# philips/janus

Hardware: AMD Instinct MI355X
Metric: reports prepared+aggregated/sec (helper, Prio3Histogram len=256) at 1/2/4/8 GPUs (higher is better)
Workload: dtype u32 limbs (Field128 mod-p integer arithmetic); 1 GPU; Prio3Histogram length=256 chunk_length=16 helper prepare_init+prepare_shares_to_prepare_message+prepare_next+aggregate, 1 segment; reports_per_gpu=1048576, global_batch=1048576, parallelism=dp1 (report shards; RCCL all-gather + mod-p combine)

## Files before the change

### janus_amd/csrc/prio3_accumulate.hip

```cpp
#include <hip/hip_runtime.h>

#include <algorithm>
#include <type_traits>

#include "prio3_host.h"
#include "sha256_device.h"

struct ZeroRanges {
  uint8_t* dst[4];
  size_t bytes[4];
};
__global__ __launch_bounds__(256) void k_zero(ZeroRanges z) {
  const size_t tid = blockIdx.x * (size_t)blockDim.x + threadIdx.x, nth = (size_t)gridDim.x * blockDim.x;
#pragma unroll
  for (int k = 0; k < 4; k++) {
    uint8_t* d = z.dst[k];
    const size_t n = z.bytes[k];
    if (!d || !n) continue;
    const size_t head = std::min(n, (size_t)((16 - ((uintptr_t)d & 15)) & 15));
    const size_t n16 = (n - head) / 16;
    for (size_t i = tid; i < n16; i += nth) ((uint4*)(d + head))[i] = make_uint4(0, 0, 0, 0);
    for (size_t i = tid * 4; i < head; i += nth * 4) *(uint32_t*)(d + i) = 0u;
    for (size_t i = head + 16 * n16 + tid * 4; i < n; i += nth * 4) *(uint32_t*)(d + i) = 0u;
  }
}


template <class F, int SG>
__global__ __launch_bounds__(256) void k_acc_seg(uint32_t n, size_t ld, uint32_t chunk,
                                                 uint32_t out_len, uint32_t nseg, const void* src,
                                                 const uint8_t* status, const uint32_t* seg,
                                                 const uint8_t* accept, void* partial,
                                                 uint64_t* pcount) {
  typedef typename F::T T;
  __shared__ T red[256];
  __shared__ uint32_t cred[256];
  const uint32_t e = blockIdx.x, c = blockIdx.y, s0 = blockIdx.z * SG;
  const uint32_t lo = c * chunk, hi = min(n, lo + chunk);
  T acc[SG];
  uint32_t cnt[SG];
#pragma unroll
  for (int q = 0; q < SG; q++) {
    acc[q] = F::zero();
    cnt[q] = 0;
  }
  for (uint32_t r = lo + threadIdx.x; r < hi; r += 256) {
    const uint32_t sr = seg ? seg[r] : 0u;
    const bool ok = status[r] == PRIO3_STATUS_FINISHED && sr < nseg && (!accept || accept[r]);
    const uint32_t k = (ok ? sr : 0xffffffffu) - s0;
    if (k < (uint32_t)SG) {
      const T x = F::load(src, (size_t)e * ld + r);
#pragma unroll
      for (int q = 0; q < SG; q++)
        if ((uint32_t)q == k) {
          acc[q] = F::add(acc[q], x);
          cnt[q]++;
        }
    }
  }
#pragma unroll
  for (int q = 0; q < SG; q++) {
    if (s0 + q >= nseg) break;
    red[threadIdx.x] = acc[q];
    cred[threadIdx.x] = cnt[q];
    __syncthreads();
    for (uint32_t st = 128; st > 0; st >>= 1) {
      if (threadIdx.x < st) {
        red[threadIdx.x] = F::add(red[threadIdx.x], red[threadIdx.x + st]);
        cred[threadIdx.x] += cred[threadIdx.x + st];
      }
      __syncthreads();
    }
    if (threadIdx.x == 0) {
      F::store(partial, ((size_t)c * nseg + s0 + q) * out_len + e, red[0]);
      if (e == 0) pcount[(size_t)c * nseg + s0 + q] = cred[0];
    }
    __syncthreads();
  }
}

template <class F>
__global__ void k_acc_fin(uint32_t nchunks, uint32_t out_len, uint32_t nseg, const void* partial,
                          const uint64_t* pcount, uint8_t* agg, uint64_t* count) {
  typedef typename F::T T;
  const uint32_t e = blockIdx.x * blockDim.x + threadIdx.x, s = blockIdx.y;
  if (e < out_len) {
    T acc = F::zero();
    for (uint32_t c = 0; c < nchunks; c++)
      acc = F::add(acc, F::load(partial, ((size_t)c * nseg + s) * out_len + e));
    F::store(agg, (size_t)s * out_len + e, acc);
  }
  if (e == 0) {
    uint64_t t = 0;
    for (uint32_t c = 0; c < nchunks; c++) t += pcount[(size_t)c * nseg + s];
    count[s] = t;
  }
}


template <class F>
__global__ __launch_bounds__(256) void k_acc_fin_blk(uint32_t nchunks, uint32_t out_len,
                                                     uint32_t nseg, const void* partial,
                                                     const uint64_t* pcount, uint8_t* agg,
                                                     uint64_t* count) {
  typedef typename F::T T;
  __shared__ T red[256];
  __shared__ uint64_t cred[256];
  const uint32_t e = blockIdx.x, s = blockIdx.y;
  T acc = F::zero();
  uint64_t t = 0;
  for (uint32_t c = threadIdx.x; c < nchunks; c += 256) {
    acc = F::add(acc, F::load(partial, ((size_t)c * nseg + s) * out_len + e));
    if (e == 0) t += pcount[(size_t)c * nseg + s];
  }
  red[threadIdx.x] = acc;
  cred[threadIdx.x] = t;
  __syncthreads();
  for (uint32_t st = 128; st > 0; st >>= 1) {
    if (threadIdx.x < st) {
      red[threadIdx.x] = F::add(red[threadIdx.x], red[threadIdx.x + st]);
      cred[threadIdx.x] += cred[threadIdx.x + st];
    }
    __syncthreads();
  }
  if (threadIdx.x == 0) {
    F::store(agg, (size_t)s * out_len + e, red[0]);
    if (e == 0) count[s] = cred[0];
  }
}

template <class F>
__global__ __launch_bounds__(256) void k_acc_multi(const AccDesc* descs, uint8_t* base) {
  typedef typename F::T T;
  __shared__ T red[256];
  __shared__ uint32_t cred[256];
  const AccDesc d = descs[blockIdx.y];
  const uint32_t e = blockIdx.x;
  if (e >= d.out_len) return;
  const uint32_t* seg = (d.flags & 1) ? (const uint32_t*)(base + d.seg_off) : nullptr;
  const uint8_t* acc = (d.flags & 2) ? base + d.acc_off : nullptr;
  for (uint32_t s0 = 0; s0 < d.nseg; s0 += 8) {
    T a[8];
    uint32_t c[8];
#pragma unroll
    for (int q = 0; q < 8; q++) {
      a[q] = F::zero();
      c[q] = 0;
    }
    for (uint32_t r = threadIdx.x; r < d.n; r += 256) {
      const uint32_t s = seg ? seg[r] : 0u;
      const bool inc = d.status[r] == PRIO3_STATUS_FINISHED && s < d.nseg && (!acc || acc[r]);
      const uint32_t k = s - s0;
      if (inc && k < 8u) {
        const T x = F::load(d.src, (size_t)e * d.ld + r);
#pragma unroll
        for (int q = 0; q < 8; q++)
          if ((uint32_t)q == k) {
            a[q] = F::add(a[q], x);
            c[q]++;
          }
      }
    }
    const uint32_t ns = min(8u, d.nseg - s0);
    for (uint32_t q = 0; q < ns; q++) {
      T v = F::zero();
      uint32_t cv = 0;
#pragma unroll
      for (int q2 = 0; q2 < 8; q2++)
        if ((uint32_t)q2 == q) {
          v = a[q2];
          cv = c[q2];
        }
      red[threadIdx.x] = v;
      cred[threadIdx.x] = cv;
      __syncthreads();
      for (uint32_t st = 128; st > 0; st >>= 1) {
        if (threadIdx.x < st) {
          red[threadIdx.x] = F::add(red[threadIdx.x], red[threadIdx.x + st]);
          cred[threadIdx.x] += cred[threadIdx.x + st];
        }
        __syncthreads();
      }
      if (threadIdx.x == 0) {
        F::store(base + d.agg_off, (size_t)(s0 + q) * d.out_len + e, red[0]);
        if (e == 0) ((uint64_t*)(base + d.cnt_off))[s0 + q] = cred[0];
      }
      __syncthreads();
    }
  }
}

__global__ __launch_bounds__(256) void k_agg_waves(uint32_t nwaves, uint32_t M,
                                                   const uint32_t* wpart, const uint32_t* wseg,
                                                   unsigned long long* cpart, uint32_t* cseg,
                                                   unsigned long long* agg64) {
  static_assert(WCH <= 64, "one chunk's wave segments are read by one wave");
  const uint32_t slot = 4 * (blockIdx.x * blockDim.x + threadIdx.x), c = blockIdx.y;
  const uint32_t w0 = c * WCH, w1 = min(nwaves, w0 + WCH), lane = threadIdx.x & 63u;
  const uint32_t my = w0 + lane < w1 ? wseg[w0 + lane] : 0xffffffffu;
  const uint64_t fused = __ballot(my != 0xffffffffu);
  const uint32_t s0 = fused ? (uint32_t)__shfl((int)my, __ffsll((long long)fused) - 1) : 0xffffffffu;
  const bool mixed = __any(my != 0xffffffffu && my != s0);
  if (slot == 0 && blockIdx.x == 0) cseg[c] = mixed ? 0xffffffffu : s0;
  if (s0 == 0xffffffffu) return;
  const bool act = slot < M * 8;
  const uint32_t ls = act ? slot : 0u;
  const size_t row = (size_t)M * 8;
  if (!mixed) {
    if (!act) return;
    unsigned long long a0 = 0, a1 = 0, a2 = 0, a3 = 0;
#pragma unroll
    for (uint32_t i = 0; i < WCH; i++) {
      const uint32_t w = min(w0 + i, w1 - 1);
      const uint4 v = *(const uint4*)(wpart + (size_t)w * row + slot);
      const uint32_t m = 0u - (uint32_t)((fused >> i) & 1u);
      a0 += v.x & m, a1 += v.y & m, a2 += v.z & m, a3 += v.w & m;
    }
    unsigned long long* o = cpart + (size_t)c * row + slot;
    o[0] = a0, o[1] = a1, o[2] = a2, o[3] = a3;
    return;
  }
  unsigned long long a0 = 0, a1 = 0, a2 = 0, a3 = 0;
  uint32_t cur = 0xffffffffu;
  auto flush = [&]() {
    if (cur == 0xffffffffu || !act) return;
    unsigned long long* o = agg64 + (size_t)cur * row + slot;
    if (a0) atomicAdd(o, a0);
    if (a1) atomicAdd(o + 1, a1);
    if (a2) atomicAdd(o + 2, a2);
    if (a3) atomicAdd(o + 3, a3);
  };
#pragma unroll 1
  for (uint32_t b = 0; b < WCH; b += 8) {
    uint4 v[8];
#pragma unroll
    for (uint32_t j = 0; j < 8; j++)
      v[j] = *(const uint4*)(wpart + (size_t)min(w0 + b + j, w1 - 1) * row + ls);
#pragma unroll
    for (uint32_t j = 0; j < 8; j++) {
      const uint32_t sg = (uint32_t)__builtin_amdgcn_readlane((int)my, (int)(b + j));
      if (sg == 0xffffffffu) continue;
      if (sg != cur) {
        flush();
        cur = sg;
        a0 = a1 = a2 = a3 = 0;
      }
      a0 += v[j].x, a1 += v[j].y, a2 += v[j].z, a3 += v[j].w;
    }
  }
  flush();
}

constexpr uint32_t FIX_T = 64;
static uint32_t fix_per(uint32_t n) { return n >= (1u << 18) ? 4096u : 512u; }
__global__ __launch_bounds__(256) void k_agg_fix(uint32_t n, const uint8_t* status,
                                                 const uint32_t* seg, const uint8_t* accept,
                                                 const uint32_t* wseg, uint32_t* fix,
                                                 uint32_t fix_cap, uint32_t nseg,
                                                 unsigned long long* counts, uint32_t oor_masked,
                                                 uint32_t per, uint32_t wshift) {
  __shared__ uint32_t tseg[FIX_T];
  __shared__ unsigned int tcnt[FIX_T];
  if (threadIdx.x < FIX_T) {
    tseg[threadIdx.x] = 0xffffffffu;
    tcnt[threadIdx.x] = 0;
  }
  __syncthreads();
  const uint32_t lo = blockIdx.x * per, hi = min(n, lo + per);
  for (uint32_t base = lo; base < hi; base += 256) {
    const uint32_t r = base + threadIdx.x;
    const bool valid = r < hi;
    const uint32_t sg = valid ? (seg ? seg[r] : 0u) : 0xffffffffu;
    const bool inc = valid && sg < nseg && status[r] == PRIO3_STATUS_FINISHED &&
                     (!accept || accept[r]);
    const bool fused = valid && wseg[r >> wshift] != 0xffffffffu && (!oor_masked || sg < nseg);
    const uint32_t s0 = (uint32_t)__shfl((int)sg, 0);
    const bool uni = __all(!valid || sg == s0);
    const unsigned long long b = __ballot(inc);
    auto add = [&](uint32_t s, unsigned int k) {
      const uint32_t h = s % FIX_T;
      const uint32_t old = atomicCAS(&tseg[h], 0xffffffffu, s);
      if (old == 0xffffffffu || old == s) atomicAdd(&tcnt[h], k);
      else atomicAdd(&counts[s], (unsigned long long)k);
    };
    if (uni) {
      if ((threadIdx.x & 63u) == 0 && b) add(s0, (unsigned int)__popcll(b));
    } else if (inc) {
      add(sg, 1u);
    }
    if (valid && fused != inc) {
      const uint32_t i = atomicAdd(&fix[0], 1u);
      if (i < fix_cap) fix[1 + i] = r | (inc ? 0u : 0x80000000u);
    }
  }
  __syncthreads();
  if (threadIdx.x < FIX_T && tseg[threadIdx.x] != 0xffffffffu && tcnt[threadIdx.x])
    atomicAdd(&counts[tseg[threadIdx.x]], (unsigned long long)tcnt[threadIdx.x]);
}

DEV f128 fold_halves_impl(const unsigned long long (&Hs)[8]);
DEV f128 fold_halves(const unsigned long long (&Hs)[8]) { return fold_halves_impl(Hs); }

__global__ __launch_bounds__(256) void k_agg_final(uint32_t M, size_t ld,
                                                   const unsigned long long* agg64,
                                                   uint32_t nchunks,
                                                   const unsigned long long* cpart,
                                                   const uint32_t* cseg, const uint32_t* fix,
                                                   const uint32_t* seg, const void* meas,
                                                   uint8_t* agg) {
  const uint32_t idx = blockIdx.x, s = idx / M, e = idx % M;
  const uint32_t tid = threadIdx.x, h = tid & 7u, cl = tid >> 3;
  __shared__ unsigned long long red[256];
  __shared__ f128 fadd[256], fsub[256];
  unsigned long long acc = 0;
  for (uint32_t c = cl; c < nchunks; c += 32)
    if (cseg[c] == s) acc += cpart[((size_t)c * M + e) * 8 + h];
  red[tid] = acc;
  f128 ad = zero128(), sb = zero128();
  const uint32_t nfix = fix[0];
  for (uint32_t i = tid; i < nfix; i += 256) {
    const uint32_t ent = fix[1 + i], r = ent & 0x7fffffffu;
    if ((seg ? seg[r] : 0u) != s) continue;
    const f128 x = Fp128::load(meas, (size_t)e * ld + r);
    if (ent & 0x80000000u) sb = add128(sb, x);
    else ad = add128(ad, x);
  }
  fadd[tid] = ad;
  fsub[tid] = sb;
  __syncthreads();
  for (uint32_t st = 128; st >= 8; st >>= 1) {
    if (tid < st) red[tid] += red[tid + st];
    __syncthreads();
  }
  for (uint32_t st = 128; st >= 1; st >>= 1) {
    if (tid < st) {
      fadd[tid] = add128(fadd[tid], fadd[tid + st]);
      fsub[tid] = add128(fsub[tid], fsub[tid + st]);
    }
    __syncthreads();
  }
  if (tid != 0) return;
  unsigned long long Hs[8];
  for (int hh = 0; hh < 8; hh++) Hs[hh] = red[hh] + agg64[(size_t)idx * 8 + hh];
  Fp128::store(agg, idx, sub128(add128(fold_halves(Hs), fadd[0]), fsub[0]));
}

__global__ __launch_bounds__(256) void k_agg_final_s(uint32_t M, size_t ld,
                                                     const unsigned long long* agg64,
                                                     uint32_t nchunks,
                                                     const unsigned long long* cpart,
                                                     const uint32_t* cseg, const uint32_t* fix,
                                                     const uint32_t* seg, const void* meas,
                                                     uint8_t* agg) {
  const uint32_t s = blockIdx.y, tid = threadIdx.x, h = tid & 7u, lane = tid & 63u;
  const uint32_t e = blockIdx.x * 32u + (tid >> 3);
  const bool live = e < M;
  const uint32_t ec = live ? e : 0u;
  unsigned long long H = agg64[((size_t)s * M + ec) * 8 + h];
  for (uint32_t c = 0; c < nchunks; c++)
    if (cseg[c] == s) H += cpart[((size_t)c * M + ec) * 8 + h];
  f128 ad = zero128(), sb = zero128();
  const uint32_t nfix = fix[0];
  for (uint32_t i = h; i < nfix; i += 8) {
    const uint32_t ent = fix[1 + i], r = ent & 0x7fffffffu;
    if ((seg ? seg[r] : 0u) != s) continue;
    const f128 x = Fp128::load(meas, (size_t)ec * ld + r);
    if (ent & 0x80000000u) sb = add128(sb, x);
    else ad = add128(ad, x);
  }
  if (nfix) {
#pragma unroll
    for (int m = 1; m < 8; m <<= 1) {
      f128 xa, xs;
#pragma unroll
      for (int k = 0; k < 4; k++) {
        xa.w[k] = (uint32_t)__shfl_xor((int)ad.w[k], m);
        xs.w[k] = (uint32_t)__shfl_xor((int)sb.w[k], m);
      }
      ad = add128(ad, xa);
      sb = add128(sb, xs);
    }
  }
  unsigned long long Hs[8];
#pragma unroll
  for (int k = 0; k < 8; k++) {
    const int src = (int)((lane & ~7u) + (uint32_t)k);
    Hs[k] = ((unsigned long long)(uint32_t)__shfl((int)(uint32_t)(H >> 32), src) << 32) |
            (uint32_t)__shfl((int)(uint32_t)H, src);
  }
  if (h != 0 || !live) return;
  Fp128::store(agg, (size_t)s * M + e, sub128(add128(fold_halves(Hs), ad), sb));
}

DEV f128 fold_halves_impl(const unsigned long long (&Hs)[8]) {
  uint32_t w[9] = {0, 0, 0, 0, 0, 0, 0, 0, 0};
  for (int hh = 0; hh < 8; hh++) {
    const unsigned long long H = Hs[hh];
    const int sh = 16 * hh, wi = sh >> 5, bi = sh & 31;
    const unsigned long long lo = bi ? (H << 16) & 0xffffffffull : H & 0xffffffffull;
    const unsigned long long mid = bi ? (H >> 16) & 0xffffffffull : H >> 32;
    const unsigned long long hi = bi ? H >> 48 : 0ull;
    unsigned long long c = (unsigned long long)w[wi] + lo;
    w[wi] = (uint32_t)c;
    c = (unsigned long long)w[wi + 1] + mid + (c >> 32);
    w[wi + 1] = (uint32_t)c;
    c = (unsigned long long)w[wi + 2] + hi + (c >> 32);
    w[wi + 2] = (uint32_t)c;
    for (int k = wi + 3; k < 9 && (c >> 32); k++) {
      c = (unsigned long long)w[k] + (c >> 32);
      w[k] = (uint32_t)c;
    }
  }
  return red288(w, w[8]);
}

template <class F>
__global__ void k_combine(uint32_t k, uint32_t len, uint32_t n_segments, const uint8_t* in,
                          const uint64_t* cin, uint8_t* out, uint64_t* cout) {
  typedef typename F::T T;
  const uint32_t e = blockIdx.x * blockDim.x + threadIdx.x;
  if (e < len) {
    T acc = F::zero();
    for (uint32_t i = 0; i < k; i++) acc = F::add(acc, F::load(in, (size_t)i * len + e));
    F::store(out, e, acc);
  }
  if (e < n_segments) {
    uint64_t s = 0;
    for (uint32_t i = 0; i < k; i++) s += cin[(size_t)i * n_segments + e];
    cout[e] = s;
  }
}

DEV void sha256_id16(const uint32_t id[4], uint32_t out[8]) {
  uint32_t w[16];
#pragma unroll
  for (int i = 0; i < 4; i++) w[i] = __builtin_bswap32(id[i]);
  w[4] = 0x80000000u;
#pragma unroll
  for (int i = 5; i < 15; i++) w[i] = 0;
  w[15] = 128;
  uint32_t st[8];
#pragma unroll
  for (int i = 0; i < 8; i++) st[i] = sha256d::IV[i];
  sha256d::compress(st, w);
#pragma unroll
  for (int i = 0; i < 8; i++) out[i] = __builtin_bswap32(st[i]);
}

__global__ void k_meta_init(uint32_t n_segments, uint32_t* ck, unsigned long long* iv) {
  const uint32_t s = blockIdx.x * blockDim.x + threadIdx.x;
  if (s >= n_segments) return;
  if (ck)
    for (int i = 0; i < 8; i++) ck[8 * s + i] = 0;
  if (iv) {
    iv[2 * s] = ~0ull;
    iv[2 * s + 1] = 0;
  }
}

constexpr uint32_t META_T = 1024, META_W = META_T / 64, META_BLOCKS = 512;
__global__ __launch_bounds__(1024) void k_meta(uint32_t n, const uint8_t* ids, const uint64_t* times,
                                             const uint8_t* status, const uint8_t* mask,
                                             const uint32_t* seg, uint32_t n_segments, uint32_t* ck,
                                             unsigned long long* iv) {
  __shared__ uint32_t s_seg0;
  __shared__ uint32_t s_ck[META_W][8];
  __shared__ unsigned long long s_lo[META_W], s_hi[META_W];
  const uint32_t tid = threadIdx.x, lane = tid & 63u, wv = tid >> 6;
  uint32_t cur = 0xffffffffu, acc_x = 0;
  unsigned long long acc_lo = ~0ull, acc_hi = 0;
  auto flush = [&]() {
    if (cur != 0xffffffffu) {
      if (ck && tid < 8 && acc_x) atomicXor(ck + 8 * cur + tid, acc_x);
      if (iv && tid == 8 && acc_hi) {
        atomicMin(iv + 2 * cur, acc_lo);
        atomicMax(iv + 2 * cur + 1, acc_hi);
      }
    }
    acc_x = 0;
    acc_lo = ~0ull;
    acc_hi = 0;
  };
  for (uint32_t base = blockIdx.x * META_T; base < n; base += gridDim.x * META_T) {
    const uint32_t r = base + tid;
    const bool valid = r < n;
    const uint32_t sg = valid ? (seg ? seg[r] : 0u) : 0xffffffffu;
    const bool in_range = valid && sg < n_segments;
    const bool inc = in_range && status[r] == PRIO3_STATUS_FINISHED && (!mask || mask[r]);
    uint32_t h[8] = {0, 0, 0, 0, 0, 0, 0, 0};
    if (ck && inc) {
      uint32_t id[4];
      load16(ids + 16 * (size_t)r, id);
      sha256_id16(id, h);
    }
    unsigned long long lo = ~0ull, hi = 0;
    if (times && in_range) {
      lo = times[r];
      hi = lo + 1;
    }
    if (tid == 0) s_seg0 = sg;
    __syncthreads();
    const bool uniform = __syncthreads_and(!valid || sg == s_seg0) && s_seg0 < n_segments;
    if (uniform) {
#pragma unroll
      for (int off = 32; off >= 1; off >>= 1) {
#pragma unroll
        for (int i = 0; i < 8; i++) h[i] ^= (uint32_t)__shfl_xor((int)h[i], off);
        const unsigned long long l2 = __shfl_xor(lo, off), h2 = __shfl_xor(hi, off);
        lo = l2 < lo ? l2 : lo;
        hi = h2 > hi ? h2 : hi;
      }
      if (lane == 0) {
#pragma unroll
        for (int i = 0; i < 8; i++) s_ck[wv][i] = h[i];
        s_lo[wv] = lo;
        s_hi[wv] = hi;
      }
      __syncthreads();
      if (s_seg0 != cur) {
        flush();
        cur = s_seg0;
      }
      if (tid < 8) {
        uint32_t x = 0;
        for (uint32_t q = 0; q < META_W; q++) x ^= s_ck[q][tid];
        acc_x ^= x;
      }
      if (tid == 8) {
        for (uint32_t q = 0; q < META_W; q++) {
          acc_lo = s_lo[q] < acc_lo ? s_lo[q] : acc_lo;
          acc_hi = s_hi[q] > acc_hi ? s_hi[q] : acc_hi;
        }
      }
    } else {
      if (ck && inc)
#pragma unroll
        for (int i = 0; i < 8; i++) atomicXor(ck + 8 * sg + i, h[i]);
      if (iv && times && in_range) {
        atomicMin(iv + 2 * sg, lo);
        atomicMax(iv + 2 * sg + 1, hi);
      }
    }
    __syncthreads();
  }
  flush();
}

__global__ void k_combine_meta(uint32_t k, uint32_t n_segments, const uint32_t* ck_in,
                               const unsigned long long* iv_in, uint32_t* ck_out,
                               unsigned long long* iv_out) {
  const uint32_t t = blockIdx.x * blockDim.x + threadIdx.x;
  if (t >= n_segments * 8) return;
  const uint32_t s = t >> 3, w = t & 7u;
  if (ck_in && ck_out) {
    uint32_t x = 0;
    for (uint32_t i = 0; i < k; i++) x ^= ck_in[((size_t)i * n_segments + s) * 8 + w];
    ck_out[(size_t)s * 8 + w] = x;
  }
  if (iv_in && iv_out && w == 0) {
    unsigned long long lo = ~0ull, hi = 0;
    for (uint32_t i = 0; i < k; i++) {
      const unsigned long long a = iv_in[((size_t)i * n_segments + s) * 2];
      const unsigned long long d = iv_in[((size_t)i * n_segments + s) * 2 + 1];
      if (d == 0) continue;
      lo = a < lo ? a : lo;
      hi = a + d > hi ? a + d : hi;
    }
    iv_out[2 * s] = hi ? lo : 0;
    iv_out[2 * s + 1] = hi ? hi - lo : 0;
  }
}

__global__ void k_meta_final(uint32_t n_segments, unsigned long long* iv) {
  const uint32_t s = blockIdx.x * blockDim.x + threadIdx.x;
  if (s >= n_segments) return;
  const unsigned long long lo = iv[2 * s], hi = iv[2 * s + 1];
  iv[2 * s] = hi ? lo : 0;
  iv[2 * s + 1] = hi ? hi - lo : 0;
}


template <class Fn>
static int by_field(size_t es, Fn fn) {
  return es == 16 ? fn(Fp128{}) : fn(Fp64{});
}

int run_accumulate(prio3_engine* e, Run* R, uint32_t c0, uint32_t n, const uint8_t* d_status,
                   const uint32_t* d_seg, const uint8_t* d_accept, uint32_t nseg, uint8_t* d_agg,
                   uint64_t* d_counts, hipStream_t st) {
  const DevParams& d = R->dp;
  const size_t es = d.es, agg_len = (size_t)d.out_len * es;
  if (n == 0) {
    HIPCHK(hipMemsetAsync(d_agg, 0, agg_len * nseg, st));
    HIPCHK(hipMemsetAsync(d_counts, 0, 8 * (size_t)nseg, st));
    return PRIO3_OK;
  }
  const bool short_out = d.out_len <= 4;
  const uint32_t chunk = short_out ? 2048 : 8192, nchunks = (n + chunk - 1) / chunk;
  const size_t part_b = ((size_t)nchunks * nseg * agg_len + 255) & ~(size_t)255;
  int rc = PRIO3_OK;
  Slab* tmp = ws_acquire(R->device, part_b + 8 * (size_t)nchunks * nseg, st, &rc);
  if (!tmp) return rc;
  void* partial = tmp->base;
  uint64_t* pcount = (uint64_t*)(tmp->base + part_b);
  const uint8_t* src = run_out_shares(R, c0);
  const size_t ld = d.ld_out;
  const int SG = nseg == 1 ? 1 : nseg <= 4 ? 4 : 8;
  const dim3 grid(d.out_len, nchunks, (nseg + SG - 1) / SG);
  rc = by_field(es, [&](auto f) -> int {
    using F = decltype(f);
    auto seg = [&](auto sg) -> int {
      TIMED(e, st, "k_acc_seg",
            (k_acc_seg<F, decltype(sg)::value><<<grid, 256, 0, st>>>(
                n, ld, chunk, d.out_len, nseg, src, d_status, d_seg, d_accept, partial, pcount)));
      return PRIO3_OK;
    };
    const int rs = SG == 1   ? seg(std::integral_constant<int, 1>{})
                   : SG == 4 ? seg(std::integral_constant<int, 4>{})
                             : seg(std::integral_constant<int, 8>{});
    if (rs) return rs;
    if (short_out)
      TIMED(e, st, "k_acc_fin",
            (k_acc_fin_blk<F><<<dim3(d.out_len, nseg), 256, 0, st>>>(
                nchunks, d.out_len, nseg, partial, pcount, d_agg, d_counts)));
    else
      TIMED(e, st, "k_acc_fin",
            (k_acc_fin<F><<<dim3((d.out_len + 255) / 256, nseg), 256, 0, st>>>(
                nchunks, d.out_len, nseg, partial, pcount, d_agg, d_counts)));
    return PRIO3_OK;
  });
  ws_release(tmp, st);
  R->last = st;
  return rc;
}

int fused_finish(prio3_engine* e, Run* R, const uint8_t* d_status, const uint32_t* seg,
                 const uint32_t* fix_seg, const uint8_t* d_accept_mask, uint32_t S,
                 uint8_t* d_agg_shares, uint64_t* d_counts, hipStream_t st) {
  const uint32_t n = R->n, M = R->dp.meas_len, ws = R->wshift;
  const uint32_t nwaves = (n + (1u << ws) - 1) >> ws;
  {
    ZeroRanges z{};
    z.dst[0] = (uint8_t*)R->agg64;
    z.bytes[0] = (size_t)S * M * 8 * 8;
    z.dst[1] = (uint8_t*)R->fix;
    z.bytes[1] = sizeof(uint32_t);
    z.dst[2] = (uint8_t*)d_counts;
    z.bytes[2] = 8 * (size_t)S;
    TIMED(e, st, "k_zero", (k_zero<<<std::min<uint32_t>(256, (uint32_t)((z.bytes[0] / 16 + 255) / 256) + 1), 256, 0, st>>>(z)));
  }
  const uint32_t nchunks = (nwaves + WCH - 1) / WCH;
  dim3 g1((M * 8 / 4 + 255) / 256, nchunks);
  TIMED(e, st, "k_agg_waves",
        (k_agg_waves<<<g1, 256, 0, st>>>(nwaves, M, R->wpart, R->wseg, R->cpart, R->cseg,
                                         R->agg64)));
  TIMED(e, st, "k_agg_fix",
        (k_agg_fix<<<(n + fix_per(n) - 1) / fix_per(n), 256, 0, st>>>(
            n, d_status, seg, d_accept_mask, R->wseg, R->fix, (uint32_t)(R->fix_cap - 1), S,
            (unsigned long long*)d_counts, fix_seg ? 1u : 0u, fix_per(n), ws)));
  if (nchunks <= 64 && S > 1)
    TIMED(e, st, "k_agg_final",
          (k_agg_final_s<<<dim3((M + 31) / 32, S), 256, 0, st>>>(
              M, R->dp.ld, R->agg64, nchunks, R->cpart, R->cseg, R->fix, fix_seg, R->sc.meas,
              d_agg_shares)));
  else
    TIMED(e, st, "k_agg_final",
          (k_agg_final<<<S * M, 256, 0, st>>>(M, R->dp.ld, R->agg64, nchunks, R->cpart, R->cseg,
                                               R->fix, fix_seg, R->sc.meas, d_agg_shares)));
  return PRIO3_OK;
}

Slab* acc_multi_enqueue(int device, uint32_t es, uint8_t* host, const AccLayout& L,
                        uint32_t n_jobs, size_t out_bytes, hipStream_t st, int* rc) {
  const AccDesc* D = (const AccDesc*)(host + L.desc_off);
  uint32_t reps = 0, max_len = 0;
  for (uint32_t i = 0; i < n_jobs; i++) {
    reps = std::max(reps, (uint32_t)((D[i].acc_off - L.acc_off) + D[i].n));
    max_len = std::max(max_len, D[i].out_len);
  }
  Slab* sl = ws_acquire(device, L.bytes, st, rc);
  if (!sl) return nullptr;
  uint8_t* b = sl->base;
  auto h2d = [&](size_t off, size_t bytes) {
    return hipMemcpyAsync(b + off, host + off, bytes, hipMemcpyHostToDevice, st) == hipSuccess;
  };
  bool ok = h2d(L.desc_off, sizeof(AccDesc) * n_jobs) && h2d(L.seg_off, 4 * (size_t)reps) &&
            h2d(L.acc_off, reps);
  if (ok) {
    by_field(es, [&](auto f) -> int {
      k_acc_multi<decltype(f)><<<dim3(max_len, n_jobs), 256, 0, st>>>(
          (const AccDesc*)(b + L.desc_off), b);
      return 0;
    });
    ok = hipGetLastError() == hipSuccess &&
         hipMemcpyAsync(host + L.out_off, b + L.out_off, out_bytes, hipMemcpyDeviceToHost, st) ==
             hipSuccess;
  }
  if (ok) return sl;
  (void)hipStreamSynchronize(st);
  ws_release(sl, st);
  *rc = PRIO3_EDEVICE;
  return nullptr;
}

int launch_combine(prio3_engine* e, uint32_t k, uint32_t n_segments, const uint8_t* d_in,
                   const uint64_t* d_counts_in, uint8_t* d_out, uint64_t* d_counts_out,
                   hipStream_t st) {
  const uint32_t len = e->dp.out_len * n_segments;
  const uint32_t blocks = (std::max(len, n_segments) + 255) / 256;
  return by_field(e->dp.es, [&](auto f) -> int {
    TIMED(e, st, "k_combine",
          (k_combine<decltype(f)><<<blocks, 256, 0, st>>>(k, len, n_segments, d_in, d_counts_in,
                                                          d_out, d_counts_out)));
    return PRIO3_OK;
  });
}

int launch_batch_metadata(prio3_engine* e, uint32_t n, const uint8_t* d_report_ids,
                          const uint64_t* d_times, const uint8_t* d_status,
                          const uint8_t* d_accept_mask, const uint32_t* d_segment_ids,
                          uint32_t n_segments, uint32_t* ck, unsigned long long* iv,
                          hipStream_t st) {
  const uint32_t sb = (n_segments + 255) / 256;
  TIMED(e, st, "k_meta_init", (k_meta_init<<<sb, 256, 0, st>>>(n_segments, ck, iv)));
  if (n)
    TIMED(e, st, "k_meta",
          (k_meta<<<std::min((n + META_T - 1) / META_T, META_BLOCKS), META_T, 0, st>>>(
              n, d_report_ids, d_times, d_status, d_accept_mask, d_segment_ids, n_segments, ck,
              d_times ? iv : nullptr)));
  if (iv) TIMED(e, st, "k_meta_final", (k_meta_final<<<sb, 256, 0, st>>>(n_segments, iv)));
  return PRIO3_OK;
}

int launch_combine_metadata(prio3_engine* e, uint32_t k, uint32_t n_segments,
                            const uint32_t* ck_in, const unsigned long long* iv_in,
                            uint32_t* ck_out, unsigned long long* iv_out, hipStream_t st) {
  TIMED(e, st, "k_combine_meta",
        (k_combine_meta<<<(n_segments * 8 + 255) / 256, 256, 0, st>>>(k, n_segments, ck_in, iv_in,
                                                                      ck_out, iv_out)));
  return PRIO3_OK;
}
```

### janus_amd/csrc/prio3_common.h

```cpp
#pragma once
#include <atomic>
#include <mutex>
#include <string>
#include <vector>
#include "../../include/janus_prio3.h"
#include "prio3_device.h"

#define MAX_ROOTS 20

#ifdef JANUS_DEVICE_CHECKS
#define DCHECK(c)                                                                        \
  do {                                                                                   \
    if (!(c)) {                                                                          \
      printf("janus device check failed: %s (%s:%d) block %u thread %u\n", #c, __FILE__, \
             __LINE__, (unsigned)blockIdx.x, (unsigned)threadIdx.x);                     \
      __builtin_trap();                                                                  \
    }                                                                                    \
  } while (0)
#else
#define DCHECK(c) ((void)0)
#endif

struct DevParams {
  uint32_t kind, es, meas_len, out_len, jr_len, arity, calls, P, logP, glen, proof_len,
      verifier_len, chunk, bits, length, prep_share_len, helper_share_len, public_share_len,
      leader_share_len;
  uint32_t n, ld, force_slow;
  uint32_t nseg;
  uint32_t qr_len, ld_out;
  uint32_t chunk1, calls1, P1, logP1, glen1;
  uint32_t invP1_128[4], normc128[4], twon128[4];
  uint32_t vk[4];
  uint32_t dst[8][2];
  uint32_t roots128[MAX_ROOTS + 1][4];
  uint64_t roots64[MAX_ROOTS + 1];
  uint32_t invP128[4], half128[4];
  uint32_t sigma128[32][4];
  uint32_t tw128[16][4];
  uint64_t invP64, half64;
  const uint4* sigma_dev;
  uint32_t trunc_xof;
  uint32_t slow_defer, redo;
  uint32_t tws[24][4];
#ifdef JANUS_TEST_REJECT
  uint32_t test_reject;
#endif
};
#ifdef JANUS_TEST_REJECT
#define REJ_BITS(p) ((p).test_reject)
#define BX_REJ(x) ((x).rej)
#define BX_SET_REJ(x, p) ((x).rej = (p).test_reject)
#else
#define REJ_BITS(p) 0u
#define BX_REJ(x) 0u
#define BX_SET_REJ(x, p) ((void)0)
#endif

struct InPtrs {
  const uint8_t* nonces;
  const uint8_t* pub;
  const uint8_t* helper;
  const uint8_t* leader;
  const uint16_t* vk_slot = nullptr;
  const uint4* vk_tab = nullptr;
  const uint8_t* leader_src = nullptr;
  const uint32_t* seg_src = nullptr;
  uint32_t* seg_dst = nullptr;
  const uint8_t* accept_src = nullptr;
  uint8_t* accept_dst = nullptr;
  uint32_t lin_ld = 0;
};

DEV void load_vk(const DevParams& p, const InPtrs& in, uint32_t r, uint32_t vk[4]) {
  if (in.vk_slot) {
    const uint4 v = in.vk_tab[in.vk_slot[r]];
    vk[0] = v.x;
    vk[1] = v.y;
    vk[2] = v.z;
    vk[3] = v.w;
  } else {
    vk[0] = p.vk[0];
    vk[1] = p.vk[1];
    vk[2] = p.vk[2];
    vk[3] = p.vk[3];
  }
}

struct Scratch {
  void* meas;
  void* proofs;
  void* jr;
  void* qr;
  uint4* part;
  uint4* corrected;
  uint8_t* flag;
  void* Lbuf;
  void* PVbuf;
  void* acc;
  void* out;
  void* beta;
  const uint32_t* seg;
  uint32_t* wpart;
  uint32_t* wseg;
};

struct OutPtrs {
  uint8_t* prep_msgs;
  uint8_t* status;
};

template <class F>
struct FC;
template <>
struct FC<Fp128> {
  static DEV f128 root(const DevParams& p, int l) { return Fp128::from_words(p.roots128[l]); }
  static DEV f128 invP(const DevParams& p) { return Fp128::from_words(p.invP128); }
  static DEV f128 half(const DevParams& p) { return Fp128::from_words(p.half128); }
};
template <>
struct FC<Fp64> {
  static DEV uint64_t root(const DevParams& p, int l) { return p.roots64[l]; }
  static DEV uint64_t invP(const DevParams& p) { return p.invP64; }
  static DEV uint64_t half(const DevParams& p) { return p.half64; }
};

DEV void load16(const uint8_t* p, uint32_t* w) {
  uint4 v = *(const uint4*)p;
  w[0] = v.x;
  w[1] = v.y;
  w[2] = v.z;
  w[3] = v.w;
}

DEV bool prep_msg_check(const DevParams& p, const InPtrs& in, const Scratch& sc, uint32_t r,
                        const uint32_t lpart[4], uint32_t msg[4]) {
  const uint4 cor = sc.corrected[r];
  uint32_t hpart[4];
  {
    const uint4 hp = sc.part[r];
    hpart[0] = hp.x, hpart[1] = hp.y, hpart[2] = hp.z, hpart[3] = hp.w;
  }
  KState s;
  kzero(s);
  Msg mm;
  msg_zero(mm);
  msg_dst(mm, p.dst[6]);
  msg_bytes16(mm, 25, lpart);
  msg_bytes16(mm, 41, hpart);
  msg_absorb_final(s, mm, 57);
  msg[0] = kword(s, 0), msg[1] = kword(s, 1), msg[2] = kword(s, 2), msg[3] = kword(s, 3);
  return msg[0] == cor.x && msg[1] == cor.y && msg[2] == cor.z && msg[3] == cor.w;
}

struct BX {
  KState s;
  uint8_t buf[168];
  uint32_t pos;
#ifdef JANUS_TEST_REJECT
  uint32_t rej = 0;
#endif
};
DEV void bx_xor_block(BX& x) {
#pragma unroll
  for (int w = 0; w < 42; w++) {
    uint32_t v = (uint32_t)x.buf[4 * w] | ((uint32_t)x.buf[4 * w + 1] << 8) |
                 ((uint32_t)x.buf[4 * w + 2] << 16) | ((uint32_t)x.buf[4 * w + 3] << 24);
    kxor_word(x.s, w, v);
  }
  keccak_p12(x.s);
}
DEV void bx_fill(BX& x) {
#pragma unroll
  for (int w = 0; w < 42; w++) {
    uint32_t v = kword(x.s, w);
    x.buf[4 * w] = v;
    x.buf[4 * w + 1] = v >> 8;
    x.buf[4 * w + 2] = v >> 16;
    x.buf[4 * w + 3] = v >> 24;
  }
  x.pos = 0;
}
DEV void bx_absorb(BX& x, uint8_t b) {
  x.buf[x.pos++] = b;
  if (x.pos == 168) {
    bx_xor_block(x);
    x.pos = 0;
  }
}
DEV void bx_absorb_w(BX& x, const uint32_t* w, int nbytes) {
  for (int i = 0; i < nbytes; i++) bx_absorb(x, (uint8_t)(w[i >> 2] >> (8 * (i & 3))));
}
DEV void bx_init(BX& x, const uint32_t* dst2, const uint32_t* seed) {
  kzero(x.s);
  x.pos = 0;
  bx_absorb(x, 8);
  bx_absorb_w(x, dst2, 8);
  bx_absorb_w(x, seed, 16);
}
DEV void bx_finalize(BX& x) {
  for (uint32_t i = x.pos; i < 168; i++) x.buf[i] = 0;
  x.buf[x.pos] ^= 0x01;
  x.buf[167] ^= 0x80;
  bx_xor_block(x);
  bx_fill(x);
}
DEV uint8_t bx_squeeze(BX& x) {
  if (x.pos == 168) {
    keccak_p12(x.s);
    bx_fill(x);
  }
  return x.buf[x.pos++];
}
template <class F>
DEV void bx_next_elem(BX& x, uint32_t* w) {
  for (;;) {
    for (int k = 0; k < F::ES / 4; k++) {
      uint32_t v = 0;
      for (int b = 0; b < 4; b++) v |= (uint32_t)bx_squeeze(x) << (8 * b);
      w[k] = v;
    }
    if (F::accept(F::from_words(w), BX_REJ(x))) return;
  }
}

template <class F>
DEV void bx_expand(const DevParams& p, const uint32_t* dst2, const uint32_t* seed,
                   const uint8_t* binder, int blen, uint32_t n, void* base, size_t ld,
                   uint32_t r) {
  BX x;
  BX_SET_REJ(x, p);
  bx_init(x, dst2, seed);
  for (int i = 0; i < blen; i++) bx_absorb(x, binder[i]);
  bx_finalize(x);
  for (uint32_t i = 0; i < n; i++) {
    uint32_t w[4];
    bx_next_elem<F>(x, w);
    F::store(base, (size_t)i * ld + r, F::from_words(w));
  }
}

template <class F>
DEV void put_elem(const DevParams& p, void* base, uint32_t idx, uint32_t r, const uint32_t* w,
                  uint32_t& flag) {
  typename F::T x = F::from_words(w);
  if (!F::accept(x, REJ_BITS(p))) flag = 1;
  DCHECK(r < p.ld);
  F::store(base, (size_t)idx * p.ld + r, x);
}

template <class F, class Put>
DEV void squeeze_block_with(const KState& s, uint32_t b, uint32_t n_elems, uint32_t& pend0,
                            uint32_t& pend1, Put&& put) {
  if constexpr (F::ES == 16) {
    uint32_t e0 = 21 * (b >> 1);
    if ((b & 1) == 0) {
#pragma unroll
      for (int t = 0; t < 10; t++) {
        uint32_t w[4] = {kword(s, 4 * t), kword(s, 4 * t + 1), kword(s, 4 * t + 2),
                         kword(s, 4 * t + 3)};
        if (e0 + t < n_elems) put(e0 + t, w);
      }
      pend0 = kword(s, 40);
      pend1 = kword(s, 41);
    } else {
      {
        uint32_t w[4] = {pend0, pend1, kword(s, 0), kword(s, 1)};
        if (e0 + 10 < n_elems) put(e0 + 10, w);
      }
#pragma unroll
      for (int t = 0; t < 10; t++) {
        uint32_t w[4] = {kword(s, 2 + 4 * t), kword(s, 3 + 4 * t), kword(s, 4 + 4 * t),
                         kword(s, 5 + 4 * t)};
        if (e0 + 11 + t < n_elems) put(e0 + 11 + t, w);
      }
    }
  } else {
    uint32_t e0 = 21 * b;
#pragma unroll
    for (int t = 0; t < 21; t++) {
      uint32_t w[2] = {kword(s, 2 * t), kword(s, 2 * t + 1)};
      if (e0 + t < n_elems) put(e0 + t, w);
    }
  }
}

template <class F>
DEV void squeeze_block(const DevParams& p, const KState& s, uint32_t b, uint32_t n_elems,
                       uint32_t& pend0, uint32_t& pend1, void* base, uint32_t r,
                       uint32_t& flag) {
  squeeze_block_with<F>(s, b, n_elems, pend0, pend1, [&](uint32_t i, const uint32_t* w) {
    put_elem<F>(p, base, i, r, w, flag);
  });
}

DEV void shl_add160(sum128& a, const f128& m, uint32_t s) {
  uint32_t w0 = m.w[0], w1 = m.w[1], w2 = m.w[2], w3 = m.w[3], w4 = 0;
  if (s) {
    const uint32_t rs = 32 - s;
    w4 = m.w[3] >> rs;
    w3 = __builtin_amdgcn_alignbit(m.w[3], m.w[2], rs);
    w2 = __builtin_amdgcn_alignbit(m.w[2], m.w[1], rs);
    w1 = __builtin_amdgcn_alignbit(m.w[1], m.w[0], rs);
    w0 = m.w[0] << s;
  }
  uint32_t c;
  a.w[0] = addc(a.w[0], w0, 0, &c);
  a.w[1] = addc(a.w[1], w1, c, &c);
  a.w[2] = addc(a.w[2], w2, c, &c);
  a.w[3] = addc(a.w[3], w3, c, &c);
  a.w[4] = a.w[4] + w4 + c;
}

struct TruncSink {
  void* out;
  size_t ld_out;
  uint32_t r, nb, n_ent, e, bit;
  sum128 acc;
  DEV TruncSink(const DevParams& p, void* o, uint32_t rr)
      : out(o), ld_out(p.ld_out), r(rr), nb(p.bits), n_ent(p.out_len), e(0), bit(0) {
    sum_zero(acc);
  }
  DEV void put(const f128& m) {
    if (e >= n_ent) return;
    shl_add160(acc, m, bit);
    if (++bit == nb) {
      Fp128::store(out, (size_t)e * ld_out + r, sum_reduce(acc));
      sum_zero(acc);
      bit = 0;
      e++;
    }
  }
};

template <bool TR>
DEV void squeeze_meas(const DevParams& p, const KState& s, uint32_t b, uint32_t n_elems,
                      uint32_t& pend0, uint32_t& pend1, void* base, uint32_t r, uint32_t& flag,
                      TruncSink& ts) {
  squeeze_block_with<Fp128>(s, b, n_elems, pend0, pend1, [&](uint32_t i, const uint32_t* w) {
    put_elem<Fp128>(p, base, i, r, w, flag);
    if constexpr (TR) ts.put(mk128(w[0], w[1], w[2], w[3]));
  });
}


DEV uint32_t bitrev(uint32_t x, uint32_t d) { return __builtin_bitreverse32(x) >> (32 - d); }

template <class F>
DEV void dft_lane(const DevParams& p, void* buf, uint32_t r, uint32_t n, uint32_t logn) {
  typedef typename F::T T;
  const size_t ld = p.ld;
  DCHECK(r < ld);
  for (uint32_t l = 1; l <= logn; l++) {
    const uint32_t half = 1u << (l - 1);
    const T wl = FC<F>::root(p, l);
    T w = F::one();
    for (uint32_t i = 0; i < half; i++) {
      for (uint32_t j = i; j < n; j += 2 * half) {
        T u = F::load(buf, (size_t)j * ld + r);
        T v = F::mul(w, F::load(buf, (size_t)(j + half) * ld + r));
        F::store(buf, (size_t)j * ld + r, F::add(u, v));
        F::store(buf, (size_t)(j + half) * ld + r, F::sub(u, v));
      }
      w = F::mul(w, wl);
    }
  }
}

template <class F>
DEV typename F::T ldf(const void* base, uint32_t e, size_t ld, uint32_t r) {
  DCHECK(r < ld);
  return F::load(base, (size_t)e * ld + r);
}


template <int N, int LOGN>
DEV void dft_reg(const DevParams& p, f128 (&x)[N], int stride) {
  typedef Fp128 F;
#pragma unroll
  for (int l = 1; l <= LOGN; l++) {
    const int half = 1 << (l - 1);
#pragma unroll
    for (int i = 0; i < half; i++) {
      const f128 w = F::from_words(p.tw128[i * stride * (N >> l)]);
#pragma unroll
      for (int j = i; j < N; j += 2 * half) {
        const f128 u = x[j];
        const f128 v = (i == 0) ? x[j + half] : F::mul(w, x[j + half]);
        x[j] = F::add(u, v);
        x[j + half] = F::sub(u, v);
      }
    }
  }
}

template <class F>
DEV bool flp_query_lane(const DevParams& p, const void* meas, const void* proofs, const void* jr,
                        typename F::T t, void* Lbuf, void* PVbuf, void* acc, uint32_t r,
                        typename F::T& v, typename F::T& pt) {
  typedef typename F::T T;
  const size_t ld = p.ld;
  const uint32_t P = p.P, A = p.arity;
  T tp = t;
  for (uint32_t l = 0; l < p.logP; l++) tp = F::mul(tp, tp);
  const bool t_ok = !F::eq(tp, F::one());
  {
    T pw = FC<F>::invP(p);
    for (uint32_t e = 0; e < P; e++) {
      F::store(Lbuf, (size_t)bitrev(e, p.logP) * ld + r, pw);
      pw = F::mul(pw, t);
    }
    dft_lane<F>(p, Lbuf, r, p.P, p.logP);
  }
  for (uint32_t e = 0; e < P; e++) {
    T q = ldf<F>(proofs, A + e, ld, r);
    if (e + P < p.glen) q = F::add(q, ldf<F>(proofs, A + e + P, ld, r));
    F::store(PVbuf, (size_t)bitrev(e, p.logP) * ld + r, q);
  }
  dft_lane<F>(p, PVbuf, r, p.P, p.logP);
  pt = F::zero();
  for (uint32_t e = p.glen; e-- > 0;) pt = F::add(F::mul(pt, t), ldf<F>(proofs, A + e, ld, r));
  auto Lc = [&](uint32_t c) { return ldf<F>(Lbuf, (P - c) & (P - 1), ld, r); };
  {
    const T L0 = Lc(0);
    for (uint32_t w = 0; w < A; w++)
      F::store(acc, (size_t)w * ld + r, F::mul(ldf<F>(proofs, w, ld, r), L0));
  }
  auto acc_add = [&](uint32_t w, const T& v) {
    size_t idx = (size_t)w * ld + r;
    F::store(acc, idx, F::add(F::load(acc, idx), v));
  };
  v = F::zero();
  if (p.kind == PRIO3_COUNT) {
    const T m = ldf<F>(meas, 0, ld, r);
    const T x = F::mul(m, Lc(1));
    acc_add(0, x);
    acc_add(1, x);
    v = F::sub(ldf<F>(PVbuf, 1, ld, r), m);
  } else if (p.kind == PRIO3_SUM) {
    const T r0 = ldf<F>(jr, 0, ld, r);
    T rp = r0;
    for (uint32_t i = 0; i < p.meas_len; i++) {
      acc_add(0, F::mul(ldf<F>(meas, i, ld, r), Lc(i + 1)));
      v = F::add(v, F::mul(rp, ldf<F>(PVbuf, i + 1, ld, r)));
      rp = F::mul(rp, r0);
    }
  } else {
    const T r0 = ldf<F>(jr, 0, ld, r);
    const T half = FC<F>::half(p);
    T rp = r0, range = F::zero(), sum = F::zero();
    for (uint32_t k = 0; k < p.calls; k++) {
      const T L = Lc(k + 1);
      for (uint32_t j = 0; j < p.chunk; j++) {
        const uint32_t i = k * p.chunk + j;
        const T m = i < p.meas_len ? ldf<F>(meas, i, ld, r) : F::zero();
        acc_add(2 * j, F::mul(F::mul(rp, m), L));
        acc_add(2 * j + 1, F::mul(F::sub(m, half), L));
        rp = F::mul(rp, r0);
        sum = F::add(sum, m);
      }
      range = F::add(range, ldf<F>(PVbuf, k + 1, ld, r));
    }
    if (p.kind == PRIO3_SUMVEC) {
      v = range;
    } else {
      const T r1 = ldf<F>(jr, 1, ld, r);
      v = F::add(F::mul(r1, range), F::mul(F::mul(r1, r1), F::sub(sum, half)));
    }
  }
  return t_ok;
}

namespace {

typedef unsigned __int128 u128;
const u128 HP128 = (((u128)0xffffffffffffffe4ULL) << 64) | 1;
const uint64_t HP64 = 0xffffffff00000001ULL;

u128 hmul(u128 a, u128 b, u128 p) {
  u128 r = 0;
  a %= p;
  while (b) {
    if (b & 1) {
      r += a;
      if (r < a || r >= p) r -= p;
    }
    u128 a2 = a + a;
    if (a2 < a || a2 >= p) a2 -= p;
    a = a2;
    b >>= 1;
  }
  return r;
}
u128 hpow(u128 a, u128 e, u128 p) {
  u128 r = 1;
  while (e) {
    if (e & 1) r = hmul(r, a, p);
    a = hmul(a, a, p);
    e >>= 1;
  }
  return r;
}

}

struct KTime {
  std::string name;
  double ms = 0;
  uint64_t launches = 0;
};

struct Mp64Params {
  uint32_t meas_len, out_len, bits, chunk, calls, P, logP, glen, proof_len ,
      arity, vlen, np;
  uint32_t dst[8][2];
  uint32_t vk_ist[8], vk_ost[8];
  uint32_t z_ist[8], z_ost[8];
  uint64_t alpha, alpha_inv, invP, half;
  const uint64_t* sigma;
};

struct prio3_engine;
bool query_sum_takes(const DevParams& p);
bool launch_query_sum(const DevParams& p, InPtrs in, Scratch sc, OutPtrs out, hipStream_t st,
                      bool leader = false);
int launch_mp64(prio3_engine* e, uint32_t n, uint32_t ld, InPtrs in, OutPtrs out, Scratch sc,
                hipStream_t st);
int launch_mp64_leader(prio3_engine* e, uint32_t n, uint32_t ld, InPtrs in, OutPtrs out,
                       Scratch sc, hipStream_t st);
int launch_mp64_leader_next(uint32_t n, const uint8_t* d_prep_msgs, Scratch sc, uint8_t* d_status,
                            hipStream_t st);
bool launch_xof_pair(const DevParams& p, InPtrs in, Scratch sc, hipStream_t st);
bool prep_pair_takes(const DevParams& p, bool pull);
bool launch_prep_pair(const DevParams& p, InPtrs in, Scratch sc, OutPtrs out, hipStream_t st,
                      bool fuse, bool pull);
bool launch_query_wide(const DevParams& p, InPtrs in, Scratch sc, OutPtrs out, hipStream_t st);
bool query_wide_takes(const DevParams& p);
void launch_fpvec_query(const DevParams& p, InPtrs in, Scratch sc, OutPtrs out, hipStream_t st,
                        bool wide, bool leader);
bool fpvec_query_wide_takes(const DevParams& p);

struct Slab;
struct Run {
  prio3_engine* e = nullptr;
  Slab* slab = nullptr;
  int device = 0;
  DevParams dp;
  uint32_t n = 0;
  Scratch sc{};
  uint8_t *nonces = nullptr, *pub = nullptr, *helper = nullptr, *leader = nullptr,
          *linput = nullptr, *msgs = nullptr, *status = nullptr;
  uint32_t *wpart = nullptr, *wseg = nullptr, *cseg = nullptr, *fix = nullptr;
  uint4* corr_all = nullptr;
  unsigned long long *cpart = nullptr, *agg64 = nullptr;
  size_t fix_cap = 0;
  bool fused = false;
  bool aggregate = false;
  bool lfused = false;
  uint32_t wshift = 6;
  uint32_t nseg = 0;
  const uint32_t* seg = nullptr;
  uint32_t* gseg = nullptr;
  uint8_t *gaccept = nullptr, *gagg = nullptr, *gcnt = nullptr;
  std::atomic<int> refs{1};
  hipStream_t last = nullptr;
  bool keep = false;
  uint32_t hpke_stride = 0;
  uint8_t *hstatus = nullptr, *hpt = nullptr;
  uint32_t* hretry = nullptr;
  uint32_t* gck = nullptr;
  unsigned long long* giv = nullptr;
};

struct prio3_engine {
  prio3_params params;
  prio3_sizes_t sz;
  DevParams dp;
  int device;
  Run* cur = nullptr;
  int fuse_acc = 1;
  int leader_fast = 1;
  int leader_fuse_acc = 1;
  int chunks = 0;
  int64_t fp_sub_bytes = 0;
  int coalesce = 1;
  int experimental_fpvec = 0;
  std::vector<hipStream_t> side;
  std::vector<hipEvent_t> side_ev;
  hipEvent_t fork_ev = nullptr;
  int force_slow = 0;
  int force_generic = 0;
  int n_cu = 256;
  int fp_round = 1;
  int pair_max = 196608;
  int timing = 0;
  int keep_scratch = 0;
  int upload_aead = 0;
  Mp64Params mp{};
  uint64_t* d_sigma64 = nullptr;
  uint4* d_sigma128 = nullptr;
  std::vector<KTime> times;
  std::mutex tmu;
  std::mutex mu;
  int lane = 0;
  std::vector<prio3_engine*> members;
  prio3_engine* owner = nullptr;
  std::atomic<uint32_t> rr{0};
  std::atomic<uint64_t> placed_jobs{0}, placed_reports{0};
};
```

### janus_amd/csrc/prio3_engine.hip

```cpp
#include <hip/hip_runtime.h>

#include <cstdio>
#include <cstdlib>
#include <cstring>
#include <mutex>
#include <string>
#include <type_traits>
#include <vector>

#include "../../include/janus_hpke.h"
#include "../../include/janus_prio3.h"
#include "prio3_host.h"
#include "sha256_host.h"

DEV void pull_body(const PullRanges& pr, size_t tid, size_t nth) {
#pragma unroll
  for (int k = 0; k < 4; k++) {
    const size_t n16 = pr.bytes[k] / 16;
    const uint4* s16 = (const uint4*)pr.src[k];
    uint4* d16 = (uint4*)pr.dst[k];
    for (size_t i = tid; i < n16; i += nth) d16[i] = s16[i];
    const size_t t = 16 * n16 + tid;
    if (t < pr.bytes[k] && tid < 16) pr.dst[k][t] = pr.src[k][t];
  }
// ... 92 lines not shown
static uint32_t optimal_chunk_length(uint32_t m) {
  if (m <= 1) return 1;
  uint32_t max_log2 = 0;
  while ((1u << max_log2) < m) max_log2++;
  max_log2 += 1;
  uint64_t best = UINT64_MAX;
  uint32_t best_chunk = 1;
  for (uint32_t l = max_log2; l >= 1; l--) {
    const uint64_t calls = (1ull << l) - 1, chunk = (m + calls - 1) / calls;
    const uint64_t cost = 2 * chunk + 2 * ((1ull << l) - 1) + 1;
    if (cost < best) {
      best = cost;
      best_chunk = (uint32_t)chunk;
    }
  }
  return best_chunk;
}

static int fill_sizes(const prio3_params* pp, prio3_sizes_t* s, DevParams* dp) {
  if (!pp) return PRIO3_EINVAL;
  uint32_t proofs = pp->num_proofs ? pp->num_proofs : 1;
  const bool mp = pp->kind == PRIO3_SUMVEC_F64_MP;
  if (mp ? (proofs < 2 || proofs > 8) : proofs != 1) return mp ? PRIO3_EINVAL : PRIO3_EUNSUPPORTED;
  DevParams d;
  memset(&d, 0, sizeof d);
  d.kind = pp->kind;
  d.bits = pp->bits;
  d.length = pp->length;
  d.chunk = pp->chunk_length;
  uint32_t algo;
  switch (pp->kind) {
    case PRIO3_COUNT:
      algo = 0;
      d.es = 8;
      d.meas_len = 1;
      d.out_len = 1;
      d.jr_len = 0;
      d.arity = 2;
      d.calls = 1;
      break;
    case PRIO3_SUM:
      if (pp->bits == 0 || pp->bits > 64) return PRIO3_EINVAL;
      algo = 1;
      d.es = 16;
      d.meas_len = pp->bits;
      d.out_len = 1;
      d.jr_len = 1;
      d.arity = 1;
      d.calls = pp->bits;
      break;
    case PRIO3_SUMVEC:
      if (pp->bits == 0 || pp->bits > 64 || pp->length == 0 || pp->chunk_length == 0)
        return PRIO3_EINVAL;
      algo = 2;
      d.es = 16;
      d.meas_len = pp->bits * pp->length;
      d.out_len = pp->length;
      d.jr_len = 1;
      d.arity = 2 * pp->chunk_length;
      d.calls = (d.meas_len + pp->chunk_length - 1) / pp->chunk_length;
      break;
    case PRIO3_SUMVEC_F64_MP:
      if (pp->bits == 0 || pp->bits > 64 || pp->length == 0 || pp->chunk_length == 0)
        return PRIO3_EINVAL;
      algo = 0xFFFF1003u;
      d.es = 8;
      d.meas_len = pp->bits * pp->length;
      d.out_len = pp->length;
      d.jr_len = 1;
      d.arity = 2 * pp->chunk_length;
      d.calls = (d.meas_len + pp->chunk_length - 1) / pp->chunk_length;
      break;
    case PRIO3_FPVEC_BOUNDED_L2:
      if ((pp->bits != 16 && pp->bits != 32) || pp->length == 0 || pp->length > (1u << 22))
        return PRIO3_EINVAL;
      algo = 0xFFFF0000u;
      d.es = 16;
      d.meas_len = pp->bits * pp->length + 2 * pp->bits - 2;
      d.out_len = pp->length;
      d.jr_len = 2;
      d.qr_len = 2;
      d.chunk = optimal_chunk_length(d.meas_len);
      d.arity = 2 * d.chunk;
      d.calls = (d.meas_len + d.chunk - 1) / d.chunk;
      d.chunk1 = optimal_chunk_length(pp->length);
      d.calls1 = (pp->length + d.chunk1 - 1) / d.chunk1;
      break;
    case PRIO3_HISTOGRAM:
      if (pp->length == 0 || pp->chunk_length == 0) return PRIO3_EINVAL;
      algo = 3;
      d.es = 16;
      d.meas_len = pp->length;
      d.out_len = pp->length;
      d.jr_len = 2;
      d.arity = 2 * pp->chunk_length;
      d.calls = (pp->length + pp->chunk_length - 1) / pp->chunk_length;
      break;
    default:
      return PRIO3_EINVAL;
  }
  d.P = next_pow2(1 + d.calls);
  d.logP = 0;
  while ((1u << d.logP) < d.P) d.logP++;
  if (d.logP > MAX_ROOTS) return PRIO3_EUNSUPPORTED;
  d.glen = 2 * (d.P - 1) + 1;
  d.proof_len = d.arity + d.glen;
  d.verifier_len = d.arity + 2;
  if (!d.qr_len) d.qr_len = 1;
  if (d.kind == PRIO3_FPVEC_BOUNDED_L2) {
    d.P1 = next_pow2(1 + d.calls1);
    while ((1u << d.logP1) < d.P1) d.logP1++;
    if (d.logP1 > MAX_ROOTS) return PRIO3_EUNSUPPORTED;
    d.glen1 = 2 * (d.P1 - 1) + 1;
    d.proof_len += d.chunk1 + d.glen1;
    d.verifier_len = 1 + d.arity + 1 + d.chunk1 + 1;
  }
  const uint32_t S = mp ? 32 : 16;
  d.helper_share_len = d.jr_len ? 3 * S : 2 * S;
  d.public_share_len = d.jr_len ? 2 * S : 0;
  d.prep_share_len = d.verifier_len * proofs * d.es + (d.jr_len ? S : 0);
  d.leader_share_len = (d.meas_len + d.proof_len * proofs) * d.es + (d.jr_len ? S : 0);
  for (uint32_t u = 1; u <= 7; u++) {
    uint8_t b[8] = {8, 0, (uint8_t)(algo >> 24), (uint8_t)(algo >> 16), (uint8_t)(algo >> 8),
                    (uint8_t)algo, 0, (uint8_t)u};
    memcpy(d.dst[u], b, 8);
  }
  {
    u128 g128 = 0;
    for (const char* c = "145091266659756586618791329697897684742"; *c; c++)
      g128 = g128 * 10 + (u128)(*c - '0');
    uint64_t g64 = 1753635133440165772ULL;
    for (int l = 0; l <= MAX_ROOTS; l++) {
      u128 r = g128;
      for (int i = 0; i < 66 - l; i++) r = hmul(r, r, HP128);
      for (int k = 0; k < 4; k++) d.roots128[l][k] = (uint32_t)(r >> (32 * k));
      u128 r64 = g64;
      for (int i = 0; i < 32 - l; i++) r64 = hmul(r64, r64, HP64);
      d.roots64[l] = (uint64_t)r64;
    }
    u128 ip = hpow(d.P, HP128 - 2, HP128), h = hpow(2, HP128 - 2, HP128);
    for (int k = 0; k < 4; k++) {
      d.invP128[k] = (uint32_t)(ip >> (32 * k));
      d.half128[k] = (uint32_t)(h >> (32 * k));
    }
    d.invP64 = (uint64_t)hpow(d.P, HP64 - 2, HP64);
    if (d.kind == PRIO3_FPVEC_BOUNDED_L2) {
      const u128 ip1 = hpow(d.P1, HP128 - 2, HP128);
      const u128 nc = ((u128)d.out_len << (2 * d.bits - 2)) >> 1;
      const u128 tn = (u128)1 << d.bits;
      for (int k = 0; k < 4; k++) {
        d.invP1_128[k] = (uint32_t)(ip1 >> (32 * k));
        d.normc128[k] = (uint32_t)(nc >> (32 * k));
        d.twon128[k] = (uint32_t)(tn >> (32 * k));
      }
    }
    if (d.P <= 32) {
      u128 alpha = 0;
      for (int k = 0; k < 4; k++) alpha |= (u128)d.roots128[d.logP][k] << (32 * k);
      for (uint32_t e2 = 0; e2 < d.P; e2++) {
        u128 ae = hpow(alpha, e2, HP128), s = 0, x = 1;
        for (uint32_t cc = 1; cc <= d.calls; cc++) {
          x = hmul(x, ae, HP128);
          s += x;
          if (s < x || s >= HP128) s -= HP128;
        }
        for (int k = 0; k < 4; k++) d.sigma128[e2][k] = (uint32_t)(s >> (32 * k));
      }
      for (uint32_t i = 0; i < d.P / 2; i++) {
        u128 w = hpow(alpha, i, HP128);
        for (int k = 0; k < 4; k++) d.tw128[i][k] = (uint32_t)(w >> (32 * k));
      }
    } else if (d.P == 64 || d.P == 128) {
      u128 alpha = 0;
      for (int k = 0; k < 4; k++) alpha |= (u128)d.roots128[d.logP][k] << (32 * k);
      const u128 aq = hpow(alpha, 8, HP128);
      for (uint32_t i = 0; i < d.P / 16; i++) {
        const u128 w = hpow(aq, i, HP128);
        for (int k = 0; k < 4; k++) d.tw128[i][k] = (uint32_t)(w >> (32 * k));
      }
      for (uint32_t i = 0; i < 8; i++) {
        const u128 w = hpow(alpha, i, HP128);
        for (int k = 0; k < 4; k++) d.tw128[8 + i][k] = (uint32_t)(w >> (32 * k));
      }
    }
    if (d.P >= 16 && d.P <= 128) {
      u128 alpha = 0;
      for (int k = 0; k < 4; k++) alpha |= (u128)d.roots128[d.logP][k] << (32 * k);
      const u128 w16 = hpow(alpha, d.P / 16, HP128), a16 = hpow(alpha, 16, HP128);
      for (uint32_t i = 0; i < 8; i++) {
        const u128 v[3] = {hpow(w16, i, HP128), hpow(alpha, i, HP128), hpow(a16, i, HP128)};
        for (int t = 0; t < 3; t++)
          for (int k = 0; k < 4; k++) d.tws[8 * t + i][k] = (uint32_t)(v[t] >> (32 * k));
      }
    }
    d.half64 = (uint64_t)hpow(2, HP64 - 2, HP64);
  }
  if (s) {
    s->field_bytes = d.es;
    s->meas_len = d.meas_len;
    s->out_len = d.out_len;
    s->proof_len = d.proof_len;
    s->verifier_len = d.verifier_len;
    s->joint_rand_len = d.jr_len;
    s->nonce_len = 16;
    s->public_share_len = d.public_share_len;
    s->helper_share_len = d.helper_share_len;
    s->prep_share_len = d.prep_share_len;
    s->prep_msg_len = d.jr_len ? S : 0;
    s->agg_share_len = d.out_len * d.es;
    s->leader_input_share_len = d.leader_share_len;
  }
  d.proof_len *= proofs;
  if (dp) *dp = d;
  return PRIO3_OK;
}

std::vector<Pending>& pending() {
  static thread_local std::vector<Pending> v;
  return v;
}
size_t time_slot(prio3_engine* e, const char* name) {
  std::lock_guard<std::mutex> lk(e->tmu);
  for (size_t i = 0; i < e->times.size(); i++)
    if (e->times[i].name == name) return i;
  e->times.push_back(KTime{name, 0, 0});
  return e->times.size() - 1;
}
void count_launch(prio3_engine* e, const char* name) {
  const size_t i = time_slot(e, name);
  std::lock_guard<std::mutex> lk(e->tmu);
  e->times[i].launches += 1;
}
void collect_times(prio3_engine* e, bool wait) {
  auto& v = pending();
  std::vector<Pending> keep;
  for (auto& pd : v) {
    if (pd.e != e || (!wait && hipEventQuery(pd.b) == hipErrorNotReady)) {
      keep.push_back(pd);
      continue;
    }
    float ms = 0;
    (void)hipEventSynchronize(pd.b);
    (void)hipEventElapsedTime(&ms, pd.a, pd.b);
    {
      std::lock_guard<std::mutex> lk(e->tmu);
      e->times[pd.idx].ms += ms;
      e->times[pd.idx].launches += 1;
    }
    (void)hipEventDestroy(pd.a);
    (void)hipEventDestroy(pd.b);
  }
  v.swap(keep);
}

static size_t fp_column_bytes(const DevParams& d) {
  const size_t es = d.es;
  return es * ((size_t)d.meas_len + d.proof_len + d.jr_len + d.qr_len + 2 * ((size_t)d.P + d.P1) +
               d.calls) +
         16 + 16 + 1;
}

static uint32_t fp_sub_ld(const prio3_engine* e, const DevParams& d, uint32_t ld_out,
                          size_t other_bytes) {
  const size_t per = fp_column_bytes(d);
  int64_t budget = e->fp_sub_bytes;
  if (budget <= 0) {
    size_t fr = 0, tot = 0, idle = 0;
    if (hipMemGetInfo(&fr, &tot) != hipSuccess) {
      (void)hipGetLastError();
      fr = tot = 0;
    }
    (void)ws_pool_bytes(e->device, &idle);
    const int64_t outb = (int64_t)(d.es * d.out_len * (size_t)ld_out + 64 * (size_t)ld_out);
    const int64_t reserve = std::max<int64_t>((int64_t)8 << 30, (int64_t)(0.10 * (double)tot));
    budget = (int64_t)(fr + idle) - outb - reserve - (int64_t)other_bytes;
  }
  uint64_t cols = (uint64_t)std::max<int64_t>(budget, 1) / per;
  cols = std::max<uint64_t>(256, cols & ~255ull);
  return (uint32_t)std::min<uint64_t>(ld_out, cols);
}

static size_t run_carve(Run* R, unsigned flags, uint8_t* base) {
  const DevParams& d = R->dp;
  const size_t es = d.es, ld = d.ld, ldo = d.ld_out, n = R->n ? R->n : 1;
  size_t off = 0;
  auto take = [&](auto** ptr, size_t bytes) {
    *ptr = base ? (std::remove_pointer_t<decltype(ptr)>)(base + off) : nullptr;
    off += (bytes + 255) & ~(size_t)255;
  };
  if (flags & RUN_SCRATCH) {
    const bool fp = d.kind == PRIO3_FPVEC_BOUNDED_L2;
    take(&R->sc.meas, es * d.meas_len * ld);
    take(&R->sc.proofs, es * d.proof_len * ld);
    take(&R->sc.jr, es * (d.jr_len ? d.jr_len : 1) * ld);
    take(&R->sc.qr, es * d.qr_len * ld);
    take(&R->sc.part, 16 * ld);
    take(&R->sc.corrected, 16 * ld);
    take(&R->sc.flag, ld);
    take(&R->sc.Lbuf, es * ((size_t)d.P + d.P1) * ld);
    take(&R->sc.PVbuf, es * ((size_t)d.P + d.P1) * ld);
    take(&R->sc.acc, fp ? 16 : es * d.arity * ld);
    take(&R->sc.out, own_out(d) ? es * d.out_len * ldo : 16);
    take(&R->sc.beta, es * d.calls * ld);
    if (fp) take(&R->corr_all, 16 * n);
  }
  if (flags & RUN_IO) {
    const size_t ml = R->e->sz.prep_msg_len ? R->e->sz.prep_msg_len : 16;
    take(&R->nonces, 16 * n);
    take(&R->pub, (size_t)(d.public_share_len ? d.public_share_len : 16) * n);
    take(&R->helper, (size_t)d.helper_share_len * n);
    take(&R->leader, (size_t)d.prep_share_len * n);
    take(&R->msgs, ml * n);
    take(&R->status, n);
  }
  if (flags & RUN_LINPUT) take(&R->linput, (size_t)d.leader_share_len * n);
  if (flags & RUN_AGG_IO) {
    const size_t S = R->nseg ? R->nseg : 1;
    take(&R->gseg, 4 * n);
    take(&R->gaccept, n);
    take(&R->gagg, (size_t)d.out_len * es * S);
    take(&R->gcnt, 8 * S);
  }
  if (flags & RUN_HPKE) {
    take(&R->hstatus, n);
    take(&R->hpt, (size_t)R->hpke_stride * n);
    take(&R->hretry, 4 * (n + 1));
  }
  if (flags & RUN_JIX) {
    const size_t S = R->nseg ? R->nseg : 1;
    take(&R->gck, 32 * S);
    take(&R->giv, 16 * S);
  }
  if (flags & RUN_FUSED) {
    const size_t waves = (n + 31) / 32, M = d.meas_len, chunks = (waves + WCH - 1) / WCH;
    take(&R->wpart, waves * M * 8 * sizeof(uint32_t));
    take(&R->wseg, waves * sizeof(uint32_t));
    take(&R->cpart, chunks * M * 8 * 8);
    take(&R->cseg, chunks * sizeof(uint32_t));
    take(&R->agg64, (size_t)(R->nseg ? R->nseg : 1) * M * 8 * 8);
    take(&R->fix, (n + 1) * sizeof(uint32_t));
  }
  return off;
}

static Run* run_create(prio3_engine* e, uint32_t n, unsigned flags, uint32_t nseg,
                       hipStream_t st, int* rc, uint32_t hpke_stride = 0) {
  Run* R = new Run();
  R->e = e;
  R->hpke_stride = hpke_stride;
  R->device = e->device;
  R->n = n;
  R->nseg = nseg;
  R->dp = e->dp;
  R->dp.n = n;
  R->dp.nseg = nseg ? nseg : 1;
  const uint32_t ld_out = ((n ? n : 1) + 63) & ~63u;
  R->dp.ld_out = ld_out;
  R->dp.ld = ld_out;
  if ((flags & RUN_SCRATCH) && e->dp.kind == PRIO3_FPVEC_BOUNDED_L2) {
    const size_t other = run_carve(R, flags & ~RUN_SCRATCH, nullptr);
    R->dp.ld = fp_sub_ld(e, e->dp, ld_out, other);
  }
  const size_t bytes = run_carve(R, flags, nullptr);
  R->slab = ws_acquire(e->device, bytes, st, rc);
  if (!R->slab) {
    delete R;
    return nullptr;
  }
  run_carve(R, flags, R->slab->base);
  R->keep = e->keep_scratch != 0;
  R->fix_cap = (size_t)n + 1;
  R->last = st;
  return R;
}

static void run_release(Run* R, hipStream_t st, bool use_st) {
  if (!R) return;
  if (R->refs.fetch_sub(1) != 1) return;
  ws_release(R->slab, use_st ? st : R->last, R->keep);
  delete R;
}

static int run_output_shares(Run* R, uint32_t c0, uint32_t n, uint8_t* out, hipStream_t st) {
  const DevParams& d = R->dp;
  const size_t es = d.es;
  if (n == 0) return PRIO3_OK;
  const uint8_t* src = run_out_shares(R, c0);
  std::vector<uint8_t> soa((size_t)d.out_len * n * es);
  HIPCHK(hipMemcpy2DAsync(soa.data(), n * es, src, (size_t)d.ld_out * es, n * es, d.out_len,
                          hipMemcpyDeviceToHost, st));
  HIPCHK(hipStreamSynchronize(st));
  for (uint32_t r = 0; r < n; r++)
    for (uint32_t i = 0; i < d.out_len; i++)
      memcpy(out + ((size_t)r * d.out_len + i) * es, soa.data() + ((size_t)i * n + r) * es, es);
  return PRIO3_OK;
}

int engine_device(const prio3_engine* e) { return e->device; }
int engine_exec_id(const prio3_engine* e) { return e->device * EXEC_LANES + e->lane; }

static prio3_engine* place(prio3_engine* e, uint32_t n) {
  prio3_engine* best = e;
  const size_t k = e->members.size();
  if (k > 1) {
    const uint32_t s0 = e->rr.fetch_add(1, std::memory_order_relaxed);
    uint64_t bl = UINT64_MAX;
    for (size_t i = 0; i < k; i++) {
      prio3_engine* m = e->members[(s0 + i) % k];
      const uint64_t l = exec_load(engine_exec_id(m));
      if (l < bl) {
        bl = l;
        best = m;
      }
    }
  }
  best->placed_jobs.fetch_add(1, std::memory_order_relaxed);
  best->placed_reports.fetch_add(n, std::memory_order_relaxed);
  return best;
}

void engine_vk(const prio3_engine* e, uint8_t out[16]) { memcpy(out, e->dp.vk, 16); }

static uint64_t fnv(uint64_t h, const void* p, size_t n) {
  const uint8_t* b = (const uint8_t*)p;
  for (size_t i = 0; i < n; i++) h = (h ^ b[i]) * 1099511628211ull;
  return h;
}

uint32_t engine_job_align(const prio3_engine* e) { return fusable(e) ? 64u : 1u; }

uint64_t engine_group_key(const prio3_engine* e) {
  uint64_t h = 1469598103934665603ull;
  h = fnv(h, &e->params, sizeof e->params);
  h = fnv(h, &e->device, sizeof e->device);
  const int opts[] = {e->force_slow, e->chunks, e->fuse_acc,           e->leader_fast,
                      e->leader_fuse_acc, e->fp_round, e->experimental_fpvec, e->force_generic,
                      e->timing, e->pair_max};
  h = fnv(h, opts, sizeof opts);
  h = fnv(h, &e->fp_sub_bytes, sizeof e->fp_sub_bytes);
  if (e->dp.kind == PRIO3_SUMVEC_F64_MP || !e->coalesce) {
    static std::atomic<uint64_t> solo{0};
    const uint64_t u[2] = {(uint64_t)(uintptr_t)e, e->coalesce ? 0 : ++solo};
    h = fnv(h, u, sizeof u);
  }
  return h;
}

uint64_t exec_job_key(const ExecJob* j) {
  uint64_t h = engine_group_key(j->e);
  if (j->opener) {
    const uint64_t u[4] = {0x5345414C4544ull, hpke_opener_key(j->opener), j->ct_stride,
                           (uint64_t)j->require_taskprov};
    h = fnv(h, u, sizeof u);
    if (j->fallback) {
      const uint64_t f[2] = {0x46414C4C4241434Bull, hpke_opener_key(j->fallback)};
      h = fnv(h, f, sizeof f);
    }
  }
  if (j->jix) {
    const uint64_t u = 0x4A4F42494E444558ull;
    h = fnv(h, &u, sizeof u);
  }
  return h;
}

void engine_io_layout(const prio3_engine* e, uint32_t cap, IoLayout* L, const ExecJob* job) {
  const DevParams& d = e->dp;
  const bool sealed = job && job->opener;
  L->len[0] = 16;
  L->len[1] = d.public_share_len;
  L->len[2] = sealed ? 0 : d.helper_share_len;
  L->len[3] = d.prep_share_len;
  size_t off = 0;
  for (int f = 0; f < 4; f++) {
    L->off[f] = off;
    off += (L->len[f] * cap + 15) & ~(size_t)15;
  }
  L->slot_off = off;
  off += (2 * (size_t)cap + 15) & ~(size_t)15;
  L->tab_off = off;
  off += 16 * (size_t)exec_max_keys();
  L->msg_len = e->sz.prep_msg_len;
  L->msg_off = off;
  off += L->msg_len * cap;
  L->status_off = off;
  off += cap;
  off = (off + 15) & ~(size_t)15;
  L->seg_off = off;
  off += (4 * (size_t)cap + 15) & ~(size_t)15;
  L->accept_off = off;
  off += (cap + 15) & ~(size_t)15;
  L->agg_len = (size_t)d.out_len * d.es;
  L->max_seg = (uint32_t)std::max<size_t>(1, std::min<size_t>(EXEC_MAX_SEGS,
                                                                ((size_t)16 << 20) / L->agg_len));
  L->agg_off = off;
  off += (L->agg_len * L->max_seg + 15) & ~(size_t)15;
  L->cnt_off = off;
  off += 8 * (size_t)L->max_seg;
  L->nenc = L->ct_stride = 0;
  if (sealed) {
    auto up = [](size_t x) { return (x + 15) & ~(size_t)15; };
    L->nenc = (uint32_t)hpke_opener_nenc(job->opener);
    L->ct_stride = job->ct_stride;
    off = up(off);
    L->enc_off = off;
    off += up((size_t)L->nenc * cap);
    L->ct_off = off;
    off += up((size_t)L->ct_stride * cap);
    L->ctlen_off = off;
    off += up(4 * (size_t)cap);
    L->time_off = off;
    off += up(8 * (size_t)cap);
    L->tslot_off = off;
    off += up(2 * (size_t)cap);
    L->ttab_off = off;
    off += 32 * (size_t)HPKE_MAX_TASKS;
    L->dtab_off = off;
    off += 8 * (size_t)HPKE_MAX_TASKS;
  }
  L->jix = job && job->jix;
  if (L->jix) {
    auto up = [](size_t x) { return (x + 15) & ~(size_t)15; };
    const size_t S = L->max_seg;
    off = up(off);
    L->jdesc_off = off;
    off += up(sizeof(JixJobDesc) * S);
    L->jclosed_off = off;
    off += 16 * (size_t)JIX_GROUP_CLOSED;
    L->jseg_off = off;
    off += up(4 * (size_t)cap);
    L->jrej_off = off;
    off += up(cap);
    L->jdup_off = off;
    off += up(cap);
    L->jstart_off = off;
    off += 8 * S;
    L->jinfo_off = off;
    off += up(sizeof(prio3_job_index_info) * S);
    L->ck_off = off;
    off += 32 * S;
    L->iv_off = off;
    off += 16 * S;
  }
  L->bytes = off;
}

static void record_prep(GroupRun* gr, hipStream_t st) {
  if (hipEventCreateWithFlags(&gr->prep, hipEventDisableTiming) != hipSuccess ||
      hipEventRecord(gr->prep, st) != hipSuccess) {
    (void)hipGetLastError();
    if (gr->prep) (void)hipEventDestroy(gr->prep);
    gr->prep = nullptr;
  }
}

static int group_begin(prio3_engine* lead, const DeviceGuard& dg, int jobs, bool own_queue,
                       uint32_t n, unsigned flags, uint32_t nseg, uint32_t hpke_stride,
                       GroupRun* gr) {
  *gr = GroupRun();
  gr->lead = lead;
  gr->jobs = jobs;
  HIPCHK(dg.rc);
  hipStream_t st = own_queue ? ws_exec_stream_get(lead->device) : ws_stream_get(lead->device);
  if (!st) return PRIO3_EDEVICE;
  int rc = PRIO3_OK;
  Run* R = run_create(lead, n, flags, nseg, st, &rc, hpke_stride);
  if (!R) {
    ws_exec_stream_put(lead->device, st);
    return rc;
  }
  gr->st = st;
  gr->R = R;
  return PRIO3_OK;
}
static int group_fail(GroupRun* gr, int code) {
  (void)hipStreamSynchronize(gr->st);
  run_release(gr->R, gr->st, true);
  if (gr->prep) (void)hipEventDestroy(gr->prep);
  ws_exec_stream_put(gr->lead->device, gr->st);
  *gr = GroupRun();
  return code;
}

__global__ __launch_bounds__(256) void k_hpke_merge(uint32_t n, const uint8_t* hs, uint8_t* status,
                                                    const uint64_t* times, const uint16_t* tslot,
                                                    const uint64_t* dtab) {
  const uint32_t i = blockIdx.x * 256u + threadIdx.x;
  if (i >= n) return;
  if (hs[i])
    status[i] = (uint8_t)(0x80u | hs[i]);
  else if (times && times[i] > dtab[tslot[i]])
    status[i] = (uint8_t)PRIO3_STATUS_REPORT_TOO_EARLY;
}

__global__ __launch_bounds__(256) void k_hpke_retry_list(uint32_t n, const uint8_t* hs,
                                                         const uint32_t* ct_len,
                                                         uint32_t ct_stride, uint32_t* list) {
  const uint32_t i = blockIdx.x * 256u + threadIdx.x;
  bool q = false;
  if (i < n && hs[i] == 4) {
    const uint32_t cl = ct_len[i];
    q = cl >= 16 && cl <= ct_stride;
  }
  const uint64_t m = __ballot(q);
  if (!m) return;
  const uint32_t lane = threadIdx.x & 63u;
  uint32_t base = 0;
  if (lane == 0) base = atomicAdd(list, (uint32_t)__popcll(m));
  base = (uint32_t)__shfl((int)base, 0);
  if (q) list[1 + base + (uint32_t)__popcll(m & ((1ull << lane) - 1ull))] = i;
}

int engine_group_issue(prio3_engine* lead, const GroupView& g, GroupRun* gr, bool own_queue) {
  DeviceGuard dg_(lead->device);
  const bool mp = lead->dp.kind == PRIO3_SUMVEC_F64_MP;
  const bool agg = g.nseg > 0;
  const bool fuse = agg && fusable(lead);
  IoLayout L;
  if (g.L)
    L = *g.L;
  else
    engine_io_layout(lead, g.cap, &L);
  const bool sealed = L.ct_stride > 0 && g.opener;
  const bool jix = g.njix > 0 && agg && sealed && L.jix;
  if (g.njix && !jix) return PRIO3_EINVAL;
  int rc = group_begin(lead, dg_, g.jobs, own_queue, g.n,
                       RUN_SCRATCH | RUN_IO | (agg ? (unsigned)RUN_AGG_IO : 0u) |
                           (fuse ? (unsigned)RUN_FUSED : 0u) | (sealed ? (unsigned)RUN_HPKE : 0u) |
                           (jix ? (unsigned)RUN_JIX : 0u),
                       agg ? g.nseg : 0, sealed ? L.ct_stride : 0, gr);
  if (rc) return rc;
  Run* R = gr->R;
  hipStream_t st = gr->st;
  auto fail = [&](int code) { return group_fail(gr, code); };
  const uint8_t* hd = g.stg_dev;
  InPtrs in{hd + L.off[0], L.len[1] ? hd + L.off[1] : nullptr, hd + L.off[2], R->leader};
  if (jix) {
    uint8_t* sd = g.stg_dev;
    JixGroupArgs a{};
    a.desc = (const JixJobDesc*)(hd + L.jdesc_off);
    a.closed = (const unsigned long long*)(hd + L.jclosed_off);
    a.ids = hd + L.off[0];
    a.times = (const unsigned long long*)(hd + L.time_off);
    a.accept = hd + L.accept_off;
    a.ids_dev = R->nonces;
    a.gseg = R->gseg;
    a.gaccept = R->gaccept;
    a.seg_out = (uint32_t*)(sd + L.jseg_off);
    a.rej_out = sd + L.jrej_off;
    a.dup_out = sd + L.jdup_off;
    a.starts_out = (unsigned long long*)(sd + L.jstart_off);
    a.info_out = (prio3_job_index_info*)(sd + L.jinfo_off);
    if (launch_jix_group(lead, g.njix, a, st) != PRIO3_OK) return fail(PRIO3_EDEVICE);
  }
  if (sealed) {
    HpkeGroupArgs a{};
    a.n = g.n;
    a.ct_stride = L.ct_stride;
    a.share_len = lead->dp.helper_share_len;
    a.pub_len = (uint32_t)L.len[1];
    a.require_taskprov = g.require_taskprov;
    a.enc = hd + L.enc_off;
    a.ct = hd + L.ct_off;
    a.ct_len = (const uint32_t*)(hd + L.ctlen_off);
    a.ids = hd + L.off[0];
    a.times = (const uint64_t*)(hd + L.time_off);
    a.pubs = L.len[1] ? hd + L.off[1] : nullptr;
    a.task_slot = (const uint16_t*)(hd + L.tslot_off);
    a.task_tab = (const uint32_t*)(hd + L.ttab_off);
    a.pt = R->hpt;
    a.shares = R->helper;
    a.status = R->hstatus;
    if (hpke_open_group_launch(g.opener, a, st) != PRIO3_OK) return fail(PRIO3_EDEVICE);
    if (g.fallback) {
// ... 1481 lines not shown
```

### janus_amd/csrc/prio3_host.h

```cpp
#pragma once
#include <hip/hip_runtime.h>

#include <cstdio>
#include <vector>

#include "prio3_common.h"
#include "prio3_runtime.h"

#define HIPCHK(x)                                                                   \
  do {                                                                              \
    hipError_t _e = (x);                                                            \
    if (_e != hipSuccess) {                                                         \
      fprintf(stderr, "janus_prio3: HIP error %s at %s:%d\n", hipGetErrorString(_e), \
              __FILE__, __LINE__);                                                  \
      return PRIO3_EDEVICE;                                                         \
    }                                                                               \
  } while (0)

struct Pending {
  prio3_engine* e;
  size_t idx;
  hipEvent_t a, b;
};
std::vector<Pending>& pending();
size_t time_slot(prio3_engine* e, const char* name);
void count_launch(prio3_engine* e, const char* name);
void collect_times(prio3_engine* e, bool wait = true);
#define TIMED(e, st, name, launch)                                   \
  do {                                                               \
    hipEvent_t _a = nullptr, _b = nullptr;                           \
    const bool _t = (e)->timing == 1 && hipEventCreate(&_a) == hipSuccess && \
                    hipEventCreate(&_b) == hipSuccess;               \
    if (_t) (void)hipEventRecord(_a, st);                            \
    launch;                                                          \
    HIPCHK(hipGetLastError());                                       \
    if (_t) {                                                        \
      (void)hipEventRecord(_b, st);                                  \
      pending().push_back(Pending{(e), time_slot(e, name), _a, _b}); \
    } else if ((e)->timing == 2) {                                   \
      count_launch((e), name);                                       \
    }                                                                \
  } while (0)

enum : unsigned {
  RUN_SCRATCH = 1,
  RUN_IO = 2,
  RUN_LINPUT = 8,
  RUN_FUSED = 16,
  RUN_AGG_IO = 32,
  RUN_HPKE = 64,
  RUN_JIX = 128,
};

static inline bool own_out(const DevParams& d) {
  return d.kind == PRIO3_SUM || d.kind == PRIO3_SUMVEC || d.kind == PRIO3_SUMVEC_F64_MP ||
         d.kind == PRIO3_FPVEC_BOUNDED_L2;
}
static inline const uint8_t* run_out_shares(const Run* R, uint32_t c0) {
  return (const uint8_t*)(own_out(R->dp) ? R->sc.out : R->sc.meas) + (size_t)R->dp.es * c0;
}

constexpr uint32_t WCH = 32;

struct PooledStream {
  int device;
  hipStream_t s;
  explicit PooledStream(int dev) : device(dev), s(ws_stream_get(dev)) {}
  ~PooledStream() { ws_stream_put(device, s); }
};

struct PullRanges {
  const uint8_t* src[4];
  uint8_t* dst[4];
  size_t bytes[4];
};
bool launch_pull(const PullRanges& pr, unsigned blocks, hipStream_t st);

bool fusable(const prio3_engine* e);
bool leader_fuse_takes(const prio3_engine* e);
bool leader_prep_takes(const prio3_engine* e);
int prepare_run(prio3_engine* e, Run* R, InPtrs in, OutPtrs out, hipStream_t st, bool fuse,
                bool allow_chunks, const PullRanges* pull = nullptr);
int leader_init_run(prio3_engine* e, Run* R, const uint8_t* d_nonces,
                    const uint8_t* d_public_shares, const uint8_t* d_leader_input_shares,
                    uint8_t* d_prep_shares, uint8_t* d_status, hipStream_t st,
                    const uint16_t* vk_slot = nullptr, const uint4* vk_tab = nullptr,
                    uint32_t lin_ld = 0);

int run_accumulate(prio3_engine* e, Run* R, uint32_t c0, uint32_t n, const uint8_t* d_status,
                   const uint32_t* d_seg, const uint8_t* d_accept, uint32_t nseg, uint8_t* d_agg,
                   uint64_t* d_counts, hipStream_t st);
int fused_finish(prio3_engine* e, Run* R, const uint8_t* d_status, const uint32_t* seg,
                 const uint32_t* fix_seg, const uint8_t* d_accept_mask, uint32_t S,
                 uint8_t* d_agg_shares, uint64_t* d_counts, hipStream_t st);
Slab* acc_multi_enqueue(int device, uint32_t es, uint8_t* host, const AccLayout& L,
                        uint32_t n_jobs, size_t out_bytes, hipStream_t st, int* rc);
int launch_combine(prio3_engine* e, uint32_t k, uint32_t n_segments, const uint8_t* d_in,
                   const uint64_t* d_counts_in, uint8_t* d_out, uint64_t* d_counts_out,
                   hipStream_t st);
int launch_batch_metadata(prio3_engine* e, uint32_t n, const uint8_t* d_report_ids,
                          const uint64_t* d_times, const uint8_t* d_status,
                          const uint8_t* d_accept_mask, const uint32_t* d_segment_ids,
                          uint32_t n_segments, uint32_t* ck, unsigned long long* iv,
                          hipStream_t st);
int launch_combine_metadata(prio3_engine* e, uint32_t k, uint32_t n_segments,
                            const uint32_t* ck_in, const unsigned long long* iv_in,
                            uint32_t* ck_out, unsigned long long* iv_out, hipStream_t st);

struct JixGroupArgs {
  const JixJobDesc* desc;
  const unsigned long long* closed;
  const uint8_t* ids;
  const unsigned long long* times;
  const uint8_t* accept;
  uint8_t* ids_dev;
  uint32_t* gseg;
  uint8_t* gaccept;
  uint32_t* seg_out;
  uint8_t *rej_out, *dup_out;
  unsigned long long* starts_out;
  prio3_job_index_info* info_out;
};
int launch_jix_group(prio3_engine* e, uint32_t n_jobs, const JixGroupArgs& a, hipStream_t st);

extern "C" int launch_leader_init(const DevParams& dp, const uint8_t* d_nonces,
                                  const uint8_t* d_pub, const uint8_t* d_lshares,
                                  const Scratch& sc, uint8_t* d_prep_shares, uint8_t* d_status,
                                  hipStream_t st, const uint16_t* vk_slot, const uint4* vk_tab);
extern "C" int launch_leader_next(const DevParams& dp, const uint8_t* d_prep_msgs,
                                  const Scratch& sc, uint8_t* d_status, hipStream_t st);
extern "C" int launch_leader_next_multi(uint32_t es, const LNextDesc* d_desc,
                                        const uint8_t* d_msgs, uint8_t* d_status, uint32_t n_jobs,
                                        uint32_t max_n, hipStream_t st);
```

### janus_amd/csrc/prio3_prepare.hip

```cpp
#include <hip/hip_runtime.h>

#include <algorithm>

#include "prio3_host.h"
#include "prio3_query_sum.h"

#ifndef XOFD_BLOCK
#define XOFD_BLOCK 256
#endif
#ifndef XOFD_OCC
#define XOFD_OCC 3
#endif
template <class F>
__device__ __forceinline__ void xof_body(const DevParams& p, const InPtrs& in, const Scratch& sc,
                                         const uint32_t r) {
  if (r >= p.n) return;
  constexpr uint32_t ES = F::ES;
  uint32_t flag = p.force_slow;
  uint32_t nonce[4], km[4], kp[4], kb[4] = {0, 0, 0, 0};
  load16(in.nonces + 16 * (size_t)r, nonce);
  const uint8_t* hs = in.helper + (size_t)r * p.helper_share_len;
  load16(hs, km);
  load16(hs + 16, kp);
  const bool JR = p.jr_len > 0;
  if (JR) load16(hs + 32, kb);

  {
    KState s;
    kzero(s);
    Msg m;
    msg_zero(m);
    msg_dst(m, p.dst[5]);
    {
      uint32_t vk[4];
      load_vk(p, in, r, vk);
      msg_bytes16(m, 9, vk);
    }
    msg_byte(m, 25, 1);
    msg_bytes16(m, 26, nonce);
    msg_absorb_final(s, m, 42);
    uint32_t q0 = 0, q1 = 0;
    squeeze_block<F>(p, s, 0, p.qr_len, q0, q1, sc.qr, r, flag);
  }

  KState ms;
  kzero(ms);
  {
    Msg m;
    msg_zero(m);
    msg_dst(m, p.dst[1]);
    msg_bytes16(m, 9, km);
    msg_byte(m, 25, 1);
    msg_absorb_final(ms, m, 26);
  }
  const uint32_t M = p.meas_len;
  const uint32_t mbytes = M * ES;
  const uint32_t K = (mbytes + 167) / 168;
  const uint32_t L = 42 + mbytes;
  const uint32_t B = L / 168, rem = L % 168;
  KState js;
  uint32_t pre[11], tail[11];
  uint32_t part[4] = {0, 0, 0, 0};
  if (JR) {
    kzero(js);
    Msg m;
    msg_zero(m);
    msg_dst(m, p.dst[7]);
    msg_bytes16(m, 9, kb);
    msg_byte(m, 25, 1);
    msg_bytes16(m, 26, nonce);
#pragma unroll
    for (int j = 0; j < 11; j++) pre[j] = m.w[j];
  }
#pragma unroll
  for (int j = 0; j < 11; j++) tail[j] = 0;
  uint32_t pend0 = 0, pend1 = 0;
  const uint32_t nb = JR ? B + 1 : K;
  for (uint32_t b = 0; b < nb; b++) {
    const bool hasW = b < K;
    if (hasW) squeeze_block<F>(p, ms, b, M, pend0, pend1, sc.meas, r, flag);
    if (JR && b < B) {
      const uint32_t w0 = hasW ? kword(ms, 0) : 0u;
#pragma unroll
      for (int j = 0; j < 10; j++)
        kxor_word(js, j, b == 0 ? pre[j] : __builtin_amdgcn_alignbit(tail[j + 1], tail[j], 16));
      kxor_word(js, 10, b == 0 ? ((pre[10] & 0xffffu) | (w0 << 16))
                               : __builtin_amdgcn_alignbit(w0, tail[10], 16));
#pragma unroll
      for (int j = 11; j < 42; j++)
        kxor_word(js, j, hasW ? __builtin_amdgcn_alignbit(kword(ms, j - 10), kword(ms, j - 11), 16)
                              : 0u);
      keccak_p12(js);
    } else if (JR) {
      uint32_t x[42];
#pragma unroll
      for (int j = 0; j < 10; j++)
        x[j] = b == 0 ? pre[j] : __builtin_amdgcn_alignbit(tail[j + 1], tail[j], 16);
      uint32_t w0 = hasW ? kword(ms, 0) : 0u;
      x[10] = b == 0 ? ((pre[10] & 0xffffu) | (w0 << 16))
                     : __builtin_amdgcn_alignbit(w0, tail[10], 16);
#pragma unroll
      for (int j = 11; j < 42; j++)
        x[j] = hasW ? __builtin_amdgcn_alignbit(kword(ms, j - 10), kword(ms, j - 11), 16) : 0u;
      {
#pragma unroll
        for (int j = 0; j < 42; j++) {
          const uint32_t lo = 4 * j;
          uint32_t mask = (lo + 4 <= rem) ? 0xffffffffu
                                          : (lo >= rem ? 0u : ((1u << (8 * (rem - lo))) - 1u));
          x[j] &= mask;
          if ((uint32_t)j == (rem >> 2)) x[j] ^= 1u << (8 * (rem & 3));
        }
        x[41] ^= 0x80000000u;
#pragma unroll
        for (int j = 0; j < 42; j++) kxor_word(js, j, x[j]);
        keccak_p12(js);
        part[0] = kword(js, 0);
        part[1] = kword(js, 1);
        part[2] = kword(js, 2);
        part[3] = kword(js, 3);
      }
    }
    if (hasW) {
#pragma unroll
      for (int t = 0; t < 11; t++) tail[t] = kword(ms, 31 + t);
    }
    if (b + 1 < K) keccak_p12(ms);
  }

  {
    KState s;
    kzero(s);
    Msg m;
    msg_zero(m);
    msg_dst(m, p.dst[2]);
    msg_bytes16(m, 9, kp);
    msg_byte(m, 25, 1);
    msg_byte(m, 26, 1);
    msg_absorb_final(s, m, 27);
    const uint32_t PL = p.proof_len;
    const uint32_t Kp = (PL * ES + 167) / 168;
    uint32_t q0 = 0, q1 = 0;
    for (uint32_t b = 0; b < Kp; b++) {
      squeeze_block<F>(p, s, b, PL, q0, q1, sc.proofs, r, flag);
      if (b + 1 < Kp) keccak_p12(s);
    }
  }

  if (JR) {
    uint32_t pub0[4];
    load16(in.pub + (size_t)r * p.public_share_len, pub0);
    KState s;
    kzero(s);
    Msg m;
    msg_zero(m);
    msg_dst(m, p.dst[6]);
    msg_bytes16(m, 25, pub0);
    msg_bytes16(m, 41, part);
    msg_absorb_final(s, m, 57);
    uint32_t cor[4] = {kword(s, 0), kword(s, 1), kword(s, 2), kword(s, 3)};
    KState t;
    kzero(t);
    Msg m2;
    msg_zero(m2);
    msg_dst(m2, p.dst[3]);
    msg_bytes16(m2, 9, cor);
    msg_byte(m2, 25, 1);
    msg_absorb_final(t, m2, 26);
    uint32_t q0 = 0, q1 = 0;
    squeeze_block<F>(p, t, 0, p.jr_len, q0, q1, sc.jr, r, flag);
    sc.part[r] = make_uint4(part[0], part[1], part[2], part[3]);
    sc.corrected[r] = make_uint4(cor[0], cor[1], cor[2], cor[3]);
  }
  sc.flag[r] = (uint8_t)flag;
}
template <class F>
__global__ __launch_bounds__(256, XOFD_OCC) void k_xof(DevParams p, InPtrs in, Scratch sc) {
  xof_body<F>(p, in, sc, blockIdx.x * blockDim.x + threadIdx.x);
}


template <bool FUSE, bool TR = false, bool PULL = false>
__device__ __forceinline__ void xofd_body(const DevParams& p, const InPtrs& in, const Scratch& sc,
                                          const uint32_t r) {
  typedef Fp128 F;
  const uint32_t lane = threadIdx.x & 63u;
  bool fuse = false, oor = false, haspad = false;
  uint32_t s0 = 0;
  if constexpr (FUSE) {
    const bool valid = r < p.n;
    const uint32_t sg = valid ? (sc.seg ? sc.seg[r] : 0u) : 0xffffffffu;
    const uint64_t inr = __ballot(valid && sg < p.nseg);
    s0 = inr ? (uint32_t)__shfl((int)sg, __ffsll((long long)inr) - 1) : 0xffffffffu;
    oor = valid && sg >= p.nseg;
    fuse = inr != 0 && __all(valid && (sg == s0 || sg >= p.nseg));
    haspad = __any(oor);
    if (lane == 0 && (r - lane) < p.n && !fuse) sc.wseg[r >> 6] = 0xffffffffu;
  }
  if (r >= p.n) return;
  uint32_t flag = p.force_slow;
  uint32_t nonce[4], km[4], kb[4];
  load16(in.nonces + 16 * (size_t)r, nonce);
  const uint8_t* hs = in.helper + (size_t)r * p.helper_share_len;
  load16(hs, km);
  load16(hs + 32, kb);
  {
    KState s;
    kzero(s);
    Msg m;
    msg_zero(m);
    msg_dst(m, p.dst[5]);
    {
      uint32_t vk[4];
      load_vk(p, in, r, vk);
      msg_bytes16(m, 9, vk);
    }
    msg_byte(m, 25, 1);
    msg_bytes16(m, 26, nonce);
    msg_absorb_final(s, m, 42);
    if (p.qr_len == 1) {
      uint32_t w[4] = {kword(s, 0), kword(s, 1), kword(s, 2), kword(s, 3)};
      put_elem<F>(p, sc.qr, 0, r, w, flag);
    } else {
      uint32_t q0 = 0, q1 = 0;
      squeeze_block<F>(p, s, 0, p.qr_len, q0, q1, sc.qr, r, flag);
    }
  }
  const uint32_t M = p.meas_len, K = (M * 16 + 167) / 168;
  const uint32_t L = 42 + M * 16, B = L / 168, rem = L % 168;
  KState ms, js;
  kzero(ms);
  kzero(js);
  {
    Msg m;
    msg_zero(m);
    msg_dst(m, p.dst[1]);
    msg_bytes16(m, 9, km);
    msg_byte(m, 25, 1);
    msg_absorb_final(ms, m, 26);
  }
  uint32_t pend0 = 0, pend1 = 0;
  TruncSink ts(p, sc.out, r);
  const int Mi = (int)M;
  uint4* tile = nullptr;
  if constexpr (FUSE) {
    __shared__ uint4 fuse_tiles[XOFD_BLOCK / 64][FTILE * 64];
    tile = fuse_tiles[__builtin_amdgcn_readfirstlane(threadIdx.x >> 6)];
  }
  uint32_t* const wrow =
      FUSE && !PULL ? sc.wpart + (size_t)__builtin_amdgcn_readfirstlane(r >> 6) * M * 8u
                    : nullptr;
  const uint32_t wlane = (lane & 7u) * 8u + (lane >> 3);
  auto mword = [&](int w) __attribute__((always_inline)) {
    return mk128(kword(ms, w), kword(ms, w + 1), kword(ms, w + 2), kword(ms, w + 3));
  };
  auto stage = [&](int e, int slot, f128 x) __attribute__((always_inline)) {
    if (e >= Mi) return;
    if (haspad && oor) x = zero128();
    tile_stage(tile, slot, lane, x);
  };
  auto flush = [&](int eb, int n) __attribute__((always_inline)) {
    const int cnt = min(n, Mi - eb);
    if (cnt <= 0) return;
    tile_fence();
    const uint32_t tot = tile_halfsum(tile, lane);
    if ((int)(lane & 7u) < cnt) {
      if constexpr (PULL) sc.wpart[((size_t)(r >> 6) * M + (uint32_t)eb) * 8u + wlane] = tot;
      else (wrow + (size_t)eb * 8u)[wlane] = tot;
    }
    tile_fence();
  };
  auto fuse_top = [&](uint32_t b, uint32_t q0, uint32_t q1) __attribute__((always_inline)) {
    const int e0 = 21 * (int)(b >> 1);
    if ((b & 1) == 0) {
      if (b) flush(e0 - 5, 5);
#pragma unroll
      for (int t = 0; t < 8; t++) stage(e0 + t, t, mword(4 * t));
    } else {
      stage(e0 + 10, 2, mk128(q0, q1, kword(ms, 0), kword(ms, 1)));
#pragma unroll
      for (int t = 0; t < 5; t++) stage(e0 + 11 + t, 3 + t, mword(2 + 4 * t));
    }
  };
  auto fuse_mid = [&](uint32_t b) __attribute__((always_inline)) {
    const int e0 = 21 * (int)(b >> 1);
    if ((b & 1) == 0) {
      flush(e0, 8);
      stage(e0 + 8, 0, mword(32));
      stage(e0 + 9, 1, mword(36));
    } else {
      flush(e0 + 8, 8);
#pragma unroll
      for (int t = 0; t < 5; t++) stage(e0 + 16 + t, t, mword(22 + 4 * t));
    }
  };
  auto fuse_tail = [&](uint32_t b) __attribute__((always_inline)) {
    const int e0 = 21 * (int)(b >> 1);
    if ((b & 1) == 0) flush(e0 + 8, 2);
    else flush(e0 + 16, 5);
  };
  auto wmask = [&](int j) __attribute__((always_inline)) {
    const uint32_t lo = 4u * (uint32_t)j;
    return (lo + 4 <= rem) ? 0xffffffffu : (lo >= rem ? 0u : ((1u << (8 * (rem - lo))) - 1u));
  };
  auto carry_tail = [&](bool last) __attribute__((always_inline)) {
#pragma unroll
    for (int j = 0; j < 10; j++) {
      uint32_t x = __builtin_amdgcn_alignbit(kword(ms, 32 + j), kword(ms, 31 + j), 16);
      if (last) x &= wmask(j);
      kxor_word(js, j, x);
    }
    uint32_t x = kword(ms, 41) >> 16;
    if (last) x &= wmask(10);
    kxor_word(js, 10, x);
  };
  {
    if (FUSE && fuse) fuse_top(0, 0, 0);
    squeeze_meas<TR>(p, ms, 0, M, pend0, pend1, sc.meas, r, flag, ts);
    Msg m;
    msg_zero(m);
    msg_dst(m, p.dst[7]);
    msg_bytes16(m, 9, kb);
    msg_byte(m, 25, 1);
    msg_bytes16(m, 26, nonce);
#pragma unroll
    for (int j = 0; j < 10; j++) kxor_word(js, j, m.w[j]);
    kxor_word(js, 10, (m.w[10] & 0xffffu) | (kword(ms, 0) << 16));
#pragma unroll
    for (int j = 11; j < 42; j++)
      kxor_word(js, j, __builtin_amdgcn_alignbit(kword(ms, j - 10), kword(ms, j - 11), 16));
    keccak_p12(js);
    if (FUSE && fuse) fuse_mid(0);
    carry_tail(B == 1);
    keccak_p12(ms);
  }
  if constexpr (PULL) {
    if (in.seg_dst) in.seg_dst[r] = in.seg_src[r];
    if (in.accept_dst) in.accept_dst[r] = in.accept_src[r];
  }
  const uint32_t Q = PULL ? p.prep_share_len / 16 : 0u;
  const size_t wbase = PULL ? (size_t)(r - lane) * (p.prep_share_len / 16) + lane : 0;
  const uint4* lsrc = PULL ? (const uint4*)in.leader_src + wbase : nullptr;
  uint4* ldst = PULL ? (uint4*)in.leader + wbase : nullptr;
#pragma unroll 1
  for (uint32_t b = 1; b < B; b++) {
    uint4 pc0, pc1;
    uint32_t q0 = 0, q1 = 0;
    if constexpr (PULL) {
      q0 = Q * (b - 1) / (B - 1);
      q1 = Q * b / (B - 1);
      if (q0 < q1) pc0 = lsrc[64 * (size_t)q0];
      if (q0 + 1 < q1) pc1 = lsrc[64 * (size_t)(q0 + 1)];
    }
    if (FUSE && fuse) fuse_top(b, pend0, pend1);
    squeeze_meas<TR>(p, ms, b, M, pend0, pend1, sc.meas, r, flag, ts);
    kxor_word(js, 10, kword(ms, 0) << 16);
#pragma unroll
    for (int j = 11; j < 42; j++)
      kxor_word(js, j, __builtin_amdgcn_alignbit(kword(ms, j - 10), kword(ms, j - 11), 16));
    keccak_p12(js);
    if (FUSE && fuse) fuse_mid(b);
    carry_tail(b + 1 == B);
    if (b + 1 < K) keccak_p12(ms);
    if constexpr (PULL) {
      if (q0 < q1) ldst[64 * (size_t)q0] = pc0;
      if (q0 + 1 < q1) ldst[64 * (size_t)(q0 + 1)] = pc1;
    }
  }
  uint32_t part[4];
  {
    const bool hasW = B < K;
    if (FUSE && fuse && hasW) fuse_top(B, pend0, pend1);
    if (hasW) squeeze_meas<TR>(p, ms, B, M, pend0, pend1, sc.meas, r, flag, ts);
#pragma unroll
    for (int j = 0; j < 42; j++) {
      uint32_t x = 0;
      if (j == 10) x = hasW ? kword(ms, 0) << 16 : 0u;
      else if (j > 10)
        x = hasW ? __builtin_amdgcn_alignbit(kword(ms, j - 10), kword(ms, j - 11), 16) : 0u;
      x &= wmask(j);
      if ((uint32_t)j == (rem >> 2)) x ^= 1u << (8 * (rem & 3));
      if (j == 41) x ^= 0x80000000u;
      kxor_word(js, j, x);
    }
    keccak_p12(js);
    if (FUSE && fuse) {
      if (hasW) fuse_mid(B);
      fuse_tail(hasW ? B : B - 1);
    }
    part[0] = kword(js, 0);
    part[1] = kword(js, 1);
    part[2] = kword(js, 2);
    part[3] = kword(js, 3);
  }
  {
    uint32_t kp[4];
    load16(hs + 16, kp);
    KState s;
    kzero(s);
    Msg m;
    msg_zero(m);
    msg_dst(m, p.dst[2]);
    msg_bytes16(m, 9, kp);
    msg_byte(m, 25, 1);
    msg_byte(m, 26, 1);
    msg_absorb_final(s, m, 27);
    const uint32_t PL = p.proof_len, Kp = (PL * 16 + 167) / 168;
    uint32_t q0 = 0, q1 = 0;
    for (uint32_t b = 0; b < Kp; b++) {
      squeeze_block<F>(p, s, b, PL, q0, q1, sc.proofs, r, flag);
      if (b + 1 < Kp) keccak_p12(s);
    }
  }
  {
    uint32_t pub0[4];
    load16(in.pub + (size_t)r * p.public_share_len, pub0);
    KState s;
    kzero(s);
    Msg m;
    msg_zero(m);
    msg_dst(m, p.dst[6]);
    msg_bytes16(m, 25, pub0);
    msg_bytes16(m, 41, part);
    msg_absorb_final(s, m, 57);
    uint32_t cor[4] = {kword(s, 0), kword(s, 1), kword(s, 2), kword(s, 3)};
    KState t;
    kzero(t);
    Msg m2;
    msg_zero(m2);
    msg_dst(m2, p.dst[3]);
    msg_bytes16(m2, 9, cor);
    msg_byte(m2, 25, 1);
    msg_absorb_final(t, m2, 26);
    uint32_t q0 = 0, q1 = 0;
    squeeze_block<F>(p, t, 0, p.jr_len, q0, q1, sc.jr, r, flag);
    sc.part[r] = make_uint4(part[0], part[1], part[2], part[3]);
    sc.corrected[r] = make_uint4(cor[0], cor[1], cor[2], cor[3]);
  }
  sc.flag[r] = (uint8_t)flag;
  if constexpr (FUSE) {
    if (fuse) {
      const bool anyflag = __any(flag != 0);
      if (lane == 0) sc.wseg[r >> 6] = anyflag ? 0xffffffffu : s0;
    }
  }
}
template <bool FUSE, bool TR = false>
__global__ __launch_bounds__(XOFD_BLOCK, XOFD_OCC) void k_xofd(DevParams p, InPtrs in, Scratch sc) {
  xofd_body<FUSE, TR>(p, in, sc, blockIdx.x * blockDim.x + threadIdx.x);
}


template <class F>
#ifndef XOF_OCC
#define XOF_OCC 4
#endif
#ifndef JR_OCC
#define JR_OCC 4
#endif
__global__ __launch_bounds__(256, XOF_OCC) void k_xof_a(DevParams p, InPtrs in, Scratch sc) {
  const uint32_t r = blockIdx.x * blockDim.x + threadIdx.x;
  if (r >= p.n) return;
  constexpr uint32_t ES = F::ES;
  uint32_t flag = p.force_slow;
  uint32_t nonce[4], km[4], kp[4];
  load16(in.nonces + 16 * (size_t)r, nonce);
  const uint8_t* hs = in.helper + (size_t)r * p.helper_share_len;
  load16(hs, km);
  load16(hs + 16, kp);
  {
    KState s;
    kzero(s);
    Msg m;
    msg_zero(m);
    msg_dst(m, p.dst[5]);
    {
      uint32_t vk[4];
      load_vk(p, in, r, vk);
      msg_bytes16(m, 9, vk);
    }
    msg_byte(m, 25, 1);
    msg_bytes16(m, 26, nonce);
    msg_absorb_final(s, m, 42);
    uint32_t w[4] = {kword(s, 0), kword(s, 1), kword(s, 2), kword(s, 3)};
    put_elem<F>(p, sc.qr, 0, r, w, flag);
  }
  {
    KState s;
    kzero(s);
    Msg m;
    msg_zero(m);
    msg_dst(m, p.dst[1]);
    msg_bytes16(m, 9, km);
    msg_byte(m, 25, 1);
    msg_absorb_final(s, m, 26);
    const uint32_t M = p.meas_len, K = (M * ES + 167) / 168;
    uint32_t q0 = 0, q1 = 0;
    for (uint32_t b = 0; b < K; b++) {
      squeeze_block<F>(p, s, b, M, q0, q1, sc.meas, r, flag);
      if (b + 1 < K) keccak_p12(s);
    }
  }
  {
    KState s;
    kzero(s);
    Msg m;
    msg_zero(m);
    msg_dst(m, p.dst[2]);
    msg_bytes16(m, 9, kp);
    msg_byte(m, 25, 1);
    msg_byte(m, 26, 1);
    msg_absorb_final(s, m, 27);
    const uint32_t PL = p.proof_len, Kp = (PL * ES + 167) / 168;
    uint32_t q0 = 0, q1 = 0;
    for (uint32_t b = 0; b < Kp; b++) {
      squeeze_block<F>(p, s, b, PL, q0, q1, sc.proofs, r, flag);
      if (b + 1 < Kp) keccak_p12(s);
    }
  }
  sc.flag[r] = (uint8_t)flag;
}

template <bool FUSE, bool LEADER = false>
__global__ __launch_bounds__(256, JR_OCC) void k_jrpart(DevParams p, InPtrs in, Scratch sc) {
  const uint32_t r = blockIdx.x * blockDim.x + threadIdx.x;
  const uint32_t lane = threadIdx.x & 63u;
  bool fuse = false;
  if constexpr (FUSE) {
    const bool valid = r < p.n;
    const uint32_t sg = valid ? (sc.seg ? sc.seg[r] : 0u) : 0xffffffffu;
    const uint32_t s0 = (uint32_t)__shfl((int)sg, 0);
    const bool flagged = valid && sc.flag[r];
    fuse = __all(valid && sg == s0 && sg < p.nseg && !flagged);
    if (lane == 0 && (r - lane) < p.n) sc.wseg[r >> 6] = fuse ? s0 : 0xffffffffu;
  }
  if (r >= p.n) return;
  const size_t ld = p.ld;
  const int M = (int)p.meas_len;
  uint32_t nonce[4], kb[4];
  load16(in.nonces + 16 * (size_t)r, nonce);
  if constexpr (LEADER)
    load16(in.helper + (size_t)r * p.leader_share_len + (size_t)(p.meas_len + p.proof_len) * 16, kb);
  else
    load16(in.helper + (size_t)r * p.helper_share_len + 32, kb);
  uint32_t pre[11];
  {
    Msg m;
    msg_zero(m);
    msg_dst(m, p.dst[7]);
    msg_bytes16(m, 9, kb);
    msg_byte(m, 25, LEADER ? 0 : 1);
    msg_bytes16(m, 26, nonce);
#pragma unroll
    for (int j = 0; j < 11; j++) pre[j] = m.w[j];
  }
  const uint4* meas = (const uint4*)sc.meas;
  auto ldel = [&](int e) -> uint4 {
    const bool ok = e >= 0 && e < M;
    uint4 v = meas[(size_t)(ok ? e : 0) * ld + r];
    return ok ? v : make_uint4(0, 0, 0, 0);
  };
  auto wsel = [](const uint4& v, int k) { return k == 0 ? v.x : k == 1 ? v.y : k == 2 ? v.z : v.w; };
  auto fused_pair = [&](int e0, const uint4& a, const uint4& b) {
    if (e0 + 1 < 0 || e0 >= M) return;
    const uint32_t tot = wave_halfsum2(mk128(a.x, a.y, a.z, a.w), mk128(b.x, b.y, b.z, b.w), lane);
    const int e = e0 + (int)(lane >> 5);
    if ((lane & 3u) == 0 && e >= 0 && e < M)
      sc.wpart[((size_t)(r >> 6) * (uint32_t)M + (uint32_t)e) * 8u + ((lane >> 2) & 7u)] = tot;
  };
  const uint32_t L = 42 + (uint32_t)M * 16;
  const uint32_t B = L / 168, rem = L % 168;
  KState s;
  kzero(s);
  for (uint32_t b = 0; b <= B; b++) {
    uint32_t x[42];
    const int q21 = 21 * (int)(b >> 1);
    if ((b & 1) == 0) {
      uint4 E[11];
#pragma unroll
      for (int t = 0; t < 11; t++) E[t] = ldel(q21 - 3 + t);
      if (FUSE && fuse) {
#pragma unroll
        for (int t = 1; t < 11; t += 2) fused_pair(q21 - 3 + t, E[t], E[t + 1]);
      }
#pragma unroll
      for (int j = 0; j < 42; j++) {
        const int u0 = j - 11 + 12, u1 = j - 10 + 12;
        const uint32_t w0 = wsel(E[u0 >> 2], u0 & 3), w1 = wsel(E[u1 >> 2], u1 & 3);
        x[j] = __builtin_amdgcn_alignbit(w1, w0, 16);
      }
      if (b == 0) {
#pragma unroll
        for (int j = 0; j < 10; j++) x[j] = pre[j];
        x[10] = (pre[10] & 0xffffu) | (wsel(E[3], 0) << 16);
      }
    } else {
      uint4 E[12];
#pragma unroll
      for (int t = 0; t < 12; t++) E[t] = ldel(q21 + 7 + t);
      if (FUSE && fuse) {
#pragma unroll
        for (int t = 1; t < 12; t += 2)
          fused_pair(q21 + 7 + t, E[t], t + 1 < 12 ? E[t + 1] : make_uint4(0, 0, 0, 0));
      }
#pragma unroll
      for (int j = 0; j < 42; j++) {
        const int u0 = j + 3, u1 = j + 4;
        const uint32_t w0 = wsel(E[u0 >> 2], u0 & 3), w1 = wsel(E[u1 >> 2], u1 & 3);
        x[j] = __builtin_amdgcn_alignbit(w1, w0, 16);
      }
    }
    if (b == B) {
#pragma unroll
      for (int j = 0; j < 42; j++) {
        const uint32_t lo = 4 * j;
        uint32_t mask = (lo + 4 <= rem) ? 0xffffffffu
                                        : (lo >= rem ? 0u : ((1u << (8 * (rem - lo))) - 1u));
        x[j] &= mask;
        if ((uint32_t)j == (rem >> 2)) x[j] ^= 1u << (8 * (rem & 3));
      }
      x[41] ^= 0x80000000u;
    }
#pragma unroll
    for (int j = 0; j < 42; j++) kxor_word(s, j, x[j]);
    keccak_p12(s);
  }
  uint32_t part[4] = {kword(s, 0), kword(s, 1), kword(s, 2), kword(s, 3)};
  uint32_t flag = sc.flag[r];
  uint32_t pub0[4];
  load16(in.pub + (size_t)r * p.public_share_len + (LEADER ? 16 : 0), pub0);
  KState c;
  kzero(c);
  {
    Msg m;
    msg_zero(m);
    msg_dst(m, p.dst[6]);
    msg_bytes16(m, 25, LEADER ? part : pub0);
    msg_bytes16(m, 41, LEADER ? pub0 : part);
    msg_absorb_final(c, m, 57);
  }
  uint32_t cor[4] = {kword(c, 0), kword(c, 1), kword(c, 2), kword(c, 3)};
  {
    KState t;
    kzero(t);
    Msg m2;
    msg_zero(m2);
    msg_dst(m2, p.dst[3]);
    msg_bytes16(m2, 9, cor);
    msg_byte(m2, 25, 1);
    msg_absorb_final(t, m2, 26);
    uint32_t q0 = 0, q1 = 0;
    squeeze_block<Fp128>(p, t, 0, p.jr_len, q0, q1, sc.jr, r, flag);
  }
  sc.part[r] = make_uint4(part[0], part[1], part[2], part[3]);
  sc.corrected[r] = make_uint4(cor[0], cor[1], cor[2], cor[3]);
  sc.flag[r] = (uint8_t)flag;
}


__global__ __launch_bounds__(256) void k_leader_unpack(DevParams p, InPtrs in, Scratch sc,
                                                       uint8_t* status, uint32_t* wpart,
                                                       uint32_t* wseg) {
  typedef Fp128 F;
  constexpr int RB = 64, CE = 32;
  __shared__ uint4 tile[RB][CE + 1];
  __shared__ uint32_t bad[RB];
  const uint32_t tid = threadIdx.x, r0 = blockIdx.x * RB;
  const size_t ld = p.ld;
  const uint32_t M = p.meas_len, PL = p.proof_len, E = M + PL;
  const uint32_t nrep = min((uint32_t)RB, p.n - r0);
  if (tid < RB) bad[tid] = 0;
  for (uint32_t c0 = 0; c0 < E; c0 += CE) {
    __syncthreads();
#pragma unroll
    for (int i = 0; i < RB * CE / 256; i++) {
      const uint32_t idx = tid + 256 * i, rr = idx / CE, e = c0 + idx % CE;
      if (rr < nrep && e < E) {
        const uint4 v =
            ((const uint4*)(in.helper + (size_t)(r0 + rr) * p.leader_share_len))[e];
        if (!F::lt_p(mk128(v.x, v.y, v.z, v.w))) atomicOr(&bad[rr], 1u);
        tile[rr][idx % CE] = v;
      }
    }
    __syncthreads();
#pragma unroll
    for (int i = 0; i < RB * CE / 256; i++) {
      const uint32_t idx = tid + 256 * i, rr = idx % RB, el = idx / RB, e = c0 + el;
      if (rr < nrep && e < E) {
        if (e < M)
          ((uint4*)sc.meas)[(size_t)e * ld + r0 + rr] = tile[rr][el];
        else
          ((uint4*)sc.proofs)[(size_t)(e - M) * ld + r0 + rr] = tile[rr][el];
      }
    }
    if (wpart && nrep == RB && c0 < M) {
      const uint32_t el = tid >> 3, h = tid & 7u, e = c0 + el;
      if (e < M) {
        uint32_t sum = 0;
#pragma unroll 8
        for (uint32_t rr = 0; rr < RB; rr++) {
          const uint32_t* w = (const uint32_t*)&tile[rr][el];
          sum += (w[h >> 1] >> ((h & 1u) * 16u)) & 0xffffu;
        }
        wpart[((size_t)blockIdx.x * M + e) * 8u + h] = sum;
      }
    }
  }
  __syncthreads();
  if (tid >= nrep) return;
  const uint32_t r = r0 + tid;
  uint32_t flag = p.force_slow;
  uint32_t nonce[4];
  load16(in.nonces + 16 * (size_t)r, nonce);
  KState s;
  kzero(s);
  Msg m;
  msg_zero(m);
  msg_dst(m, p.dst[5]);
  {
    uint32_t vk[4];
    load_vk(p, in, r, vk);
    msg_bytes16(m, 9, vk);
  }
  msg_byte(m, 25, 1);
  msg_bytes16(m, 26, nonce);
  msg_absorb_final(s, m, 42);
  uint32_t w[4] = {kword(s, 0), kword(s, 1), kword(s, 2), kword(s, 3)};
  put_elem<F>(p, sc.qr, 0, r, w, flag);
  if (p.qr_len > 1) {
    uint32_t w1[4] = {kword(s, 4), kword(s, 5), kword(s, 6), kword(s, 7)};
    put_elem<F>(p, sc.qr, 1, r, w1, flag);
  }
  sc.flag[r] = (uint8_t)flag;
  status[r] = bad[tid] ? PRIO3_STATUS_INPUT_SHARE_DECODE : PRIO3_STATUS_FINISHED;
  if (wseg) {
    const bool fuse = nrep == RB && __all(!bad[tid]);
    if (tid == 0) wseg[blockIdx.x] = fuse ? 0u : 0xffffffffu;
  }
}

DEV void leader_jr_body(const DevParams& p, const InPtrs& in, const Scratch& sc,
                        uint8_t* status, uint32_t* wpart, uint32_t* wseg, const uint32_t r) {
// ... 636 lines not shown
  const uint32_t A = p.arity, C = p.chunk, M = p.meas_len, K = p.calls;
  uint8_t status = LEADER ? out.status[r] : PRIO3_STATUS_FINISHED;
  uint8_t* lout = LEADER ? out.prep_msgs + (size_t)r * p.prep_share_len : nullptr;
  const T t = ldf<F>(sc.qr, 0, ld, r);
  T sumL = F::zero();
  auto store_L = [&](int idx, const T& val) {
    const uint32_t c = (uint32_t)((PP - idx) & (PP - 1));
    if (c == 0) {
      F::store(sc.Lbuf, r, val);
    } else if (c <= K) {
      F::store(sc.Lbuf, (size_t)c * ld + r, val);
      sumL = F::add(sumL, val);
    }
  };
  if constexpr (PP <= 16) {
    T x[PP];
    T pw = FC<F>::invP(p);
#pragma unroll
    for (int e = 0; e < PP; e++) {
      x[__builtin_bitreverse32(e) >> (32 - LOGP)] = pw;
      pw = F::mul(pw, t);
    }
    if (F::eq(pw, FC<F>::invP(p))) status = PRIO3_STATUS_PREP_INIT;
    dft_reg<PP, LOGP>(p, x, 1);
#pragma unroll
    for (int k = 0; k < PP; k++) store_L(k, x[k]);
  } else {
    static_assert(PP == 32, "PP must be <= 32");
    T t8 = t;
#pragma unroll
    for (int i = 0; i < 3; i++) t8 = F::mul(t8, t8);
    const T t16 = F::mul(t8, t8);
    const T t32 = F::mul(t16, t16);
    if (F::eq(t32, F::one())) status = PRIO3_STATUS_PREP_INIT;
    const T ip = FC<F>::invP(p);
    const T a = F::add(F::one(), t16), b = F::sub(F::one(), t16);
    const T c = F::mul(t8, a), wd = F::mul(F::mul(t8, b), F::from_words(p.tw128[8]));
#pragma unroll
    for (int ph = 0; ph < 4; ph++) {
      const T g = ph == 0 ? F::add(a, c) : ph == 1 ? F::add(b, wd) : ph == 2 ? F::sub(a, c)
                                                                              : F::sub(b, wd);
      T x[8];
      T pw = F::mul(ip, g);
      const T ratio = ph == 0 ? t : F::mul(t, F::from_words(p.tw128[ph]));
#pragma unroll
      for (int e = 0; e < 8; e++) {
        x[__builtin_bitreverse32(e) >> 29] = pw;
        if (e + 1 < 8) pw = F::mul(pw, ratio);
      }
      dft_reg<8, 3>(p, x, 4);
#pragma unroll
      for (int k = 0; k < 8; k++) store_L(4 * k + ph, x[k]);
    }
  }
  T pt = F::zero(), range;
  {
    constexpr int GLEN = 2 * (PP - 1) + 1, NB = (GLEN + 7) / 8;
    T pw[8];
    pw[0] = F::one();
    pw[1] = t;
#pragma unroll
    for (int i = 2; i < 8; i++) pw[i] = F::mul(pw[i - 1], t);
    const T t8b = F::mul(pw[7], t);
    mac128 R;
    mac_zero(R);
    auto ldc = [&](int e) { return ldf<F>(sc.proofs, A + (e < GLEN ? e : 0), ld, r); };
    T cb[8];
#pragma unroll
    for (int i = 0; i < 8; i++) cb[i] = ldc(8 * (NB - 1) + i);
#pragma unroll 1
    for (int q = NB - 1; q >= 0; q--) {
      T cn[8];
      const int qn = q > 0 ? q - 1 : 0;
#pragma unroll
      for (int i = 0; i < 8; i++) cn[i] = ldc(8 * qn + i);
      mac128 S;
      mac_zero(S);
#pragma unroll
      for (int i = 0; i < 8; i++) {
        const int e = 8 * q + i;
        if (e < GLEN) {
          mac_add(S, cb[i], pw[i]);
          mac_add(R, cb[i], F::from_words(p.sigma128[e & (PP - 1)]));
        }
        cb[i] = cn[i];
      }
      const T sq = mac_reduce_f(S);
      pt = q == NB - 1 ? sq : F::add(F::mul(pt, t8b), sq);
    }
    range = mac_reduce_f(R);
  }
  F::store(sc.PVbuf, (size_t)1 * ld + r, pt);
  F::store(sc.PVbuf, (size_t)2 * ld + r, range);
  const T r0 = ldf<F>(sc.jr, 0, ld, r);
  {
    T rC = F::one(), sq = r0;
    for (uint32_t e = C; e; e >>= 1) {
      if (e & 1) rC = F::mul(rC, sq);
      if (e > 1) sq = F::mul(sq, sq);
    }
    T rk = F::one();
    for (uint32_t k0 = 0; k0 < K; k0 += 8) {
      T lb[8];
#pragma unroll
      for (int q = 0; q < 8; q++) lb[q] = ldf<F>(sc.Lbuf, k0 + q < K ? k0 + q + 1 : 1, ld, r);
#pragma unroll
      for (int q = 0; q < 8; q++) {
        if (k0 + q < K) {
          F::store(sc.beta, (size_t)(k0 + q) * ld + r, F::mul(lb[q], rk));
          rk = F::mul(rk, rC);
        }
      }
    }
  }
  const T half = FC<F>::half(p);
  F::store(sc.PVbuf, r, F::mul(half, sumL));
  const uint8_t* lps = in.leader + (size_t)r * p.prep_share_len;
  bool decode_ok = true;
  auto lv = [&](uint32_t e) {
    T x = F::load(lps, e);
    if (!F::lt_p(x)) decode_ok = false;
    return x;
  };
  sum128 Ssum;
  sum_zero(Ssum);
  T G = F::zero(), rj = r0;
  uint64_t lane = (uint64_t)sc.meas + (uint64_t)r * F::ES;
  asm("" : "+v"(lane));
  for (uint32_t jg = 0; jg < C; jg += GS) {
    mac128 Aa[GS], Bb[GS];
#pragma unroll
    for (int q = 0; q < GS; q++) {
      mac_zero(Aa[q]);
      mac_zero(Bb[q]);
    }
    constexpr int WIRE_AHEAD = 1;
    struct wire_ops {
      T m[GS];
      T be, L;
    };
    auto ldrow = [&](const void* base, uint32_t e) {
      const uint64_t off = ((uint64_t)base - (uint64_t)sc.meas) + (uint64_t)e * ld * F::ES;
      const uint64_t offu =
          ((uint64_t)(uint32_t)__builtin_amdgcn_readfirstlane((int)(uint32_t)(off >> 32)) << 32) |
          (uint32_t)__builtin_amdgcn_readfirstlane((int)(uint32_t)off);
      typedef uint32_t u32x4 __attribute__((ext_vector_type(4)));
      const u32x4 v = *(const __attribute__((address_space(1))) u32x4*)(lane + offu);
      return mk128(v.x, v.y, v.z, v.w);
    };
    const uint32_t Klast = K ? K - 1 : 0;
    auto issue = [&](uint32_t k, wire_ops& s) {
#pragma unroll
      for (int q = 0; q < GS; q++) {
        const uint32_t i = k * C + jg + q;
        const bool valid = (k < K) && (jg + q < C) && (i < M);
        s.m[q] = ldrow(sc.meas, i & (valid ? 0xffffffffu : 0u));
      }
      const uint32_t kc = min(k, Klast);
      s.be = ldrow(sc.beta, kc);
      s.L = ldrow(sc.Lbuf, kc + 1);
    };
    auto use = [&](uint32_t k, wire_ops& s) {
#pragma unroll
      for (int q = 0; q < GS; q++)
        asm volatile(""
                     : "+v"(s.m[q].w[0]), "+v"(s.m[q].w[1]), "+v"(s.m[q].w[2]), "+v"(s.m[q].w[3])
                     :
                     : "memory");
#pragma unroll
      for (int q = 0; q < GS; q++) {
        const bool valid = (jg + q < C) && (k * C + jg + q < M);
        const uint32_t msk = valid ? 0xffffffffu : 0u;
        const T mc = mk128(s.m[q].w[0] & msk, s.m[q].w[1] & msk, s.m[q].w[2] & msk,
                           s.m[q].w[3] & msk);
        mac_add(Aa[q], s.be, mc);
        mac_add(Bb[q], s.L, mc);
        sum_add(Ssum, mc);
      }
    };
    constexpr int NS = WIRE_AHEAD + 1;
    wire_ops ws[NS];
    uint32_t k = __builtin_amdgcn_readfirstlane(0);
    asm volatile("" : "+s"(k));
#pragma unroll
    for (int u = 0; u < WIRE_AHEAD; u++) issue(k + u, ws[u]);
#pragma unroll 1
    for (uint32_t e = K % NS; e; e--, k++) {
      issue(k + WIRE_AHEAD, ws[WIRE_AHEAD]);
      use(k, ws[0]);
#pragma unroll
      for (int u = 0; u < WIRE_AHEAD; u++) ws[u] = ws[u + 1];
    }
#pragma unroll 1
    for (; k < K; k += NS) {
#pragma unroll
      for (int u = 0; u < NS; u++) {
        issue(k + u + WIRE_AHEAD, ws[(u + WIRE_AHEAD) % NS]);
        use(k + u, ws[u]);
      }
    }
    T sd[2 * GS], lw[2 * GS], r0f;
    auto fin_load = [&](int q) {
      const uint32_t jc = jg + q < C ? jg + q : jg;
      if constexpr (!LEADER) {
        lw[2 * q] = F::load(lps, 1 + 2 * jc);
        lw[2 * q + 1] = F::load(lps, 2 + 2 * jc);
      }
    };
    const T L0 = ldrow(sc.Lbuf, 0), halfL = ldrow(sc.PVbuf, 0);
#pragma unroll
    for (int q = 0; q < GS; q++) {
      const uint32_t jc = jg + q < C ? jg + q : jg;
      sd[2 * q + 1] = ldrow(sc.proofs, 2 * jc + 1);
      sd[2 * q] = ldrow(sc.proofs, 2 * jc);
    }
    fin_load(0);
    asm volatile("" ::: "memory");
    mac128 Gq;
    mac_zero(Gq);
#pragma unroll
    for (int q = 0; q < GS; q++) {
      const uint32_t j = jg + q;
      if (q == 0 || j < C) {
        mac_add(Bb[q], sd[2 * q + 1], L0);
        T f1 = F::sub(mac_reduce_f(Bb[q]), halfL);
        if (q == 0) {
          asm volatile("" : "+v"(f1.w[0])::"memory");
          r0f = ldrow(sc.jr, 0);
#pragma unroll
          for (int q2 = 1; q2 < GS; q2++) fin_load(q2);
          asm volatile("" ::: "memory");
        }
        const T Aq = mac_reduce_f(Aa[q]);
        mac128 F0;
        mac_zero(F0);
        mac_add(F0, sd[2 * q], L0);
        mac_add(F0, rj, Aq);
        const T f0 = mac_reduce_f(F0);
        if constexpr (LEADER) {
          F::store(lout, 1 + 2 * j, f0);
          F::store(lout, 2 + 2 * j, f1);
        } else {
          if (!F::lt_p(lw[2 * q]) || !F::lt_p(lw[2 * q + 1])) decode_ok = false;
          mac_add(Gq, F::add(lw[2 * q], f0), F::add(lw[2 * q + 1], f1));
        }
        rj = F::mul(rj, r0f);
      }
    }
    if constexpr (!LEADER) G = F::add(G, mac_reduce_f(Gq));
  }
  const T S = sum_reduce(Ssum);
  pt = ldf<F>(sc.PVbuf, 1, ld, r);
  range = ldf<F>(sc.PVbuf, 2, ld, r);
  T v;
  if (p.kind == PRIO3_SUMVEC) {
    v = range;
  } else {
    const T r1 = ldf<F>(sc.jr, 1, ld, r);
    v = F::add(F::mul(r1, range), F::mul(F::mul(r1, r1), F::sub(S, half)));
  }
  if constexpr (LEADER) {
    F::store(lout, 0, v);
    F::store(lout, A + 1, pt);
    *(uint4*)(lout + (size_t)p.verifier_len * F::ES) = sc.part[r];
    out.status[r] = status;
  } else {
  const T V0 = F::add(lv(0), v);
  const T PT = F::add(lv(A + 1), pt);
  if (status == PRIO3_STATUS_FINISHED) {
    if (!decode_ok)
      status = PRIO3_STATUS_PREP_SHARE_DECODE;
    else if (!F::is_zero(V0) || !F::eq(G, PT))
      status = PRIO3_STATUS_PREP_MSG;
  }
  uint32_t lpart[4], msg[4];
  load16(lps + (size_t)p.verifier_len * F::ES, lpart);
  if (!prep_msg_check(p, in, sc, r, lpart, msg) && status == PRIO3_STATUS_FINISHED)
    status = PRIO3_STATUS_PREP_NEXT;
  if (status != PRIO3_STATUS_FINISHED) msg[0] = msg[1] = msg[2] = msg[3] = 0;
  ((uint4*)out.prep_msgs)[r] = make_uint4(msg[0], msg[1], msg[2], msg[3]);
  out.status[r] = status;
  }
  if (p.kind == PRIO3_SUMVEC) {
    for (uint32_t e = 0; e < p.out_len; e++) {
      T acc = F::zero(), pw = F::one();
      for (uint32_t b = 0; b < p.bits; b++) {
        acc = F::add(acc, F::mul(pw, ldf<F>(sc.meas, e * p.bits + b, ld, r)));
        pw = F::add(pw, pw);
      }
      F::store(sc.out, (size_t)e * ld + r, acc);
    }
  }
}
template <int GS, int PP, int LEADER = 0>
__global__ __launch_bounds__(256, 3) void k_query_h(DevParams p, InPtrs in, Scratch sc,
                                                  OutPtrs out) {
  query_h_body<GS, PP, LEADER>(p, in, sc, out, blockIdx.x * blockDim.x + threadIdx.x);
}

template <bool FUSE, bool PULL = false>
__global__ __launch_bounds__(XOFD_BLOCK, 3) void k_prep_h(DevParams p, InPtrs in, Scratch sc,
                                                   OutPtrs out) {
  const uint32_t r = blockIdx.x * blockDim.x + threadIdx.x;
  xofd_body<FUSE, false, PULL>(p, in, sc, r);
  query_h_body<2, 32>(p, in, sc, out, r);
}

template <int PP>
__global__ __launch_bounds__(256, 3) void k_leader_prep(DevParams p, InPtrs in, Scratch sc,
                                                        OutPtrs out, uint32_t* wpart,
                                                        uint32_t* wseg) {
  const uint32_t r = blockIdx.x * blockDim.x + threadIdx.x;
  leader_jr_body(p, in, sc, out.status, wpart, wseg, r);
  query_h_body<2, PP, 1>(p, in, sc, out, r);
}

template <int NPH>
__global__ __launch_bounds__(256, 3) void k_prep_sum(DevParams p, InPtrs in, Scratch sc,
                                                     OutPtrs out) {
  const uint32_t r = blockIdx.x * blockDim.x + threadIdx.x;
  xofd_body<false, false>(p, in, sc, r);
  qsum::query_sum_body<NPH, 0>(p, in, sc, out, r);
}

template <int PP>
__global__ __launch_bounds__(64) void k_slow_redo(DevParams p, InPtrs in, Scratch sc, OutPtrs out) {
  const uint32_t r0 = (blockIdx.x * blockDim.x + threadIdx.x) * REDO_RPL;
  if (r0 >= p.n || !redo_any(p, sc, r0)) return;
  const uint8_t* fl = sc.flag + r0;
  for (uint32_t i = 0; i < REDO_RPL && r0 + i < p.n; i++)
    if (fl[i]) {
      xof_slow_one<Fp128>(p, in, sc, r0 + i);
      query_h_body<2, PP>(p, in, sc, out, r0 + i);
    }
}

template <int NPH>
__global__ __launch_bounds__(64) void k_slow_redo_sum(DevParams p, InPtrs in, Scratch sc,
                                                      OutPtrs out) {
  const uint32_t r0 = (blockIdx.x * blockDim.x + threadIdx.x) * REDO_RPL;
  if (r0 >= p.n || !redo_any(p, sc, r0)) return;
  const uint8_t* fl = sc.flag + r0;
  for (uint32_t i = 0; i < REDO_RPL && r0 + i < p.n; i++)
    if (fl[i]) {
      xof_slow_one<Fp128>(p, in, sc, r0 + i);
      qsum::query_sum_body<NPH, 0>(p, in, sc, out, r0 + i);
    }
}


static void fp_sub_sizes(const prio3_engine* e, uint32_t n, uint32_t cap, bool wide,
                         uint32_t& nsub, uint32_t& sub) {
  nsub = (n + cap - 1) / cap;
  sub = std::min(cap, (((n + nsub - 1) / nsub) + 255) & ~255u);
  if (wide && e->fp_round && nsub > 1) {
    const uint32_t Q = (uint32_t)e->n_cu * 4u * 2u * 8u;
    const uint32_t s2 = sub / Q * Q;
    if (s2 > 0 && n - (nsub - 1) * s2 <= cap) sub = s2;
  }
}

template <class F>
static void launch_xof_slow(const prio3_engine* e, const DevParams& p, const InPtrs& in,
                            const Scratch& sc, hipStream_t st) {
  (void)e;
  k_xof_slow<F><<<slow_blocks(p.n), 64, 0, st>>>(p, in, sc);
}

bool fusable(const prio3_engine* e) {
  return e->fuse_acc && e->dp.kind == PRIO3_HISTOGRAM && e->dp.jr_len &&
         (42 + e->dp.meas_len * 16) / 168 >= 2;
}

static int ensure_side_streams(prio3_engine* e) {
  while (e->side.size() < 2) {
    hipStream_t s2;
    hipEvent_t j;
    HIPCHK(hipStreamCreateWithFlags(&s2, hipStreamNonBlocking));
    HIPCHK(hipEventCreateWithFlags(&j, hipEventDisableTiming));
    e->side.push_back(s2);
    e->side_ev.push_back(j);
  }
  if (!e->fork_ev) HIPCHK(hipEventCreateWithFlags(&e->fork_ev, hipEventDisableTiming));
  return PRIO3_OK;
}

static bool prep_fused_takes(const prio3_engine* e, const DevParams& dp, bool fuse) {
  if (e->force_generic) return false;
  const bool ps = dp.kind == PRIO3_HISTOGRAM || dp.kind == PRIO3_SUMVEC;
  const bool dual = dp.es == 16 && dp.jr_len && (42 + dp.meas_len * 16) / 168 >= 2;
  if (dp.kind == PRIO3_SUM) return dual && !fuse && query_sum_takes(dp);
  return ps && dual && dp.P == 32;
}

enum : int { DEFER_NONE = 0, DEFER_QH = 1, DEFER_SUM = 2, DEFER_GEN64 = 3 };
static int launch_prepare(prio3_engine* e, const DevParams& base, uint32_t c0, uint32_t n,
                          InPtrs in, OutPtrs out, Scratch sc, hipStream_t st, bool fuse,
                          int* deferred, bool pair = false) {
  DevParams dp = base;
  dp.n = n;
  dp.force_slow = (uint32_t)e->force_slow;
  dp.slow_defer = 0;
  dp.redo = 0;
  const size_t es = dp.es;
  in.nonces += 16 * (size_t)c0;
  if (in.pub) in.pub += (size_t)dp.public_share_len * c0;
  in.helper += (size_t)dp.helper_share_len * c0;
  in.leader += (size_t)dp.prep_share_len * c0;
  if (in.vk_slot) in.vk_slot += c0;
  out.prep_msgs += (size_t)(dp.kind == PRIO3_SUMVEC_F64_MP ? 32 : 16) * c0;
  out.status += c0;
  void** soa[] = {&sc.meas, &sc.proofs, &sc.jr, &sc.qr, &sc.Lbuf, &sc.PVbuf, &sc.acc, &sc.out,
                  &sc.beta};
  for (auto q : soa)
    if (*q) *q = (uint8_t*)*q + es * c0;
  sc.part += c0;
  sc.corrected += c0;
  sc.flag += c0;
  if (sc.seg) sc.seg += c0;
  if (sc.wseg) sc.wseg += c0 / 64;
  if (sc.wpart) sc.wpart += (size_t)(c0 / 64) * dp.meas_len * 8;
  const uint32_t blocks = (n + 255) / 256;
  const uint32_t xblocks = (n + XOFD_BLOCK - 1) / XOFD_BLOCK;
  if (dp.kind == PRIO3_SUMVEC_F64_MP) {
    int rc = PRIO3_OK;
    TIMED(e, st, "k_mp64_prepare", (rc = launch_mp64(e, n, dp.ld, in, out, sc, st)));
    return rc;
  }
  if (dp.kind == PRIO3_FPVEC_BOUNDED_L2) {
    uint32_t nsub, sub;
    const bool qwide = !e->force_generic && fpvec_query_wide_takes(dp);
    fp_sub_sizes(e, n, dp.ld, qwide, nsub, sub);
    for (uint32_t si = 0; si < nsub; si++) {
      const uint32_t s0 = si * sub;
      DevParams q = dp;
      q.n = si + 1 < nsub ? sub : n - s0;
      InPtrs qi = in;
      qi.nonces += 16 * (size_t)s0;
      qi.pub += (size_t)dp.public_share_len * s0;
      qi.helper += (size_t)dp.helper_share_len * s0;
      qi.leader += (size_t)dp.prep_share_len * s0;
      if (qi.vk_slot) qi.vk_slot += s0;
      OutPtrs qo = out;
      qo.prep_msgs += 16 * (size_t)s0;
      qo.status += s0;
      Scratch qs = sc;
      qs.out = (uint8_t*)sc.out + es * s0;
      const uint32_t qb = (q.n + 255) / 256;
      const bool dual = (42 + dp.meas_len * 16) / 168 >= 2;
      q.trunc_xof = dual ? 1u : 0u;
      bool paired = false;
      if (dual) TIMED(e, st, "k_xof_pair", (paired = launch_xof_pair(q, qi, qs, st)));
      if (!paired && dual)
        TIMED(e, st, "k_xofd",
              (k_xofd<false, true><<<(q.n + XOFD_BLOCK - 1) / XOFD_BLOCK, XOFD_BLOCK, 0, st>>>(
                  q, qi, qs)));
      else if (!paired)
        TIMED(e, st, "k_xof", (k_xof<Fp128><<<qb, 256, 0, st>>>(q, qi, qs)));
      TIMED(e, st, "k_xof_slow", launch_xof_slow<Fp128>(e, q, qi, qs, st));
      if (qwide)
        TIMED(e, st, "k_query_fpw", launch_fpvec_query(q, qi, qs, qo, st, true, false));
      else
        TIMED(e, st, "k_query_fp", launch_fpvec_query(q, qi, qs, qo, st, false, false));
    }
    return PRIO3_OK;
  }
  if (dp.es == 16) {
    const bool ps = dp.kind == PRIO3_HISTOGRAM || dp.kind == PRIO3_SUMVEC;
    const bool wide = ps && !e->force_generic && dp.P != 32 && query_wide_takes(dp);
    const bool dual = dp.jr_len && (42 + dp.meas_len * 16) / 168 >= 2;
    dp.trunc_xof = dp.kind == PRIO3_SUMVEC && wide && dual && !fuse ? 1u : 0u;
    if (prep_fused_takes(e, dp, fuse)) {
      dp.slow_defer = 1u;
      if (dp.kind == PRIO3_SUM) {
        if (deferred) *deferred = DEFER_SUM;
        switch (dp.P) {
          case 16: TIMED(e, st, "k_prep_sum", (k_prep_sum<1><<<blocks, 256, 0, st>>>(dp, in, sc, out))); break;
          case 32: TIMED(e, st, "k_prep_sum", (k_prep_sum<2><<<blocks, 256, 0, st>>>(dp, in, sc, out))); break;
          case 64: TIMED(e, st, "k_prep_sum", (k_prep_sum<4><<<blocks, 256, 0, st>>>(dp, in, sc, out))); break;
          default: TIMED(e, st, "k_prep_sum", (k_prep_sum<8><<<blocks, 256, 0, st>>>(dp, in, sc, out))); break;
        }
      } else {
        if (deferred) *deferred = DEFER_QH;
        const bool pl = in.leader_src != nullptr;
        bool paired = false;
        if (pair)
          TIMED(e, st, "k_prep_hp", (paired = launch_prep_pair(dp, in, sc, out, st, fuse, pl)));
        if (paired) {
        } else if (fuse && pl)
          TIMED(e, st, "k_prep_h", (k_prep_h<true, true><<<xblocks, XOFD_BLOCK, 0, st>>>(dp, in, sc, out)));
        else if (fuse)
          TIMED(e, st, "k_prep_h", (k_prep_h<true><<<xblocks, XOFD_BLOCK, 0, st>>>(dp, in, sc, out)));
        else if (pl)
          TIMED(e, st, "k_prep_h", (k_prep_h<false, true><<<xblocks, XOFD_BLOCK, 0, st>>>(dp, in, sc, out)));
        else
          TIMED(e, st, "k_prep_h", (k_prep_h<false><<<xblocks, XOFD_BLOCK, 0, st>>>(dp, in, sc, out)));
      }
      return PRIO3_OK;
    }
    if (dual) {
      if (fuse)
        TIMED(e, st, "k_xofd", (k_xofd<true><<<xblocks, XOFD_BLOCK, 0, st>>>(dp, in, sc)));
      else if (dp.trunc_xof)
        TIMED(e, st, "k_xofd", (k_xofd<false, true><<<xblocks, XOFD_BLOCK, 0, st>>>(dp, in, sc)));
      else
        TIMED(e, st, "k_xofd", (k_xofd<false><<<xblocks, XOFD_BLOCK, 0, st>>>(dp, in, sc)));
    } else {
      TIMED(e, st, "k_xof_a", (k_xof_a<Fp128><<<blocks, 256, 0, st>>>(dp, in, sc)));
      TIMED(e, st, "k_jrpart", (k_jrpart<false><<<blocks, 256, 0, st>>>(dp, in, sc)));
    }
    const bool qh_path =
        ps && !e->force_generic && !wide && (dp.P == 32 || dp.P == 16 || dp.P == 8);
    dp.slow_defer = qh_path ? 1u : 0u;
    if (qh_path && deferred) *deferred = DEFER_QH;
    if (!qh_path) TIMED(e, st, "k_xof_slow", launch_xof_slow<Fp128>(e, dp, in, sc, st));
    bool done = false;
    if (wide) TIMED(e, st, "k_query_w", (done = launch_query_wide(dp, in, sc, out, st)));
    if (done) {
    } else if (qh_path && dp.P == 32)
      TIMED(e, st, "k_query_h", (k_query_h<2, 32><<<blocks, 256, 0, st>>>(dp, in, sc, out)));
    else if (qh_path && dp.P == 16)
      TIMED(e, st, "k_query_h", (k_query_h<2, 16><<<blocks, 256, 0, st>>>(dp, in, sc, out)));
    else if (qh_path && dp.P == 8)
      TIMED(e, st, "k_query_h", (k_query_h<2, 8><<<blocks, 256, 0, st>>>(dp, in, sc, out)));
    else if (ps)
      TIMED(e, st, "k_query_ps", (k_query_ps<4><<<blocks, 256, 0, st>>>(dp, in, sc, out)));
    else {
      bool qs = false;
      if (!e->force_generic && query_sum_takes(dp))
        TIMED(e, st, "k_query_sum", (qs = launch_query_sum(dp, in, sc, out, st)));
      if (!qs) TIMED(e, st, "k_query", (k_query<Fp128><<<blocks, 256, 0, st>>>(dp, in, sc, out)));
    }
  } else {
    dp.slow_defer = 1u;
    if (deferred) *deferred = DEFER_GEN64;
    TIMED(e, st, "k_prep_gen", (k_prep_gen<Fp64><<<blocks, 256, 0, st>>>(dp, in, sc, out)));
  }
  return PRIO3_OK;
}

static int launch_slow_redo(prio3_engine* e, const DevParams& base, uint32_t n, InPtrs in,
                            OutPtrs out, Scratch sc, hipStream_t st, int family) {
  DevParams dp = base;
  dp.n = n;
  dp.force_slow = (uint32_t)e->force_slow;
  dp.trunc_xof = 0;
  dp.slow_defer = 1;
  dp.redo = 1;
  const uint32_t g = redo_blocks(n);
  if (family == DEFER_GEN64) {
    TIMED(e, st, "k_slow_redo", (k_slow_redo_gen<Fp64><<<g, 64, 0, st>>>(dp, in, sc, out)));
  } else if (family == DEFER_SUM) {
    switch (dp.P) {
      case 16: TIMED(e, st, "k_slow_redo", (k_slow_redo_sum<1><<<g, 64, 0, st>>>(dp, in, sc, out))); break;
      case 32: TIMED(e, st, "k_slow_redo", (k_slow_redo_sum<2><<<g, 64, 0, st>>>(dp, in, sc, out))); break;
      case 64: TIMED(e, st, "k_slow_redo", (k_slow_redo_sum<4><<<g, 64, 0, st>>>(dp, in, sc, out))); break;
      default: TIMED(e, st, "k_slow_redo", (k_slow_redo_sum<8><<<g, 64, 0, st>>>(dp, in, sc, out))); break;
    }
  } else if (dp.P == 32)
    TIMED(e, st, "k_slow_redo", (k_slow_redo<32><<<g, 64, 0, st>>>(dp, in, sc, out)));
  else if (dp.P == 16)
    TIMED(e, st, "k_slow_redo", (k_slow_redo<16><<<g, 64, 0, st>>>(dp, in, sc, out)));
  else
    TIMED(e, st, "k_slow_redo", (k_slow_redo<8><<<g, 64, 0, st>>>(dp, in, sc, out)));
  return PRIO3_OK;
}

static bool pulls_in_xof(const prio3_engine* e, const DevParams& dp, bool fuse, uint32_t n) {
  const uint32_t B = (42 + dp.meas_len * 16) / 168;
  return prep_fused_takes(e, dp, fuse) && dp.kind != PRIO3_SUM && dp.prep_share_len % 16 == 0 &&
         B >= 2 && dp.prep_share_len / 16 <= 2 * (B - 1) && n % 64 == 0;
}

static bool pair_takes(const prio3_engine* e, const DevParams& base, uint32_t n, bool fuse,
                       bool pulling) {
  if (e->pair_max <= 0 || n == 0 || n > (uint32_t)e->pair_max || !prep_fused_takes(e, base, fuse))
    return false;
  DevParams d = base;
  d.n = n;
  return prep_pair_takes(d, pulling);
}

int prepare_run(prio3_engine* e, Run* R, InPtrs in, OutPtrs out, hipStream_t st, bool fuse,
                bool allow_chunks, const PullRanges* pull) {
  const uint32_t n = R->n;
  if (pull && pulls_in_xof(e, R->dp, fuse, n)) {
    in.leader_src = pull->src[0];
    in.seg_src = (const uint32_t*)pull->src[1];
    in.seg_dst = (uint32_t*)pull->dst[1];
    in.accept_src = pull->src[2];
    in.accept_dst = pull->dst[2];
    allow_chunks = false;
  } else if (pull) {
    if (!launch_pull(*pull, 256, st)) return PRIO3_EDEVICE;
  }
  Scratch sc = R->sc;
  sc.seg = R->seg;
  sc.wpart = R->wpart;
  sc.wseg = R->wseg;
  R->last = st;
  const bool pair = pair_takes(e, R->dp, n, fuse, in.leader_src != nullptr);
  R->wshift = pair ? 5u : 6u;
  const uint32_t K = e->chunks > 0 ? (uint32_t)e->chunks
                     : (prep_fused_takes(e, R->dp, fuse) || R->dp.kind == PRIO3_SUMVEC_F64_MP)
                         ? 1u
                         : std::max(1u, (n + (1u << 16)) >> 17);
  const uint32_t csz = ((n + K - 1) / K + 255) & ~255u;
  int deferred = DEFER_NONE;
  if (pair || !allow_chunks || K == 1 || n <= csz || R->dp.kind == PRIO3_FPVEC_BOUNDED_L2) {
    const int rc = launch_prepare(e, R->dp, 0, n, in, out, sc, st, fuse, &deferred, pair);
    if (rc == PRIO3_OK && deferred)
      return launch_slow_redo(e, R->dp, n, in, out, sc, st, deferred);
    return rc;
  }
  int rc = ensure_side_streams(e);
  if (rc) return rc;
  HIPCHK(hipEventRecord(e->fork_ev, st));
  for (auto s2 : e->side) HIPCHK(hipStreamWaitEvent(s2, e->fork_ev, 0));
  uint32_t c = 0;
  for (uint32_t c0 = 0; c0 < n; c0 += csz, c++) {
    rc = launch_prepare(e, R->dp, c0, std::min(csz, n - c0), in, out, sc, e->side[c % 2], fuse,
                        &deferred);
    if (rc) return rc;
  }
  for (size_t i = 0; i < e->side.size(); i++) {
    HIPCHK(hipEventRecord(e->side_ev[i], e->side[i]));
    HIPCHK(hipStreamWaitEvent(st, e->side_ev[i], 0));
  }
  if (deferred) return launch_slow_redo(e, R->dp, n, in, out, sc, st, deferred);
  return PRIO3_OK;
}

static int leader_init_fpvec(prio3_engine* e, Run* R, const uint8_t* d_nonces,
                             const uint8_t* d_pub, const uint8_t* d_lin, uint8_t* d_prep_shares,
                             uint8_t* d_status, hipStream_t st) {
  DevParams dp = R->dp;
  dp.force_slow = (uint32_t)e->force_slow;
  dp.trunc_xof = 0;
  if (!fpvec_query_wide_takes(dp) || !R->corr_all) return PRIO3_EUNSUPPORTED;
  const uint32_t n = R->n, cap = dp.ld;
  uint32_t nsub, sub;
  fp_sub_sizes(e, n, cap, true, nsub, sub);
  const size_t es = dp.es;
  for (uint32_t si = 0; si < nsub; si++) {
    const uint32_t s0 = si * sub;
    DevParams q = dp;
    q.n = si + 1 < nsub ? sub : n - s0;
    InPtrs qi{d_nonces + 16 * (size_t)s0,
              d_pub ? d_pub + (size_t)dp.public_share_len * s0 : nullptr,
              d_lin + (size_t)dp.leader_share_len * s0, nullptr};
    OutPtrs qo{d_prep_shares + (size_t)dp.prep_share_len * s0, d_status + s0};
    Scratch qs = R->sc;
    qs.out = (uint8_t*)R->sc.out + es * s0;
    const uint32_t blocks = (q.n + 255) / 256, blocks64 = (q.n + 63) / 64;
    TIMED(e, st, "k_leader_unpack",
          (k_leader_unpack<<<(q.n + 63) / 64, 256, 0, st>>>(q, qi, qs, qo.status, nullptr, nullptr)));
    TIMED(e, st, "k_jrpart", (k_jrpart<false, true><<<blocks, 256, 0, st>>>(q, qi, qs)));
    TIMED(e, st, "k_leader_slowfix", (k_leader_slowfix<<<blocks64, 64, 0, st>>>(q, qi, qs)));
    TIMED(e, st, "k_query_fpw", launch_fpvec_query(q, qi, qs, qo, st, true, true));
    HIPCHK(hipMemcpyAsync(R->corr_all + s0, qs.corrected, 16 * (size_t)q.n,
                          hipMemcpyDeviceToDevice, st));
  }
  return PRIO3_OK;
}

bool leader_prep_takes(const prio3_engine* e) {
  const DevParams& dp = e->dp;
  return e->leader_fast && (dp.kind == PRIO3_HISTOGRAM || dp.kind == PRIO3_SUMVEC) && dp.jr_len &&
         (dp.P == 32 || dp.P == 16 || dp.P == 8) &&
         dp.leader_share_len == 16 * (dp.meas_len + dp.proof_len + 1);
}

int leader_init_run(prio3_engine* e, Run* R, const uint8_t* d_nonces,
                    const uint8_t* d_public_shares, const uint8_t* d_leader_input_shares,
                    uint8_t* d_prep_shares, uint8_t* d_status, hipStream_t st,
                    const uint16_t* vk_slot, const uint4* vk_tab, uint32_t lin_ld) {
  DevParams dp = R->dp;
  dp.force_slow = (uint32_t)e->force_slow;
  const uint32_t n = R->n;
  R->last = st;
  if (dp.kind == PRIO3_FPVEC_BOUNDED_L2)
    return leader_init_fpvec(e, R, d_nonces, d_public_shares, d_leader_input_shares,
                             d_prep_shares, d_status, st);
  if (dp.kind == PRIO3_SUMVEC_F64_MP) {
    int rc = PRIO3_OK;
    TIMED(e, st, "k_mp64_prepare",
          (rc = launch_mp64_leader(e, n, dp.ld, InPtrs{d_nonces, d_public_shares,
                                                       d_leader_input_shares, nullptr},
                                   OutPtrs{d_prep_shares, d_status}, R->sc, st)));
    return rc;
  }
  const bool ps = dp.kind == PRIO3_HISTOGRAM || dp.kind == PRIO3_SUMVEC;
  if (ps && dp.jr_len && (dp.P == 32 || dp.P == 16 || dp.P == 8) && e->leader_fast) {
    InPtrs in{d_nonces, d_public_shares, d_leader_input_shares, nullptr};
    in.vk_slot = vk_slot;
    in.vk_tab = vk_tab;
    in.lin_ld = lin_ld;
    OutPtrs out{d_prep_shares, d_status};
    const uint32_t blocks = (n + 255) / 256, blocks64 = (n + 63) / 64;
    uint32_t* wp = R->lfused ? R->wpart : nullptr;
    uint32_t* wsg = R->lfused ? R->wseg : nullptr;
    DevParams d1 = dp;
    d1.slow_defer = 1;
    if (dp.P == 32)
      TIMED(e, st, "k_leader_prep",
            (k_leader_prep<32><<<blocks, 256, 0, st>>>(d1, in, R->sc, out, wp, wsg)));
    else if (dp.P == 16)
      TIMED(e, st, "k_leader_prep",
            (k_leader_prep<16><<<blocks, 256, 0, st>>>(d1, in, R->sc, out, wp, wsg)));
    else
      TIMED(e, st, "k_leader_prep",
            (k_leader_prep<8><<<blocks, 256, 0, st>>>(d1, in, R->sc, out, wp, wsg)));
    dp.redo = 1;
    TIMED(e, st, "k_leader_slowfix",
          (k_leader_slowfix<<<blocks64, 64, 0, st>>>(dp, in, R->sc)));
    if (dp.P == 32)
      TIMED(e, st, "k_query_h", (k_query_h<2, 32, 1><<<blocks, 256, 0, st>>>(dp, in, R->sc, out)));
    else if (dp.P == 16)
      TIMED(e, st, "k_query_h", (k_query_h<2, 16, 1><<<blocks, 256, 0, st>>>(dp, in, R->sc, out)));
    else
      TIMED(e, st, "k_query_h", (k_query_h<2, 8, 1><<<blocks, 256, 0, st>>>(dp, in, R->sc, out)));
    return PRIO3_OK;
  }
  if (dp.kind == PRIO3_SUM && e->leader_fast && query_sum_takes(dp)) {
    InPtrs in{d_nonces, d_public_shares, d_leader_input_shares, nullptr};
    in.vk_slot = vk_slot;
    in.vk_tab = vk_tab;
    OutPtrs out{d_prep_shares, d_status};
    const uint32_t blocks = (n + 255) / 256, blocks64 = (n + 63) / 64;
    TIMED(e, st, "k_leader_unpack",
          (k_leader_unpack<<<(n + 63) / 64, 256, 0, st>>>(dp, in, R->sc, d_status, nullptr,
                                                         nullptr)));
    TIMED(e, st, "k_jrpart", (k_jrpart<false, true><<<blocks, 256, 0, st>>>(dp, in, R->sc)));
    TIMED(e, st, "k_leader_slowfix",
          (k_leader_slowfix<<<blocks64, 64, 0, st>>>(dp, in, R->sc)));
    bool ok = false;
    TIMED(e, st, "k_query_sum", (ok = launch_query_sum(dp, in, R->sc, out, st, true)));
    return ok ? PRIO3_OK : PRIO3_EDEVICE;
  }
  int rc2 = PRIO3_OK;
  TIMED(e, st, "k_leader_init",
        rc2 = launch_leader_init(dp, d_nonces, d_public_shares, d_leader_input_shares, R->sc,
                                 d_prep_shares, d_status, st, vk_slot, vk_tab));
  return rc2;
}

bool leader_fuse_takes(const prio3_engine* e) {
  const DevParams& d = e->dp;
  return e->leader_fuse_acc && e->leader_fast && d.jr_len && d.kind == PRIO3_HISTOGRAM &&
         (d.P == 32 || d.P == 16 || d.P == 8) && !own_out(d) && d.es == 16;
}
```

Baseline: 179.7 million reports/s.

## Fuse aggregation kernels, compact redo list, self-clean accumulators, single-pass meta reduce

Merges the aggregation fix-up and wave-reduction kernels into one launch with block roles. The prepare kernel now builds a compacted list of flagged reports, so the slow-redo pass touches only those instead of scanning every report. The slow-redo kernel also zeroes the next run's scratch, and the final kernels reset their accumulators, which removes separate zeroing launches. The meta kernel does its cross-block reduction in one pass using a last-block ticket. The cost is more complex cross-kernel invariants, atomics and a host mutex on the shared zero words.

```diff
diff --git a/janus_amd/csrc/prio3_accumulate.hip b/janus_amd/csrc/prio3_accumulate.hip
--- a/janus_amd/csrc/prio3_accumulate.hip
+++ b/janus_amd/csrc/prio3_accumulate.hip
@@ -1,28 +1,15 @@
 #include <hip/hip_runtime.h>
 
 #include <algorithm>
+#include <mutex>
 #include <type_traits>
+#include <vector>
 
 #include "prio3_host.h"
 #include "sha256_device.h"
 
-struct ZeroRanges {
-  uint8_t* dst[4];
-  size_t bytes[4];
-};
 __global__ __launch_bounds__(256) void k_zero(ZeroRanges z) {
-  const size_t tid = blockIdx.x * (size_t)blockDim.x + threadIdx.x, nth = (size_t)gridDim.x * blockDim.x;
-#pragma unroll
-  for (int k = 0; k < 4; k++) {
-    uint8_t* d = z.dst[k];
-    const size_t n = z.bytes[k];
-    if (!d || !n) continue;
-    const size_t head = std::min(n, (size_t)((16 - ((uintptr_t)d & 15)) & 15));
-    const size_t n16 = (n - head) / 16;
-    for (size_t i = tid; i < n16; i += nth) ((uint4*)(d + head))[i] = make_uint4(0, 0, 0, 0);
-    for (size_t i = tid * 4; i < head; i += nth * 4) *(uint32_t*)(d + i) = 0u;
-    for (size_t i = head + 16 * n16 + tid * 4; i < n; i += nth * 4) *(uint32_t*)(d + i) = 0u;
-  }
+  zero_ranges(z, blockIdx.x * (size_t)blockDim.x + threadIdx.x, (size_t)gridDim.x * blockDim.x);
 }
 
 
@@ -190,18 +177,18 @@
   }
 }
 
-__global__ __launch_bounds__(256) void k_agg_waves(uint32_t nwaves, uint32_t M,
-                                                   const uint32_t* wpart, const uint32_t* wseg,
-                                                   unsigned long long* cpart, uint32_t* cseg,
-                                                   unsigned long long* agg64) {
+__device__ __forceinline__ void agg_waves_role(uint32_t bx, uint32_t c, uint32_t nwaves,
+                                               uint32_t M, const uint32_t* wpart,
+                                               const uint32_t* wseg, unsigned long long* cpart,
+                                               uint32_t* cseg, unsigned long long* agg64) {
   static_assert(WCH <= 64, "one chunk's wave segments are read by one wave");
-  const uint32_t slot = 4 * (blockIdx.x * blockDim.x + threadIdx.x), c = blockIdx.y;
+  const uint32_t slot = 4 * (bx * blockDim.x + threadIdx.x);
   const uint32_t w0 = c * WCH, w1 = min(nwaves, w0 + WCH), lane = threadIdx.x & 63u;
   const uint32_t my = w0 + lane < w1 ? wseg[w0 + lane] : 0xffffffffu;
   const uint64_t fused = __ballot(my != 0xffffffffu);
   const uint32_t s0 = fused ? (uint32_t)__shfl((int)my, __ffsll((long long)fused) - 1) : 0xffffffffu;
   const bool mixed = __any(my != 0xffffffffu && my != s0);
-  if (slot == 0 && blockIdx.x == 0) cseg[c] = mixed ? 0xffffffffu : s0;
+  if (slot == 0) cseg[c] = mixed ? 0xffffffffu : s0;
   if (s0 == 0xffffffffu) return;
   const bool act = slot < M * 8;
   const uint32_t ls = act ? slot : 0u;
@@ -252,13 +239,25 @@
 }
 
 constexpr uint32_t FIX_T = 64;
-static uint32_t fix_per(uint32_t n) { return n >= (1u << 18) ? 4096u : 512u; }
-__global__ __launch_bounds__(256) void k_agg_fix(uint32_t n, const uint8_t* status,
-                                                 const uint32_t* seg, const uint8_t* accept,
-                                                 const uint32_t* wseg, uint32_t* fix,
-                                                 uint32_t fix_cap, uint32_t nseg,
-                                                 unsigned long long* counts, uint32_t oor_masked,
-                                                 uint32_t per, uint32_t wshift) {
+static uint32_t fix_per(uint32_t n) { return n >= (1u << 18) ? 1024u : 512u; }
+struct AggFixArgs {
+  uint32_t n;
+  const uint8_t* status;
+  const uint32_t* seg;
+  const uint8_t* accept;
+  uint32_t *fix, *ents;
+  uint32_t fix_cap, nseg;
+  unsigned long long* counts;
+  uint32_t oor_masked, per, wshift;
+};
+__device__ __forceinline__ void agg_fix_role(uint32_t blk, const AggFixArgs& a,
+                                             const uint32_t* wseg) {
+  const uint32_t n = a.n, nseg = a.nseg, wshift = a.wshift, oor_masked = a.oor_masked;
+  const uint32_t fix_cap = a.fix_cap, per = a.per;
+  const uint8_t *status = a.status, *accept = a.accept;
+  const uint32_t* seg = a.seg;
+  uint32_t *fix = a.fix, *ents = a.ents;
+  unsigned long long* counts = a.counts;
   __shared__ uint32_t tseg[FIX_T];
   __shared__ unsigned int tcnt[FIX_T];
   if (threadIdx.x < FIX_T) {
@@ -266,7 +265,7 @@
     tcnt[threadIdx.x] = 0;
   }
   __syncthreads();
-  const uint32_t lo = blockIdx.x * per, hi = min(n, lo + per);
+  const uint32_t lo = blk * per, hi = min(n, lo + per);
   for (uint32_t base = lo; base < hi; base += 256) {
     const uint32_t r = base + threadIdx.x;
     const bool valid = r < hi;
@@ -289,8 +288,8 @@
       add(sg, 1u);
     }
     if (valid && fused != inc) {
-      const uint32_t i = atomicAdd(&fix[0], 1u);
-      if (i < fix_cap) fix[1 + i] = r | (inc ? 0u : 0x80000000u);
+      const uint32_t i = atomicAdd(fix, 1u);
+      if (i < fix_cap) ents[i] = r | (inc ? 0u : 0x80000000u);
     }
   }
   __syncthreads();
@@ -298,14 +297,34 @@
     atomicAdd(&counts[tseg[threadIdx.x]], (unsigned long long)tcnt[threadIdx.x]);
 }
 
+__global__ __launch_bounds__(256) void k_agg_parts(uint32_t fix_blocks, uint32_t gx, AggFixArgs fa,
+                                                   uint32_t nwaves, uint32_t M,
+                                                   const uint32_t* wpart, const uint32_t* wseg,
+                                                   unsigned long long* cpart, uint32_t* cseg,
+                                                   unsigned long long* agg64) {
+  if (blockIdx.x < fix_blocks) {
+    agg_fix_role(blockIdx.x, fa, wseg);
+    return;
+  }
+  const uint32_t b = blockIdx.x - fix_blocks;
+  agg_waves_role(b % gx, b / gx, nwaves, M, wpart, wseg, cpart, cseg, agg64);
+}
+
 DEV f128 fold_halves_impl(const unsigned long long (&Hs)[8]);
 DEV f128 fold_halves(const unsigned long long (&Hs)[8]) { return fold_halves_impl(Hs); }
 
+struct AggFinalArgs {
+  const uint32_t* nfix;
+  const uint32_t* ents;
+  uint32_t* next;
+  unsigned long long* fcnt;
+  unsigned long long* counts;
+};
 __global__ __launch_bounds__(256) void k_agg_final(uint32_t M, size_t ld,
-                                                   const unsigned long long* agg64,
+                                                   unsigned long long* agg64,
                                                    uint32_t nchunks,
                                                    const unsigned long long* cpart,
-                                                   const uint32_t* cseg, const uint32_t* fix,
+                                                   const uint32_t* cseg, AggFinalArgs fa,
                                                    const uint32_t* seg, const void* meas,
                                                    uint8_t* agg) {
   const uint32_t idx = blockIdx.x, s = idx / M, e = idx % M;
@@ -317,9 +336,9 @@
     if (cseg[c] == s) acc += cpart[((size_t)c * M + e) * 8 + h];
   red[tid] = acc;
   f128 ad = zero128(), sb = zero128();
-  const uint32_t nfix = fix[0];
+  const uint32_t nfix = *fa.nfix;
   for (uint32_t i = tid; i < nfix; i += 256) {
-    const uint32_t ent = fix[1 + i], r = ent & 0x7fffffffu;
+    const uint32_t ent = fa.ents[i], r = ent & 0x7fffffffu;
     if ((seg ? seg[r] : 0u) != s) continue;
     const f128 x = Fp128::load(meas, (size_t)e * ld + r);
     if (ent & 0x80000000u) sb = add128(sb, x);
@@ -332,7 +351,7 @@
     if (tid < st) red[tid] += red[tid + st];
     __syncthreads();
   }
-  for (uint32_t st = 128; st >= 1; st >>= 1) {
+  for (uint32_t st = nfix ? 128 : 0; st >= 1; st >>= 1) {
     if (tid < st) {
       fadd[tid] = add128(fadd[tid], fadd[tid + st]);
       fsub[tid] = add128(fsub[tid], fsub[tid + st]);
@@ -341,28 +360,45 @@
   }
   if (tid != 0) return;
   unsigned long long Hs[8];
-  for (int hh = 0; hh < 8; hh++) Hs[hh] = red[hh] + agg64[(size_t)idx * 8 + hh];
+  for (int hh = 0; hh < 8; hh++) {
+    Hs[hh] = red[hh] + agg64[(size_t)idx * 8 + hh];
+    agg64[(size_t)idx * 8 + hh] = 0;
+  }
+  if (e == 0) {
+    fa.counts[s] = fa.fcnt[s];
+    fa.fcnt[s] = 0;
+  }
+  if (idx == 0) *fa.next = 0;
   Fp128::store(agg, idx, sub128(add128(fold_halves(Hs), fadd[0]), fsub[0]));
 }
 
 __global__ __launch_bounds__(256) void k_agg_final_s(uint32_t M, size_t ld,
-                                                     const unsigned long long* agg64,
+                                                     unsigned long long* agg64,
                                                      uint32_t nchunks,
                                                      const unsigned long long* cpart,
-                                                     const uint32_t* cseg, const uint32_t* fix,
+                                                     const uint32_t* cseg, AggFinalArgs fa,
                                                      const uint32_t* seg, const void* meas,
                                                      uint8_t* agg) {
   const uint32_t s = blockIdx.y, tid = threadIdx.x, h = tid & 7u, lane = tid & 63u;
   const uint32_t e = blockIdx.x * 32u + (tid >> 3);
   const bool live = e < M;
   const uint32_t ec = live ? e : 0u;
-  unsigned long long H = agg64[((size_t)s * M + ec) * 8 + h];
+  unsigned long long H = 0;
+  if (live) {
+    H = agg64[((size_t)s * M + e) * 8 + h];
+    agg64[((size_t)s * M + e) * 8 + h] = 0;
+  }
+  if (blockIdx.x == 0 && tid == 0) {
+    fa.counts[s] = fa.fcnt[s];
+    fa.fcnt[s] = 0;
+    if (s == 0) *fa.next = 0;
+  }
   for (uint32_t c = 0; c < nchunks; c++)
     if (cseg[c] == s) H += cpart[((size_t)c * M + ec) * 8 + h];
   f128 ad = zero128(), sb = zero128();
-  const uint32_t nfix = fix[0];
+  const uint32_t nfix = *fa.nfix;
   for (uint32_t i = h; i < nfix; i += 8) {
-    const uint32_t ent = fix[1 + i], r = ent & 0x7fffffffu;
+    const uint32_t ent = fa.ents[i], r = ent & 0x7fffffffu;
     if ((seg ? seg[r] : 0u) != s) continue;
     const f128 x = Fp128::load(meas, (size_t)ec * ld + r);
     if (ent & 0x80000000u) sb = add128(sb, x);
@@ -459,10 +495,11 @@
 }
 
 constexpr uint32_t META_T = 1024, META_W = META_T / 64, META_BLOCKS = 512;
-__global__ __launch_bounds__(1024) void k_meta(uint32_t n, const uint8_t* ids, const uint64_t* times,
-                                             const uint8_t* status, const uint8_t* mask,
-                                             const uint32_t* seg, uint32_t n_segments, uint32_t* ck,
-                                             unsigned long long* iv) {
+__global__ __launch_bounds__(1024) void k_meta_seg(uint32_t n, const uint8_t* ids,
+                                                 const uint64_t* times,
+                                                 const uint8_t* status, const uint8_t* mask,
+                                                 const uint32_t* seg, uint32_t n_segments,
+                                                 uint32_t* ck, unsigned long long* iv) {
   __shared__ uint32_t s_seg0;
   __shared__ uint32_t s_ck[META_W][8];
   __shared__ unsigned long long s_lo[META_W], s_hi[META_W];
@@ -544,6 +581,157 @@
     __syncthreads();
   }
   flush();
+}
+
+constexpr uint32_t META_FAST_SEGS = 8;
+struct MetaRow {
+  uint32_t ck[8];
+  unsigned long long lo, hi;
+};
+constexpr uint32_t META_COLS = 10;
+__global__ __launch_bounds__(1024) void k_meta(uint32_t n, const uint8_t* ids,
+                                             const uint64_t* times, const uint8_t* status,
+                                             const uint8_t* mask, const uint32_t* seg,
+                                             uint32_t n_segments, uint32_t* ck,
+                                             unsigned long long* iv, MetaRow* rows,
+                                             uint32_t* ticket) {
+  __shared__ uint32_t s_seg0;
+  __shared__ uint32_t s_ck[META_W][8];
+  __shared__ unsigned long long s_lo[META_W], s_hi[META_W];
+  __shared__ uint32_t t_ck[META_FAST_SEGS][8];
+  __shared__ unsigned long long t_lo[META_FAST_SEGS], t_hi[META_FAST_SEGS];
+  __shared__ unsigned long long s_red[META_T];
+  __shared__ unsigned long long s_fin[8][META_FAST_SEGS * META_COLS];
+  const uint32_t tid = threadIdx.x, lane = tid & 63u, wv = tid >> 6;
+  if (tid < META_FAST_SEGS * 8) t_ck[tid >> 3][tid & 7u] = 0;
+  if (tid < META_FAST_SEGS) {
+    t_lo[tid] = ~0ull;
+    t_hi[tid] = 0;
+  }
+  __syncthreads();
+  for (uint32_t base = blockIdx.x * META_T; base < n; base += gridDim.x * META_T) {
+    const uint32_t r = base + tid;
+    const bool valid = r < n;
+    const uint32_t sg = valid ? (seg ? seg[r] : 0u) : 0xffffffffu;
+    const bool in_range = valid && sg < n_segments;
+    const bool inc = in_range && status[r] == PRIO3_STATUS_FINISHED && (!mask || mask[r]);
+    uint32_t h[8] = {0, 0, 0, 0, 0, 0, 0, 0};
+    if (ck && inc) {
+      uint32_t id[4];
+      load16(ids + 16 * (size_t)r, id);
+      sha256_id16(id, h);
+    }
+    unsigned long long lo = ~0ull, hi = 0;
+    if (times && in_range) {
+      lo = times[r];
+      hi = lo + 1;
+    }
+    if (tid == 0) s_seg0 = sg;
+    __syncthreads();
+    const bool uniform = __syncthreads_and(!valid || sg == s_seg0) && s_seg0 < n_segments;
+    if (uniform) {
+#pragma unroll
+      for (int off = 32; off >= 1; off >>= 1) {
+#pragma unroll
+        for (int i = 0; i < 8; i++) h[i] ^= (uint32_t)__shfl_xor((int)h[i], off);
+        const unsigned long long l2 = __shfl_xor(lo, off), h2 = __shfl_xor(hi, off);
+        lo = l2 < lo ? l2 : lo;
+        hi = h2 > hi ? h2 : hi;
+      }
+      if (lane == 0) {
+#pragma unroll
+        for (int i = 0; i < 8; i++) s_ck[wv][i] = h[i];
+        s_lo[wv] = lo;
+        s_hi[wv] = hi;
+      }
+      __syncthreads();
+      if (tid < 8) {
+        uint32_t x = 0;
+        for (uint32_t q = 0; q < META_W; q++) x ^= s_ck[q][tid];
+        t_ck[s_seg0][tid] ^= x;
+      }
+      if (tid == 8) {
+        unsigned long long a = t_lo[s_seg0], b = t_hi[s_seg0];
+        for (uint32_t q = 0; q < META_W; q++) {
+          a = s_lo[q] < a ? s_lo[q] : a;
+          b = s_hi[q] > b ? s_hi[q] : b;
+        }
+        t_lo[s_seg0] = a;
+        t_hi[s_seg0] = b;
+      }
+    } else {
+      if (ck && inc)
+#pragma unroll
+        for (int i = 0; i < 8; i++) atomicXor(&t_ck[sg][i], h[i]);
+      if (times && in_range) {
+        atomicMin(&t_lo[sg], lo);
+        atomicMax(&t_hi[sg], hi);
+      }
+    }
+    __syncthreads();
+  }
+  const uint32_t ncols = n_segments * META_COLS;
+  MetaRow* my = rows + (size_t)blockIdx.x * n_segments;
+  if (tid < n_segments * 8)
+    __hip_atomic_store(&my[tid >> 3].ck[tid & 7u], t_ck[tid >> 3][tid & 7u], __ATOMIC_RELAXED,
+                       __HIP_MEMORY_SCOPE_AGENT);
+  if (tid >= 64 && tid < 64 + n_segments) {
+    __hip_atomic_store(&my[tid - 64].lo, t_lo[tid - 64], __ATOMIC_RELAXED,
+                       __HIP_MEMORY_SCOPE_AGENT);
+    __hip_atomic_store(&my[tid - 64].hi, t_hi[tid - 64], __ATOMIC_RELAXED,
+                       __HIP_MEMORY_SCOPE_AGENT);
+  }
+  asm volatile("s_waitcnt vmcnt(0)" ::: "memory");
+  __syncthreads();
+  if (tid == 0) {
+    const uint32_t t =
+        __hip_atomic_fetch_add(ticket, 1u, __ATOMIC_RELAXED, __HIP_MEMORY_SCOPE_AGENT);
+    const bool last = t == gridDim.x - 1;
+    if (last) {
+      __builtin_amdgcn_fence(__ATOMIC_ACQUIRE, "agent");
+      asm volatile("s_waitcnt vmcnt(0)" ::: "memory");
+    }
+    s_seg0 = last ? 1u : 0u;
+  }
+  __syncthreads();
+  if (!s_seg0) return;
+  const uint32_t G = META_T / ncols, c = tid % ncols, g = tid / ncols;
+  auto fold = [](uint32_t k, unsigned long long v, unsigned long long x) {
+    return k < 8 ? v ^ x : k == 8 ? (x < v ? x : v) : (x > v ? x : v);
+  };
+  if (g < G) {
+    const uint32_t s = c / META_COLS, k = c % META_COLS;
+    unsigned long long v = k == 8 ? ~0ull : 0ull;
+    for (uint32_t b = g; b < gridDim.x; b += G) {
+      const MetaRow* row = rows + (size_t)b * n_segments + s;
+      v = fold(k, v, k < 8 ? row->ck[k] : k == 8 ? row->lo : row->hi);
+    }
+    s_red[g * ncols + c] = v;
+  }
+  __syncthreads();
+  if (tid < 8 * ncols) {
+    const uint32_t k = c % META_COLS;
+    unsigned long long v = k == 8 ? ~0ull : 0ull;
+    for (uint32_t q = g; q < G; q += 8) v = fold(k, v, s_red[q * ncols + c]);
+    s_fin[g][c] = v;
+  }
+  __syncthreads();
+  if (tid < ncols) {
+    const uint32_t k = c % META_COLS;
+    unsigned long long v = s_fin[0][c];
+    for (uint32_t q = 1; q < 8; q++) v = fold(k, v, s_fin[q][c]);
+    s_fin[0][c] = v;
+  }
+  __syncthreads();
+  if (tid < n_segments * 8 && ck)
+    ck[tid] = (uint32_t)s_fin[0][(tid >> 3) * META_COLS + (tid & 7u)];
+  if (tid >= 64 && tid < 64 + n_segments && iv) {
+    const uint32_t s = tid - 64;
+    const unsigned long long lo = s_fin[0][s * META_COLS + 8], hi = s_fin[0][s * META_COLS + 9];
+    iv[2 * s] = hi ? lo : 0;
+    iv[2 * s + 1] = hi ? hi - lo : 0;
+  }
+  if (tid == 0) __hip_atomic_store(ticket, 0u, __ATOMIC_RELAXED, __HIP_MEMORY_SCOPE_AGENT);
 }
 
 __global__ void k_combine_meta(uint32_t k, uint32_t n_segments, const uint32_t* ck_in,
@@ -634,39 +822,51 @@
   return rc;
 }
 
+ZeroRanges fused_first_zero(const Run* R) {
+  ZeroRanges z{};
+  const size_t S = R->nseg ? R->nseg : 1;
+  z.dst[0] = (uint8_t*)R->agg64;
+  z.bytes[0] = S * R->dp.meas_len * 8 * 8;
+  z.dst[1] = (uint8_t*)R->fix;
+  z.bytes[1] = 2 * sizeof(uint32_t);
+  z.dst[2] = (uint8_t*)R->fcnt;
+  z.bytes[2] = 8 * S;
+  return z;
+}
+
 int fused_finish(prio3_engine* e, Run* R, const uint8_t* d_status, const uint32_t* seg,
                  const uint32_t* fix_seg, const uint8_t* d_accept_mask, uint32_t S,
                  uint8_t* d_agg_shares, uint64_t* d_counts, hipStream_t st) {
   const uint32_t n = R->n, M = R->dp.meas_len, ws = R->wshift;
   const uint32_t nwaves = (n + (1u << ws) - 1) >> ws;
-  {
-    ZeroRanges z{};
-    z.dst[0] = (uint8_t*)R->agg64;
-    z.bytes[0] = (size_t)S * M * 8 * 8;
-    z.dst[1] = (uint8_t*)R->fix;
-    z.bytes[1] = sizeof(uint32_t);
-    z.dst[2] = (uint8_t*)d_counts;
-    z.bytes[2] = 8 * (size_t)S;
+  if (!R->fclean) {
+    const ZeroRanges z = fused_first_zero(R);
     TIMED(e, st, "k_zero", (k_zero<<<std::min<uint32_t>(256, (uint32_t)((z.bytes[0] / 16 + 255) / 256) + 1), 256, 0, st>>>(z)));
-  }
+    R->fgen = 0;
+  }
+  R->fclean = false;
+  const uint32_t g = R->fgen & 1u;
   const uint32_t nchunks = (nwaves + WCH - 1) / WCH;
-  dim3 g1((M * 8 / 4 + 255) / 256, nchunks);
-  TIMED(e, st, "k_agg_waves",
-        (k_agg_waves<<<g1, 256, 0, st>>>(nwaves, M, R->wpart, R->wseg, R->cpart, R->cseg,
-                                         R->agg64)));
-  TIMED(e, st, "k_agg_fix",
-        (k_agg_fix<<<(n + fix_per(n) - 1) / fix_per(n), 256, 0, st>>>(
-            n, d_status, seg, d_accept_mask, R->wseg, R->fix, (uint32_t)(R->fix_cap - 1), S,
-            (unsigned long long*)d_counts, fix_seg ? 1u : 0u, fix_per(n), ws)));
+  const uint32_t gx = (M * 8 / 4 + 255) / 256;
+  const uint32_t fix_blocks = (n + fix_per(n) - 1) / fix_per(n);
+  AggFixArgs fx{n, d_status, seg, d_accept_mask, R->fix + g, R->fix + 2, (uint32_t)R->fix_cap, S,
+                R->fcnt, fix_seg ? 1u : 0u, fix_per(n), ws};
+  TIMED(e, st, "k_agg_parts",
+        (k_agg_parts<<<fix_blocks + gx * nchunks, 256, 0, st>>>(
+            fix_blocks, gx, fx, nwaves, M, R->wpart, R->wseg, R->cpart, R->cseg, R->agg64)));
+  const AggFinalArgs fa{R->fix + g, R->fix + 2, R->fix + (g ^ 1u), R->fcnt,
+                        (unsigned long long*)d_counts};
   if (nchunks <= 64 && S > 1)
     TIMED(e, st, "k_agg_final",
           (k_agg_final_s<<<dim3((M + 31) / 32, S), 256, 0, st>>>(
-              M, R->dp.ld, R->agg64, nchunks, R->cpart, R->cseg, R->fix, fix_seg, R->sc.meas,
+              M, R->dp.ld, R->agg64, nchunks, R->cpart, R->cseg, fa, fix_seg, R->sc.meas,
               d_agg_shares)));
   else
     TIMED(e, st, "k_agg_final",
           (k_agg_final<<<S * M, 256, 0, st>>>(M, R->dp.ld, R->agg64, nchunks, R->cpart, R->cseg,
-                                               R->fix, fix_seg, R->sc.meas, d_agg_shares)));
+                                               fa, fix_seg, R->sc.meas, d_agg_shares)));
+  R->fgen++;
+  R->fclean = true;
   return PRIO3_OK;
 }
 
@@ -716,16 +916,58 @@
   });
 }
 
+constexpr size_t STREAM_ZERO_MAX = 64;
+uint32_t* stream_zero_words(int device, hipStream_t st, std::mutex** smu) {
+  struct Ctx {
+    int device;
+    hipStream_t st;
+    uint32_t* mem;
+    std::mutex* mu;
+  };
+  static std::mutex mu;
+  static std::vector<Ctx> all;
+  std::lock_guard<std::mutex> lk(mu);
+  for (const Ctx& c : all)
+    if (c.device == device && c.st == st) {
+      if (smu) *smu = c.mu;
+      return c.mem;
+    }
+  if (all.size() >= STREAM_ZERO_MAX) return nullptr;
+  uint32_t* mem = nullptr;
+  const size_t bytes = 256 + sizeof(MetaRow) * META_BLOCKS * META_FAST_SEGS;
+  if (hipMalloc((void**)&mem, bytes) != hipSuccess) {
+    (void)hipGetLastError();
+    return nullptr;
+  }
+  if (hipMemsetAsync(mem, 0, 256, st) != hipSuccess) {
+    (void)hipGetLastError();
+    (void)hipFree(mem);
+    return nullptr;
+  }
+  all.push_back(Ctx{device, st, mem, new std::mutex});
+  if (smu) *smu = all.back().mu;
+  return mem;
+}
+
 int launch_batch_metadata(prio3_engine* e, uint32_t n, const uint8_t* d_report_ids,
                           const uint64_t* d_times, const uint8_t* d_status,
                           const uint8_t* d_accept_mask, const uint32_t* d_segment_ids,
                           uint32_t n_segments, uint32_t* ck, unsigned long long* iv,
                           hipStream_t st) {
+  if (n_segments <= META_FAST_SEGS)
+    if (uint32_t* ctx = stream_zero_words(e->device, st)) {
+      const uint32_t blocks = std::max(1u, std::min((n + META_T - 1) / META_T, META_BLOCKS));
+      TIMED(e, st, "k_meta",
+            (k_meta<<<blocks, META_T, 0, st>>>(n, d_report_ids, d_times, d_status, d_accept_mask,
+                                               d_segment_ids, n_segments, ck, iv,
+                                               (MetaRow*)(ctx + 64), ctx)));
+      return PRIO3_OK;
+    }
   const uint32_t sb = (n_segments + 255) / 256;
   TIMED(e, st, "k_meta_init", (k_meta_init<<<sb, 256, 0, st>>>(n_segments, ck, iv)));
   if (n)
     TIMED(e, st, "k_meta",
-          (k_meta<<<std::min((n + META_T - 1) / META_T, META_BLOCKS), META_T, 0, st>>>(
+          (k_meta_seg<<<std::min((n + META_T - 1) / META_T, META_BLOCKS), META_T, 0, st>>>(
               n, d_report_ids, d_times, d_status, d_accept_mask, d_segment_ids, n_segments, ck,
               d_times ? iv : nullptr)));
   if (iv) TIMED(e, st, "k_meta_final", (k_meta_final<<<sb, 256, 0, st>>>(n_segments, iv)));
diff --git a/janus_amd/csrc/prio3_common.h b/janus_amd/csrc/prio3_common.h
--- a/janus_amd/csrc/prio3_common.h
+++ b/janus_amd/csrc/prio3_common.h
@@ -102,6 +102,9 @@
   const uint32_t* seg;
   uint32_t* wpart;
   uint32_t* wseg;
+  uint32_t* redo_cnt = nullptr;
+  uint32_t* redo_list = nullptr;
+  uint32_t redo_c0 = 0;
 };
 
 struct OutPtrs {
@@ -550,9 +553,13 @@
   uint8_t *nonces = nullptr, *pub = nullptr, *helper = nullptr, *leader = nullptr,
           *linput = nullptr, *msgs = nullptr, *status = nullptr;
   uint32_t *wpart = nullptr, *wseg = nullptr, *cseg = nullptr, *fix = nullptr;
+  uint32_t* redo_list = nullptr;
   uint4* corr_all = nullptr;
   unsigned long long *cpart = nullptr, *agg64 = nullptr;
   size_t fix_cap = 0;
+  unsigned long long* fcnt = nullptr;
+  uint32_t fgen = 0;
+  bool fclean = false;
   bool fused = false;
   bool aggregate = false;
   bool lfused = false;
diff --git a/janus_amd/csrc/prio3_engine.hip b/janus_amd/csrc/prio3_engine.hip
--- a/janus_amd/csrc/prio3_engine.hip
+++ b/janus_amd/csrc/prio3_engine.hip
@@ -418,6 +418,7 @@
     take(&R->sc.acc, fp ? 16 : es * d.arity * ld);
     take(&R->sc.out, own_out(d) ? es * d.out_len * ldo : 16);
     take(&R->sc.beta, es * d.calls * ld);
+    if (es == 16 && d.P == 32) take(&R->redo_list, 4 * n);
     if (fp) take(&R->corr_all, 16 * n);
   }
   if (flags & RUN_IO) {
@@ -454,7 +455,8 @@
     take(&R->cpart, chunks * M * 8 * 8);
     take(&R->cseg, chunks * sizeof(uint32_t));
     take(&R->agg64, (size_t)(R->nseg ? R->nseg : 1) * M * 8 * 8);
-    take(&R->fix, (n + 1) * sizeof(uint32_t));
+    take(&R->fix, (n + 2) * sizeof(uint32_t));
+    take(&R->fcnt, 8 * (size_t)(R->nseg ? R->nseg : 1));
   }
   return off;
 }
@@ -485,7 +487,7 @@
   }
   run_carve(R, flags, R->slab->base);
   R->keep = e->keep_scratch != 0;
-  R->fix_cap = (size_t)n + 1;
+  R->fix_cap = (size_t)n;
   R->last = st;
   return R;
 }
diff --git a/janus_amd/csrc/prio3_host.h b/janus_amd/csrc/prio3_host.h
--- a/janus_amd/csrc/prio3_host.h
+++ b/janus_amd/csrc/prio3_host.h
@@ -2,6 +2,7 @@
 #include <hip/hip_runtime.h>
 
 #include <cstdio>
+#include <mutex>
 #include <vector>
 
 #include "prio3_common.h"
@@ -61,6 +62,26 @@
 }
 
 constexpr uint32_t WCH = 32;
+
+struct ZeroRanges {
+  uint8_t* dst[4];
+  size_t bytes[4];
+};
+__device__ __forceinline__ void zero_ranges(const ZeroRanges& z, size_t tid, size_t nth) {
+#pragma unroll
+  for (int k = 0; k < 4; k++) {
+    uint8_t* d = z.dst[k];
+    const size_t n = z.bytes[k];
+    if (!d || !n) continue;
+    const size_t h0 = (16 - ((uintptr_t)d & 15)) & 15, head = n < h0 ? n : h0;
+    const size_t n16 = (n - head) / 16;
+    for (size_t i = tid; i < n16; i += nth) ((uint4*)(d + head))[i] = make_uint4(0, 0, 0, 0);
+    for (size_t i = tid * 4; i < head; i += nth * 4) *(uint32_t*)(d + i) = 0u;
+    for (size_t i = head + 16 * n16 + tid * 4; i < n; i += nth * 4) *(uint32_t*)(d + i) = 0u;
+  }
+}
+ZeroRanges fused_first_zero(const Run* R);
+uint32_t* stream_zero_words(int device, hipStream_t st, std::mutex** mu = nullptr);
 
 struct PooledStream {
   int device;
diff --git a/janus_amd/csrc/prio3_prepare.hip b/janus_amd/csrc/prio3_prepare.hip
--- a/janus_amd/csrc/prio3_prepare.hip
+++ b/janus_amd/csrc/prio3_prepare.hip
@@ -180,7 +180,7 @@
 }
 
 
-template <bool FUSE, bool TR = false, bool PULL = false>
+template <bool FUSE, bool TR = false, bool PULL = false, bool LIST = false>
 __device__ __forceinline__ void xofd_body(const DevParams& p, const InPtrs& in, const Scratch& sc,
                                           const uint32_t r) {
   typedef Fp128 F;
@@ -438,6 +438,17 @@
     sc.corrected[r] = make_uint4(cor[0], cor[1], cor[2], cor[3]);
   }
   sc.flag[r] = (uint8_t)flag;
+  if constexpr (LIST) {
+    const uint64_t fm = __ballot(flag != 0);
+    if (fm && sc.redo_cnt) {
+      const uint32_t first = (uint32_t)__ffsll((long long)fm) - 1u;
+      uint32_t base = 0;
+      if (lane == first) base = atomicAdd(sc.redo_cnt, (uint32_t)__popcll(fm));
+      base = (uint32_t)__shfl((int)base, (int)first);
+      if (flag)
+        sc.redo_list[base + (uint32_t)__popcll(fm & ((1ull << lane) - 1ull))] = sc.redo_c0 + r;
+    }
+  }
   if constexpr (FUSE) {
     if (fuse) {
       const bool anyflag = __any(flag != 0);
@@ -1680,7 +1691,7 @@
 __global__ __launch_bounds__(XOFD_BLOCK, 3) void k_prep_h(DevParams p, InPtrs in, Scratch sc,
                                                    OutPtrs out) {
   const uint32_t r = blockIdx.x * blockDim.x + threadIdx.x;
-  xofd_body<FUSE, false, PULL>(p, in, sc, r);
+  xofd_body<FUSE, false, PULL, true>(p, in, sc, r);
   query_h_body<2, 32>(p, in, sc, out, r);
 }
 
@@ -1702,7 +1713,26 @@
 }
 
 template <int PP>
-__global__ __launch_bounds__(64) void k_slow_redo(DevParams p, InPtrs in, Scratch sc, OutPtrs out) {
+__global__ __launch_bounds__(64) void k_slow_redo(DevParams p, InPtrs in, Scratch sc, OutPtrs out,
+                                                  ZeroRanges z) {
+  zero_ranges(z, blockIdx.x * (size_t)blockDim.x + threadIdx.x, (size_t)gridDim.x * blockDim.x);
+  if (sc.redo_cnt) {
+    const uint32_t cnt = __hip_atomic_load(sc.redo_cnt, __ATOMIC_RELAXED, __HIP_MEMORY_SCOPE_AGENT);
+    for (uint32_t i = blockIdx.x * blockDim.x + threadIdx.x; i < cnt; i += gridDim.x * blockDim.x) {
+      const uint32_t r = sc.redo_list[i];
+      xof_slow_one<Fp128>(p, in, sc, r);
+      query_h_body<2, PP>(p, in, sc, out, r);
+    }
+    if (threadIdx.x == 0) {
+      const uint32_t t = __hip_atomic_fetch_add(sc.redo_cnt + 1, 1u, __ATOMIC_ACQ_REL,
+                                                __HIP_MEMORY_SCOPE_AGENT);
+      if (t == gridDim.x - 1) {
+        __hip_atomic_store(sc.redo_cnt, 0u, __ATOMIC_RELAXED, __HIP_MEMORY_SCOPE_AGENT);
+        __hip_atomic_store(sc.redo_cnt + 1, 0u, __ATOMIC_RELAXED, __HIP_MEMORY_SCOPE_AGENT);
+      }
+    }
+    return;
+  }
   const uint32_t r0 = (blockIdx.x * blockDim.x + threadIdx.x) * REDO_RPL;
   if (r0 >= p.n || !redo_any(p, sc, r0)) return;
   const uint8_t* fl = sc.flag + r0;
@@ -1771,7 +1801,8 @@
   return ps && dual && dp.P == 32;
 }
 
-enum : int { DEFER_NONE = 0, DEFER_QH = 1, DEFER_SUM = 2, DEFER_GEN64 = 3 };
+enum : int { DEFER_NONE = 0, DEFER_QH = 1, DEFER_SUM = 2, DEFER_GEN64 = 3, DEFER_QH_LIST = 4 };
+constexpr uint32_t REDO_LIST_BLOCKS = 32;
 static int launch_prepare(prio3_engine* e, const DevParams& base, uint32_t c0, uint32_t n,
                           InPtrs in, OutPtrs out, Scratch sc, hipStream_t st, bool fuse,
                           int* deferred, bool pair = false) {
@@ -1798,6 +1829,7 @@
   if (sc.seg) sc.seg += c0;
   if (sc.wseg) sc.wseg += c0 / 64;
   if (sc.wpart) sc.wpart += (size_t)(c0 / 64) * dp.meas_len * 8;
+  sc.redo_c0 = c0;
   const uint32_t blocks = (n + 255) / 256;
   const uint32_t xblocks = (n + XOFD_BLOCK - 1) / XOFD_BLOCK;
   if (dp.kind == PRIO3_SUMVEC_F64_MP) {
@@ -1864,6 +1896,7 @@
         bool paired = false;
         if (pair)
           TIMED(e, st, "k_prep_hp", (paired = launch_prep_pair(dp, in, sc, out, st, fuse, pl)));
+        if (!paired && deferred) *deferred = DEFER_QH_LIST;
         if (paired) {
         } else if (fuse && pl)
           TIMED(e, st, "k_prep_h", (k_prep_h<true, true><<<xblocks, XOFD_BLOCK, 0, st>>>(dp, in, sc, out)));
@@ -1918,14 +1951,19 @@
 }
 
 static int launch_slow_redo(prio3_engine* e, const DevParams& base, uint32_t n, InPtrs in,
-                            OutPtrs out, Scratch sc, hipStream_t st, int family) {
+                            OutPtrs out, Scratch sc, hipStream_t st, int family, Run* R) {
+  const bool list = family == DEFER_QH_LIST && sc.redo_cnt;
+  if (family == DEFER_QH_LIST) family = DEFER_QH;
+  if (!list) sc.redo_cnt = nullptr;
+  const bool clean = R && R->agg64 && family == DEFER_QH;
+  const ZeroRanges z = clean ? fused_first_zero(R) : ZeroRanges{};
   DevParams dp = base;
   dp.n = n;
   dp.force_slow = (uint32_t)e->force_slow;
   dp.trunc_xof = 0;
   dp.slow_defer = 1;
   dp.redo = 1;
-  const uint32_t g = redo_blocks(n);
+  const uint32_t g = list ? REDO_LIST_BLOCKS : redo_blocks(n);
   if (family == DEFER_GEN64) {
     TIMED(e, st, "k_slow_redo", (k_slow_redo_gen<Fp64><<<g, 64, 0, st>>>(dp, in, sc, out)));
   } else if (family == DEFER_SUM) {
@@ -1936,11 +1974,15 @@
       default: TIMED(e, st, "k_slow_redo", (k_slow_redo_sum<8><<<g, 64, 0, st>>>(dp, in, sc, out))); break;
     }
   } else if (dp.P == 32)
-    TIMED(e, st, "k_slow_redo", (k_slow_redo<32><<<g, 64, 0, st>>>(dp, in, sc, out)));
+    TIMED(e, st, "k_slow_redo", (k_slow_redo<32><<<g, 64, 0, st>>>(dp, in, sc, out, z)));
   else if (dp.P == 16)
-    TIMED(e, st, "k_slow_redo", (k_slow_redo<16><<<g, 64, 0, st>>>(dp, in, sc, out)));
+    TIMED(e, st, "k_slow_redo", (k_slow_redo<16><<<g, 64, 0, st>>>(dp, in, sc, out, z)));
   else
-    TIMED(e, st, "k_slow_redo", (k_slow_redo<8><<<g, 64, 0, st>>>(dp, in, sc, out)));
+    TIMED(e, st, "k_slow_redo", (k_slow_redo<8><<<g, 64, 0, st>>>(dp, in, sc, out, z)));
+  if (clean) {
+    R->fclean = true;
+    R->fgen = 0;
+  }
   return PRIO3_OK;
 }
 
@@ -1976,6 +2018,15 @@
   sc.seg = R->seg;
   sc.wpart = R->wpart;
   sc.wseg = R->wseg;
+  std::unique_lock<std::mutex> zlock;
+  if (R->redo_list && prep_fused_takes(e, R->dp, fuse) && R->dp.kind != PRIO3_SUM) {
+    std::mutex* zmu = nullptr;
+    if (uint32_t* zw = stream_zero_words(R->device, st, &zmu)) {
+      zlock = std::unique_lock<std::mutex>(*zmu);
+      sc.redo_cnt = zw + 1;
+      sc.redo_list = R->redo_list;
+    }
+  }
   R->last = st;
   const bool pair = pair_takes(e, R->dp, n, fuse, in.leader_src != nullptr);
   R->wshift = pair ? 5u : 6u;
@@ -1988,7 +2039,7 @@
   if (pair || !allow_chunks || K == 1 || n <= csz || R->dp.kind == PRIO3_FPVEC_BOUNDED_L2) {
     const int rc = launch_prepare(e, R->dp, 0, n, in, out, sc, st, fuse, &deferred, pair);
     if (rc == PRIO3_OK && deferred)
-      return launch_slow_redo(e, R->dp, n, in, out, sc, st, deferred);
+      return launch_slow_redo(e, R->dp, n, in, out, sc, st, deferred, R);
     return rc;
   }
   int rc = ensure_side_streams(e);
@@ -2005,7 +2056,7 @@
     HIPCHK(hipEventRecord(e->side_ev[i], e->side[i]));
     HIPCHK(hipStreamWaitEvent(st, e->side_ev[i], 0));
   }
-  if (deferred) return launch_slow_redo(e, R->dp, n, in, out, sc, st, deferred);
+  if (deferred) return launch_slow_redo(e, R->dp, n, in, out, sc, st, deferred, R);
   return PRIO3_OK;
 }
 
```

New measurement: 182.1 million reports/s, median of 6. 1.01x the previous value.
